# GuidoManni/BodySLAM

Measured on AMD Instinct MI355X. Metric: frames/sec depth+pose+back-proj, 640x480 seq, higher is better.
Workload: dtype f16

## Files before the change

bodyslam_amd/_lib.py:

```python
from __future__ import annotations

import ctypes as C
import os
from typing import Optional

import torch

_HERE = os.path.dirname(os.path.abspath(__file__))
LIB_PATH = os.environ.get("BODYSLAM_HIP_LIB") or os.path.join(_HERE, "libbodyslam_hip.so")

F32, F16, BF16 = 0, 1, 2
F64 = 3
ACT_NONE, ACT_RELU, ACT_GELU, ACT_SOFTPLUS, ACT_SOFTPLUS_FAST = 0, 1, 2, 3, 4
OUT_PLAIN, OUT_SHUFFLE, OUT_QKV = 0, 1, 2

_TORCH2BS = {torch.float32: F32, torch.float16: F16, torch.bfloat16: BF16}
BS2TORCH = {F32: torch.float32, F16: torch.float16, BF16: torch.bfloat16}


class BodySlamHipError(RuntimeError):
    pass


class GemmDesc(C.Structure):
    _fields_ = [
        ("A", C.c_void_p), ("W", C.c_void_p), ("dtype", C.c_int32),
        ("M", C.c_int32), ("N", C.c_int32), ("K", C.c_int32), ("lda", C.c_int32), ("conv", C.c_int32),
        ("Hin", C.c_int32), ("Win", C.c_int32), ("Cin", C.c_int32), ("Hout", C.c_int32), ("Wout", C.c_int32),
        ("KH", C.c_int32), ("KW", C.c_int32), ("stride", C.c_int32), ("pad_h", C.c_int32), ("pad_w", C.c_int32),
        ("relu_a", C.c_int32),
        ("bias", C.c_void_p), ("bias_group_rows", C.c_int32), ("act", C.c_int32),
        ("scale", C.c_void_p), ("res", C.c_void_p), ("res_dtype", C.c_int32), ("ldr", C.c_int32), ("res2", C.c_void_p),
        ("out", C.c_void_p), ("out2", C.c_void_p), ("out3", C.c_void_p),
        ("out_dtype", C.c_int32), ("ldo", C.c_int32), ("out_mode", C.c_int32),
        ("out_group_rows", C.c_int32), ("out_group_stride", C.c_int32), ("out_row_offset", C.c_int32),
        ("shuffle_s", C.c_int32), ("shuffle_cout", C.c_int32),
        ("qkv_hidden", C.c_int32), ("qkv_tokens", C.c_int32), ("qkv_sp", C.c_int32), ("q_scale", C.c_float),
        ("tile", C.c_int32), ("seg1", C.c_int32), ("out_split_off", C.c_int32), ("res_split_off", C.c_int32),
        ("f8_seg", C.c_int32), ("f8_scales", C.c_uint32), ("out_f8", C.c_int32), ("res_f8", C.c_int32),
        ("qkv_cls_last", C.c_int32), ("qkv_cls_rows", C.c_int32), ("qkv_patch_row0", C.c_int32), ("f8_wonly_from", C.c_int32), ("out_lo8_rows", C.c_int32),
        ("f8_skip_from", C.c_int32), ("bias2_row0", C.c_int32), ("bias2_group_rows", C.c_int32), ("out_planes_rows", C.c_int32),
        ("bias2", C.c_void_p),
        ("qkv_lo_off", C.c_int32), ("out2_relu", C.c_int32),
    ]


_lib: Optional[C.CDLL] = None

_SIGS = {
    "bs_init": [C.c_int],
    "bs_version": [],
    "bs_gemm": [C.POINTER(GemmDesc), C.c_void_p],
    "bs_gemm_tile": [C.POINTER(GemmDesc)],
    "bs_attention": [C.c_void_p] * 5 + [C.c_int32] * 5 + [C.c_void_p],
    "bs_attention_table": [C.c_void_p] * 5 + [C.c_int32] * 7 + [C.c_void_p],
    "bs_attention_table_corr": [C.c_void_p] * 8 + [C.c_int32] * 7 + [C.c_void_p],
    "bs_layernorm": [C.c_void_p] * 5 + [C.c_int32, C.c_int32, C.c_float, C.c_int32, C.c_void_p],
    "bs_cast": [C.c_void_p, C.c_void_p, C.c_int64, C.c_int32, C.c_void_p],
    "bs_copy_f32": [C.c_void_p, C.c_void_p, C.c_int64, C.c_void_p],
    "bs_cast_split": [C.c_void_p, C.c_void_p, C.c_int64, C.c_int32, C.c_int32, C.c_void_p],
    "bs_relu_split": [C.c_void_p, C.c_void_p, C.c_int64, C.c_int32, C.c_int32, C.c_void_p],
    "bs_preprocess_patches": [C.c_void_p, C.c_void_p] + [C.c_int32] * 7 + [C.c_void_p],
    "bs_preprocess_image": [C.c_void_p, C.c_void_p] + [C.c_int32] * 6 + [C.c_void_p],
    "bs_fill_rows": [C.c_void_p, C.c_void_p, C.c_int32, C.c_int32, C.c_int32, C.c_void_p],
    "bs_resize_bilinear_nhwc": [C.c_void_p, C.c_void_p] + [C.c_int32] * 8 + [C.c_void_p],
    "bs_upconv_tapsum": [C.c_void_p] * 3 + [C.c_int32] * 9 + [C.c_void_p],
    "bs_upconv_fused": [C.c_void_p] * 4 + [C.c_int32] * 15 + [C.c_void_p],
    "bs_resize_bias_relu_nhwc": [C.c_void_p] * 3 + [C.c_int32] * 8 + [C.c_void_p],
    "bs_col_mean": [C.c_void_p, C.c_int64] + [C.c_int32] * 5 + [C.c_void_p, C.c_void_p, C.c_int64, C.c_int32, C.c_void_p],
    "bs_rank1_bias": [C.c_void_p] * 3 + [C.c_int32] * 3 + [C.c_void_p],
    "bs_depth_u16_to_m": [C.c_void_p, C.c_int64, C.c_double, C.c_double, C.c_void_p, C.c_void_p],
    "bs_engine_load": [C.c_char_p, C.c_void_p],
    "bs_engine_destroy": [C.c_void_p],
    "bs_engine_io": [C.c_void_p, C.c_char_p, C.c_void_p, C.c_void_p],
    "bs_engine_device_bytes": [C.c_void_p],
    "bs_engine_run": [C.c_void_p, C.c_void_p],
    "bs_engine_upload": [C.c_void_p, C.c_char_p, C.c_void_p, C.c_int64],
    "bs_engine_download": [C.c_void_p, C.c_char_p, C.c_void_p, C.c_int64],
    "bs_zoedepth_forward": [C.c_void_p, C.c_void_p, C.c_int32, C.c_int32, C.c_int32, C.c_void_p, C.c_void_p, C.c_void_p],
    "bs_cyclepose_forward": [C.c_void_p, C.c_void_p, C.c_int32, C.c_int32, C.c_int32, C.c_void_p, C.c_int32, C.c_void_p, C.c_void_p],
    "bs_tsdf_frames_upload": [C.c_void_p, C.c_void_p, C.c_void_p, C.c_void_p, C.c_void_p, C.c_int32, C.c_void_p, C.c_void_p],
    "bs_tsdf_touch_batch": [C.c_void_p, C.c_int32, C.c_int32, C.c_int32, C.c_int32, C.c_double, C.c_double, C.c_void_p, C.c_void_p, C.c_int32, C.c_void_p,
                            C.c_void_p],
    "bs_tsdf_integrate_batch": [C.c_void_p, C.c_int32, C.c_int32, C.c_int32, C.c_void_p, C.c_void_p, C.c_void_p, C.c_int32, C.c_void_p, C.c_int32, C.c_void_p,
                                C.c_void_p, C.c_void_p, C.c_void_p, C.c_int32, C.c_int32, C.c_double, C.c_double, C.c_void_p],
    "bs_tsdf_update_batch": [C.c_void_p, C.c_int32, C.c_int32, C.c_int32, C.c_void_p, C.c_void_p, C.c_void_p, C.c_int32, C.c_void_p, C.c_int32, C.c_void_p,
                             C.c_void_p, C.c_void_p, C.c_void_p, C.c_int32, C.c_int32, C.c_double, C.c_double, C.c_uint64, C.c_void_p],
    "bs_odo_prepare": [C.c_void_p, C.c_void_p, C.c_int32, C.c_int32, C.c_int32, C.c_double, C.c_void_p, C.c_void_p, C.c_void_p],
    "bs_odo_pyrdown": [C.c_void_p, C.c_int32, C.c_int32, C.c_int32, C.c_void_p, C.c_int32, C.c_double, C.c_void_p],
    "bs_odo_sobel": [C.c_void_p, C.c_int32, C.c_int32, C.c_int32, C.c_void_p, C.c_void_p, C.c_void_p],
    "bs_odo_accumulate": [C.c_void_p] * 8 + [C.c_int32, C.c_int32, C.c_void_p, C.c_void_p, C.c_double, C.c_double, C.c_double, C.c_void_p, C.c_void_p,
                                              C.c_int32, C.c_void_p],
    "bs_odo_step": [C.c_void_p] * 8 + [C.c_int32, C.c_int32, C.c_int32, C.c_void_p, C.c_void_p, C.c_int32, C.c_double, C.c_double, C.c_double, C.c_void_p,
                                        C.c_void_p, C.c_int32, C.c_void_p],
    "bs_odo_p2p_prepare": [C.c_void_p, C.c_int32, C.c_int32, C.c_int32, C.c_double, C.c_void_p, C.c_void_p],
    "bs_odo_p2p_target": [C.c_void_p, C.c_int32, C.c_int32, C.c_int32, C.c_void_p, C.c_void_p, C.c_void_p],
    "bs_odo_p2p_accumulate": [C.c_void_p, C.c_void_p, C.c_int32, C.c_int32, C.c_void_p, C.c_void_p, C.c_double, C.c_double, C.c_void_p, C.c_void_p,
                              C.c_void_p],
    "bs_odo_p2p_step": [C.c_void_p, C.c_void_p, C.c_int32, C.c_int32, C.c_int32, C.c_void_p, C.c_void_p, C.c_int32, C.c_double, C.c_double, C.c_void_p,
                        C.c_void_p, C.c_void_p],
    "bs_tsdf_extract": [C.c_void_p, C.c_int32, C.c_void_p, C.c_void_p, C.c_int32, C.c_void_p, C.c_int32, C.c_int32, C.c_double, C.c_void_p, C.c_void_p,
                        C.c_void_p, C.c_void_p, C.c_void_p, C.c_void_p],
    "bs_tsdf_mesh": [C.c_void_p, C.c_int32, C.c_void_p, C.c_void_p, C.c_int32, C.c_void_p, C.c_int32, C.c_int32, C.c_double, C.c_void_p, C.c_int32] + [C.c_void_p] * 7,
    "bs_tsdf_raycast": [C.c_void_p, C.c_void_p, C.c_int32, C.c_int32, C.c_int32, C.c_double, C.c_double, C.c_void_p, C.c_void_p, C.c_int32, C.c_void_p,
                        C.c_int32, C.c_int32, C.c_double, C.c_double, C.c_void_p, C.c_void_p, C.c_void_p, C.c_void_p, C.c_void_p],
    "bs_attractor_step": [C.c_void_p] * 4 + [C.c_int32] * 8 + [C.c_void_p],
    "bs_add_resized": [C.c_void_p] * 3 + [C.c_int32] * 7 + [C.c_void_p],
    "bs_mlp2": [C.c_void_p, C.c_int32] + [C.c_void_p] * 5 + [C.c_int32] * 6 + [C.c_void_p],
    "bs_mlp2_add": [C.c_void_p] * 7 + [C.c_int32] * 10 + [C.c_void_p],
    "bs_projector_level": [C.c_void_p] * 10 + [C.c_int32] * 9 + [C.c_void_p],
    "bs_logbinom_depth": [C.c_void_p] * 8 + [C.c_int32] * 5 + [C.c_float, C.c_float, C.c_int32, C.c_void_p],
    "bs_logbinom_depth_ex": [C.c_void_p] * 7 + [C.c_int32] + [C.c_void_p] * 2 + [C.c_int32] * 5 + [C.c_float, C.c_float, C.c_int32, C.c_void_p],
    "bs_small_attention": [C.c_void_p, C.c_void_p, C.c_int32, C.c_int32, C.c_int32, C.c_int32, C.c_void_p],
    "bs_route_argmax": [C.c_void_p, C.c_int32, C.c_void_p, C.c_int32, C.c_void_p],
    "bs_postprocess_depth": [C.c_void_p] * 3 + [C.c_int32] * 6 + [C.c_void_p],
    "bs_cyclepose_im2col": [C.c_void_p] * 3 + [C.c_int32] * 4 + [C.c_void_p],
    "bs_cyclepose_im2col_window": [C.c_void_p] * 3 + [C.c_int32] * 8 + [C.c_void_p],
    "bs_instnorm_relu_nhwc": [C.c_void_p] * 4 + [C.c_int32] * 3 + [C.c_float, C.c_int32, C.c_void_p],
    "bs_avgpool_nhwc": [C.c_void_p, C.c_void_p, C.c_int32, C.c_int32, C.c_int32, C.c_void_p],
    "bs_cyclepose_head": [C.c_void_p] * 12 + [C.c_int32] * 3 + [C.c_void_p],
    "bs_backproject": [C.c_void_p, C.c_int32, C.c_int32, C.c_int32, C.c_void_p, C.c_double, C.c_double] + [C.c_void_p] * 6,
    "bs_pose_chain": [C.c_void_p, C.c_int32, C.c_void_p, C.c_void_p, C.c_void_p],
    "bs_pose_chain_from": [C.c_void_p, C.c_int32, C.c_void_p, C.c_void_p, C.c_void_p],
    "bs_pixel_to_3d": [C.c_void_p, C.c_int64, C.c_void_p, C.c_void_p, C.c_void_p],
    "bs_depth_metrics_workspace": [C.c_int32, C.c_int32, C.c_int32],
    "bs_depth_metrics": [C.c_void_p, C.c_void_p] + [C.c_int32] * 3 + [C.c_double, C.c_double, C.c_int32, C.c_double, C.c_void_p, C.c_int64,
# ... 88 lines not shown


_inited_device: Optional[int] = None


def init(device: int = 0) -> None:
    global _inited_device
    lib = load_library()
    if _inited_device == device:
        return
    if not torch.cuda.is_available():
        raise BodySlamHipError("bodyslam_amd needs an MI355X (gfx950) GPU: torch.cuda.is_available() is False "
                               "and there is no CPU fallback")
    check(lib.bs_init(device), "bs_init")
    _inited_device = device


def check(status: int, what: str) -> None:
    if status != 0:
        msg = load_library().bs_last_error().decode(errors="replace")
        raise BodySlamHipError(f"{what} failed with status {status}: {msg}")


def stream_ptr() -> int:
    return torch.cuda.current_stream().cuda_stream


def dt(t: torch.Tensor) -> int:
    return _TORCH2BS[t.dtype]


def p(t: Optional[torch.Tensor]) -> Optional[int]:
    return None if t is None else t.data_ptr()


def make_gemm_desc(A: torch.Tensor, W: torch.Tensor, out: torch.Tensor, *, M: int, N: int, K: int, lda: int,
                   conv=None, relu_a: bool = False, bias: Optional[torch.Tensor] = None, bias_group_rows: int = 0,
                   act: int = ACT_NONE, scale: Optional[torch.Tensor] = None, res: Optional[torch.Tensor] = None,
                   res2: Optional[torch.Tensor] = None, ldr: int = 0, ldo: Optional[int] = None, out_group=None,
                   shuffle=None, qkv=None, a_offset: int = 0, tile: int = 0, seg1: int = 0, out_split_off: int = 0,
                   res_split_off: int = 0, f8_seg: int = 0, f8_scales=(127, 127, 127, 127), out_f8=None, res_f8: bool = False,
                   f8_wonly_from: int = 0, out_lo8_rows: int = 0, f8_skip_from: int = 0, bias2=None, out_planes_rows: int = 0,
                   out_relu: Optional[torch.Tensor] = None) -> GemmDesc:
    d = GemmDesc()
    d.A = A.data_ptr() + a_offset * A.element_size()
    d.W = W.data_ptr()
    assert A.dtype == W.dtype and A.dtype in (torch.float16, torch.bfloat16), (A.dtype, W.dtype)
    d.dtype = dt(A)
    d.M, d.N, d.K, d.lda = M, N, K, lda
    if conv is not None:
        d.conv = 1
        (d.Hin, d.Win, d.Cin, d.Hout, d.Wout, d.KH, d.KW, d.stride, d.pad_h, d.pad_w) = conv
    d.relu_a = int(relu_a)
    if bias is not None:
        assert bias.dtype == torch.float32
        d.bias = bias.data_ptr()
    d.bias_group_rows = bias_group_rows
    d.act = act
    if scale is not None:
        assert scale.dtype == torch.float32
        d.scale = scale.data_ptr()
    if res is not None:
        d.res = res.data_ptr()
        d.res_dtype = dt(res)
        d.ldr = ldr if ldr else N
    if res2 is not None:
        assert res is not None and res2.dtype == A.dtype
        d.res2 = res2.data_ptr()
    d.out = out.data_ptr()
    d.out_dtype = dt(out)
    d.ldo = N if ldo is None else ldo
    if out_group is not None:
        d.out_group_rows, d.out_group_stride, d.out_row_offset = out_group
    if shuffle is not None:
        d.out_mode = OUT_SHUFFLE
        d.shuffle_s, d.shuffle_cout, d.Hout, d.Wout = shuffle
    if qkv is not None:
        d.out_mode = OUT_QKV
        hidden, tokens, sp, q_scale, out_k, out_vt = qkv[:6]
        d.qkv_cls_last = int(bool(qkv[6])) if len(qkv) > 6 else 0
        d.qkv_cls_rows = int(qkv[7]) if len(qkv) > 7 else 0
        d.qkv_patch_row0 = int(qkv[8]) if len(qkv) > 8 else d.qkv_cls_rows
        d.qkv_lo_off = int(qkv[9]) if len(qkv) > 9 else 0
        d.qkv_hidden, d.qkv_tokens, d.qkv_sp, d.q_scale = hidden, tokens, sp, q_scale
        d.out2 = out_k.data_ptr()
        d.out3 = out_vt.data_ptr()
    d.tile = tile
    d.seg1, d.out_split_off, d.res_split_off = seg1, out_split_off, res_split_off
    d.f8_seg = f8_seg
    d.f8_scales = f8_scales[0] | (f8_scales[1] << 8) | (f8_scales[2] << 16) | (f8_scales[3] << 24)
    d.out_f8 = 0 if out_f8 is None else ((out_f8[0] & 0xff) | ((out_f8[1] & 0xff) << 8))
    d.res_f8 = int(res_f8)
    d.f8_wonly_from = f8_wonly_from
    d.out_lo8_rows = out_lo8_rows
    d.f8_skip_from = f8_skip_from
    d.out_planes_rows = out_planes_rows
    if bias2 is not None:
        b2, row0, grows = bias2
        assert b2.dtype == torch.float32 and b2.shape[-1] == N
        d.bias2, d.bias2_row0, d.bias2_group_rows = b2.data_ptr(), row0, grows
    if out_relu is not None:
        assert qkv is None and out_f8 is not None and out_relu.dtype == out.dtype and out_relu.numel() == out.numel()
        d.out2 = out_relu.data_ptr()
        d.out2_relu = 1
    return d


def gemm(A: torch.Tensor, W: torch.Tensor, out: torch.Tensor, **kw) -> None:
    d = make_gemm_desc(A, W, out, **kw)
    check(load_library().bs_gemm(C.byref(d), stream_ptr()), "bs_gemm")


def _gemm_bytes(d) -> float:
    rows_in = float(d.M if not d.conv else d.M / max(d.stride * d.stride, 1))
    rows_f8 = 0.0 if d.f8_skip_from < 0 else (rows_in if (d.conv or not d.f8_skip_from) else float(min(d.f8_skip_from, d.M)))
    taps = d.KH * d.KW if d.conv else 1
    a = rows_in * (d.Cin if d.conv else d.K) * 2 + rows_f8 * d.f8_seg
    w = float(d.N) * (d.K * 2 + taps * d.f8_seg)
    if d.out_dtype == F32:
        per_row = [4.0, 4.0, 4.0]
    elif d.out_f8:
        per_row = [4.0, 3.0, 2.0]
    else:
        per_row = [2.0 * (2 if d.out_split_off else 1)] * 3
    full = float(d.M)
    r_planes = float(min(d.out_planes_rows, d.M)) if d.out_planes_rows else full
    r_lo = float(min(d.out_lo8_rows, d.M)) if d.out_lo8_rows else r_planes
    r_lo = min(r_lo, r_planes)
    out = d.N * (r_lo * per_row[0] + (r_planes - r_lo) * per_row[1] + (full - r_planes) * per_row[2])
    res = float(d.M) * d.N * (4 if (d.res and d.res_dtype == F32) else 0)
    return a + w + out + res


class Plan:

    def __init__(self, device=None):
        self.device = None if device is None else torch.device(device)
        self.calls = []
        self.names = []
        self.keep = []
        self.keep_descs = []
        self.marks = {}
        self.gemm_info = {}
        self.stack_info = {}
        self.events = None
        self._graph = None

    def gemm(self, name, A, W, out, **kw):
        passes = kw.pop("precision_passes", 1)
        d = make_gemm_desc(A, W, out, **kw)
        kw["precision_passes"] = passes
        self.keep.append((d, A, W, out, kw))
        self.keep_descs.append(d)
        self.calls.append((load_library().bs_gemm, (C.byref(d),)))
        self.names.append(name)
        self.gemm_info[len(self.calls) - 1] = dict(
            name=name, tile=load_library().bs_gemm_tile(C.byref(d)), conv=bool(d.conv),
            flops=2.0 * d.N * (d.M * d.K + (0 if d.f8_skip_from < 0 else (min(d.f8_skip_from, d.M) if d.f8_skip_from else d.M)) * (d.KH * d.KW if d.conv else 1) * d.f8_seg
                               / (4 if d.f8_wonly_from else 2)),
            alg_flops=2.0 * d.M * d.N * (d.K / kw.get("precision_passes", 1)),
            bytes=_gemm_bytes(d))

    def add(self, name, fn_name, *args):
        cargs = []
        for a in args:
            if isinstance(a, torch.Tensor):
# ... 73 lines not shown
def _f8_pack_device(device):
    if device is None or os.environ.get("BS_PACK_ON_HOST") == "1":
        return torch.device("cpu")
    device = torch.device(device)
    if device.type != "cuda":
        return torch.device("cpu")
    ok = _F8_ON_DEVICE.get(device.index)
    if ok is None:
        g = torch.Generator().manual_seed(7)
        t = torch.cat([torch.randn(4096, generator=g) * 100.0, torch.randn(4096, generator=g) * 1e-2, torch.linspace(-460.0, 460.0, 4097),
                       torch.arange(0, 4096, dtype=torch.float32) * 2.0 ** -11, torch.tensor([0.0, -0.0, 448.0, -448.0, 2.0 ** -9, 2.0 ** -10, 3 * 2.0 ** -11])])
        t = t.clamp(-448.0, 448.0)
        try:
            ok = bool(torch.equal(t.to(torch.float8_e4m3fn).view(torch.uint8), t.to(device).to(torch.float8_e4m3fn).view(torch.uint8).cpu()))
        except Exception:
            ok = False
        _F8_ON_DEVICE[device.index] = ok
    return device if ok else torch.device("cpu")


def f8_weight(w: torch.Tensor, dtype, planes: str = "both", device=None) -> tuple:
    import math
    w = w.detach().to(_f8_pack_device(device)).float()
    hi = w.to(dtype)
    lo = w - hi.float()

    def plane(t):
        mx = float(t.abs().max())
        e = 0 if mx == 0.0 else min(int(math.floor(math.log2(448.0 / mx))), 100)
        return (t * (2.0 ** e)).clamp(-448.0, 448.0).to(torch.float8_e4m3fn).view(torch.uint8), e

    hi8, e_hi = plane(hi.float())
    lo8, e_lo = plane(lo)
    hi16 = hi.contiguous().view(torch.uint8).view(w.shape[0], -1)
    if planes == "lo":
        row = torch.cat([hi16, lo8], 1).contiguous()
    elif planes == "hi_only":
        row = torch.cat([hi16, torch.zeros_like(lo8), hi8], 1).contiguous()
    else:
        row = torch.cat([hi16, lo8, hi8], 1).contiguous()
    return row.view(dtype), (127 - e_lo, 127 - e_hi)


def f8_conv_weight(w_ohwi: torch.Tensor, dtype, device=None) -> tuple:
    import math
    w = w_ohwi.detach().to(_f8_pack_device(device)).float()
    O, kh, kw, I = w.shape
    assert I % 128 == 0, I
    hi = w.to(dtype)
    lo = w - hi.float()

    def plane(t):
        mx = float(t.abs().max())
        e = 0 if mx == 0.0 else min(int(math.floor(math.log2(448.0 / mx))), 100)
        q = (t * (2.0 ** e)).clamp(-448.0, 448.0).to(torch.float8_e4m3fn).view(torch.uint8)
        return q.reshape(O, kh, kw, I // 128, 128).permute(0, 3, 1, 2, 4).reshape(O, -1), e

    hi8, e_hi = plane(hi.float())
    lo8, e_lo = plane(lo)
    hi16 = conv_weight(hi).view(torch.uint8).view(O, -1)
    row = torch.cat([hi16, lo8, hi8], 1).contiguous()
    return row.view(dtype), (127 - e_lo, 127 - e_hi)


F8_ACT_HI_EXP, F8_ACT_LO_EXP = 0, 11


def conv_weight(w_ohwi: torch.Tensor) -> torch.Tensor:
    O, kh, kw, I = w_ohwi.shape
    assert I % 64 == 0, I
    return w_ohwi.reshape(O, kh, kw, I // 64, 64).permute(0, 3, 1, 2, 4).reshape(O, -1).contiguous()


def conv_geom(Hin, Win, Cin, KH, KW, stride, pad):
    Hout = (Hin + 2 * pad - KH) // stride + 1
    Wout = (Win + 2 * pad - KW) // stride + 1
    return (Hin, Win, Cin, Hout, Wout, KH, KW, stride, pad, pad)


def attention(q, k, vt, bias, out, B, nh, S, Sp, split=0):
    check(load_library().bs_attention(p(q), p(k), p(vt), p(bias), p(out), B, nh, S, Sp, dt(q) | split, stream_ptr()), "bs_attention")


def attention_table(q, k, vt, table, out, B, nh, hp, wp, Sp, split=0, grouped=0):
    check(load_library().bs_attention_table(p(q), p(k), p(vt), p(table), p(out), B, nh, hp, wp, Sp, int(grouped), dt(q) | split, stream_ptr()),
          "bs_attention_table")


def attention_table_corr(q, k, vt, q_lo, k_lo, vt_lo, table, out, B, nh, hp, wp, Sp, split=0, grouped=0):
    check(load_library().bs_attention_table_corr(p(q), p(k), p(vt), p(q_lo), p(k_lo), p(vt_lo), p(table), p(out), B, nh, hp, wp, Sp, int(grouped),
                                                 dt(q) | split, stream_ptr()), "bs_attention_table_corr")


def layernorm(x, gamma, beta, out16, out32, rows, cols, eps, dtype=F16):
    check(load_library().bs_layernorm(p(x), p(gamma), p(beta), p(out16), p(out32), rows, cols, eps,
                                      dt(out16) if out16 is not None else dtype, stream_ptr()), "bs_layernorm")


def cast(x, out):
    check(load_library().bs_cast(p(x), p(out), x.numel(), dt(out), stream_ptr()), "bs_cast")


def cast_split(x, out, rows, cols, f8=False):
    check(load_library().bs_cast_split(p(x), p(out), rows, cols, dt(out) | (32 if f8 else 0), stream_ptr()), "bs_cast_split")


def relu_split(x, out, rows, cols, f8=False):
    check(load_library().bs_relu_split(p(x), p(out), rows, cols, dt(out) | (32 if f8 else 0), stream_ptr()), "bs_relu_split")


def preprocess_patches(frames, out, B, H, W, nh, nw, flip):
    check(load_library().bs_preprocess_patches(p(frames), p(out), B, H, W, nh, nw, int(flip), dt(out), stream_ptr()),
          "bs_preprocess_patches")


def preprocess_image(frames, out, B, H, W, nh, nw, flip):
    check(load_library().bs_preprocess_image(p(frames), p(out), B, H, W, nh, nw, int(flip), stream_ptr()), "bs_preprocess_image")


def fill_rows(x, v, B, rows_per_image, cols):
    check(load_library().bs_fill_rows(p(x), p(v), B, rows_per_image, cols, stream_ptr()), "bs_fill_rows")


def resize_bilinear_nhwc(x, out, B, Hin, Win, Cch, Hout, Wout, align_corners=True, split=False):
    check(load_library().bs_resize_bilinear_nhwc(p(x), p(out), B, Hin, Win, Cch, Hout, Wout, int(align_corners) | (4 if split == 2 else (2 if split else 0)), dt(x),
                                                 stream_ptr()), "bs_resize_bilinear_nhwc")


def depth_u16_to_m(depth_u16: torch.Tensor, depth_scale: float, depth_trunc: float) -> torch.Tensor:
    assert depth_u16.dtype == torch.int16 and depth_u16.is_cuda and depth_u16.is_contiguous()
    out = torch.empty(depth_u16.shape, dtype=torch.float32, device=depth_u16.device)
    check(load_library().bs_depth_u16_to_m(p(depth_u16), depth_u16.numel(), float(depth_scale), float(depth_trunc), p(out), stream_ptr()),
          "bs_depth_u16_to_m")
    return out


def col_mean(A, lda, row0, rows_per_group, groups, row_step, K, out, zero=None):
    assert out.dtype == torch.bfloat16 and (zero is None or zero.dtype == torch.float32)
    check(load_library().bs_col_mean(p(A), lda, row0, rows_per_group, groups, row_step, K, p(out), p(zero), 0 if zero is None else zero.numel(),
                                     dt(A), stream_ptr()), "bs_col_mean")


def rank1_bias(abar, dw, out):
    assert abar.dtype == torch.bfloat16 and dw.dtype == torch.bfloat16 and out.dtype == torch.float32
    G, K = abar.shape
    N = dw.shape[0]
    assert dw.shape[1] == K and tuple(out.shape) == (G, N)
    check(load_library().bs_rank1_bias(p(abar), p(dw), p(out), G, N, K, stream_ptr()), "bs_rank1_bias")


def upconv_tapsum(y, bias, out, B, Hin, Win, Cout, Hout, Wout, align_corners=True, split=False, relu=True):
    check(load_library().bs_upconv_tapsum(p(y), p(bias), p(out), B, Hin, Win, Cout, Hout, Wout,
                                          int(align_corners) | (4 if split == 2 else (2 if split else 0)), int(relu), dt(out), stream_ptr()),
          "bs_upconv_tapsum")


def upconv_fused(x, w, bias, out, B, Hin, Win, Cin, Cout, mode=0, split=0, relu=True, f8_scales=(127, 127, 127, 127)):
    check(load_library().bs_upconv_fused(p(x), p(w), p(bias), p(out), B, Hin, Win, Cin, Cout, 2 * Hin, 2 * Win,
                                         1 | (4 if split == 2 else (2 if split else 0)), int(relu), mode, *[int(v) for v in f8_scales], dt(out),
                                         stream_ptr()), "bs_upconv_fused")


def resize_bias_relu_nhwc(x, bias, out, B, Hin, Win, Cch, Hout, Wout, split=False):
    check(load_library().bs_resize_bias_relu_nhwc(p(x), p(bias), p(out), B, Hin, Win, Cch, Hout, Wout, 1 | (2 if split else 0), dt(out), stream_ptr()),
          "bs_resize_bias_relu_nhwc")


def attractor_step(A, bins_prev, bins_out, route, B, Hp, Wp, H, W, groups, n_bins, n_attr):
    check(load_library().bs_attractor_step(p(A), p(bins_prev), p(bins_out), p(route), B, Hp, Wp, H, W, groups, n_bins, n_attr,
                                           stream_ptr()), "bs_attractor_step")


def mlp2(x, ldx, W1, b1, W2, b2, out, M, K1, N1, N2, act2=ACT_SOFTPLUS_FAST):
    check(load_library().bs_mlp2(p(x), ldx, p(W1), p(b1), p(W2), p(b2), p(out), M, K1, N1, N2, act2, dt(x), stream_ptr()), "bs_mlp2")
# ... 631 lines not shown
```

bodyslam_amd/csrc/attention.hip:

```cpp
#include <stdlib.h>

#include <type_traits>

#include "common.h"

namespace bs {
__device__ __forceinline__ float half_swap_max(float v) {
    int k = __builtin_bit_cast(int, v);
    k ^= (k >> 31) & 0x7fffffff;
    const auto sw = __builtin_amdgcn_permlane32_swap((unsigned)k, (unsigned)k, false, false);
    const int a = (int)sw[0], b = (int)sw[1];
    int m = a > b ? a : b;
    m ^= (m >> 31) & 0x7fffffff;
    return __builtin_bit_cast(float, m);
}

__device__ __forceinline__ void dma_barrier() {
    asm volatile("s_waitcnt vmcnt(0)" ::: "memory");
    __syncthreads();
}


template <typename T, int QW>
__global__ __launch_bounds__(QW * 64) void attention_kernel(const T* __restrict__ Q, const T* __restrict__ K, const T* __restrict__ Vt,
// ... 359 lines not shown
    dma_barrier();
    if (1 < nkt) stage(1, 1);
    load_bias(0);
    for (int kt = 0; kt < nkt; ++kt) {
        if (ablate & 32) break;
        if (kt > 0) {
            dma_barrier();
            if (kt + 1 < nkt && !(ablate & 16)) stage(kt + 1, (kt + 1) & 1);
        }
        const char* sk = smem + (kt & 1) * STAGE;
        const char* sv = sk + 8 * 1024;
#pragma unroll
        for (int sub = 0; sub < 2; ++sub) {
            const int ky = kt * 2 + sub;
            if (ky > hp) break;
            f32x16 sacc;
#pragma unroll
            for (int i = 0; i < 16; ++i) sacc[i] = bnext[i] - m_run;
            if (ky + 1 <= hp && !(ablate & 8)) load_bias(ky + 1);
            const int krow = sub * 32 + kap;
#pragma unroll
            for (int ks = 0; ks < 4; ++ks) {
                if (ablate & 4) break;
                const int chunk = 2 * ks + h2;
                const v8 kf = *reinterpret_cast<const v8*>(sk + krow * 128 + ((chunk ^ ((krow >> 1) & 7)) << 4));
                sacc = T16<T>::mfma32(kf, qf[ks], sacc);
            }
            float mloc = fmaxf(fmaxf(sacc[0], sacc[1]), sacc[2]);
#pragma unroll
            for (int i = 3; i < 15; i += 2) mloc = fmaxf(fmaxf(mloc, sacc[i]), sacc[i + 1]);
            mloc = fmaxf(mloc, sacc[15]);
            mloc = half_swap_max(mloc);
            if (first || __any(mloc > THR)) {
                const float sh = first ? mloc : fmaxf(mloc, 0.0f);
                const float alpha = first ? 1.0f : __builtin_amdgcn_exp2f(-sh);
                l_run *= alpha;
#pragma unroll
                for (int i = 0; i < 16; ++i) {
                    oacc[0][i] *= alpha;
                    oacc[1][i] *= alpha;
                    sacc[i] -= sh;
                }
                m_run += sh;
                first = false;
            }
            float p[16];
            float psum = 0.f;
            if (ablate & 1) {
#pragma unroll
                for (int i = 0; i < 16; ++i) p[i] = sacc[i];
            } else {
#pragma unroll
                for (int i = 0; i < 16; ++i) {
                    p[i] = __builtin_amdgcn_exp2f(sacc[i]);
                    psum += p[i];
                }
            }
            l_run += psum;
            v8 pf[2];
#pragma unroll
            for (int s2 = 0; s2 < 2; ++s2)
#pragma unroll
                for (int e = 0; e < 8; ++e) pf[s2][e] = T16<T>::from_f32(p[8 * s2 + e]);
#pragma unroll
            for (int dh = 0; dh < 2; ++dh) {
                if (ablate & 2) break;
                const int drow = dh * 32 + r;
#pragma unroll
                for (int s2 = 0; s2 < 2; ++s2) {
                    const int chunk = sub * 4 + 2 * s2 + h2;
                    const v8 vf = *reinterpret_cast<const v8*>(sv + drow * 128 + ((chunk ^ ((drow >> 1) & 7)) << 4));
                    oacc[dh] = T16<T>::mfma32(vf, pf[s2], oacc[dh]);
                }
            }
        }
    }
    const float l_tot = l_run + __shfl_xor(l_run, 32, 64);
    const float inv = 1.0f / l_tot;
    __syncthreads();
    store_out_tile<T>(smem + wave * 8192, oacc, inv, out, split, nh, head, grouped ? (int64_t)grouped + (int64_t)b * (S - 1) : (int64_t)b * S + 1,
                      grouped ? (int64_t)b : (int64_t)b * S, S, q0, active, lane, cls_planes);
}

template <typename T, int QW, bool CORR>
__device__ __forceinline__ void cls_query_pass(const T* __restrict__ Qg, const T* __restrict__ Kg, const T* __restrict__ Vg, const T* __restrict__ Qlg,
                                               const T* __restrict__ Klg, const T* __restrict__ Vlg, int Sp, int hp, const float* __restrict__ tail3,
                                               char* area, int wave, int lane, T* __restrict__ out, int split, int nh, int head, int64_t row0,
                                               int64_t row_cls, int S, bool cls_planes) {
    typedef typename T16<T>::v8 v8;
    const int r = lane & 31, h2 = lane >> 5;
    const int kap = (r & ~12) | ((r & 4) << 1) | ((r & 8) >> 1);
    const int q0 = hp * 32;
    constexpr float THR = 6.0f;
    const float b_cp = tail3[0], b_cc = tail3[2];
    v8 qf[4], qlf[CORR ? 4 : 1];
#pragma unroll
    for (int ks = 0; ks < 4; ++ks) {
        qf[ks] = *reinterpret_cast<const v8*>(Qg + (int64_t)(q0 + r) * 64 + ks * 16 + h2 * 8);
        if constexpr (CORR) qlf[ks] = *reinterpret_cast<const v8*>(Qlg + (int64_t)(q0 + r) * 64 + ks * 16 + h2 * 8);
    }
    f32x16 oacc[2];
#pragma unroll
    for (int i = 0; i < 16; ++i) {
        oacc[0][i] = 0.f;
        oacc[1][i] = 0.f;
    }
    float m_run = 0.f, l_run = 0.f;
    bool first = true;
    auto load_k = [&](int ky, v8 (&kf)[4], v8 (&kfl)[CORR ? 4 : 1]) {
        const int64_t krow = (int64_t)ky * 32 + kap;
#pragma unroll
        for (int ks = 0; ks < 4; ++ks) {
            kf[ks] = *reinterpret_cast<const v8*>(Kg + krow * 64 + (2 * ks + h2) * 8);
            if constexpr (CORR) kfl[ks] = *reinterpret_cast<const v8*>(Klg + krow * 64 + (2 * ks + h2) * 8);
        }
    };
    v8 kf[4], kfl[CORR ? 4 : 1];
    load_k(wave, kf, kfl);
#pragma unroll 1
    for (int ky = wave; ky <= hp; ky += QW) {
        v8 vf[4], vfl[CORR ? 4 : 1];
#pragma unroll
        for (int dh = 0; dh < 2; ++dh)
#pragma unroll
            for (int s2 = 0; s2 < 2; ++s2) {
                const int64_t voff = (int64_t)(dh * 32 + r) * Sp + ky * 32 + (2 * s2 + h2) * 8;
                vf[dh * 2 + s2] = *reinterpret_cast<const v8*>(Vg + voff);
                if constexpr (CORR) vfl[dh * 2 + s2] = *reinterpret_cast<const v8*>(Vlg + voff);
            }
        v8 kn[4], knl[CORR ? 4 : 1];
        const int kyn = ky + QW <= hp ? ky + QW : ky;
        load_k(kyn, kn, knl);
        f32x16 sacc;
#pragma unroll
        for (int i = 0; i < 16; ++i) sacc[i] = (ky < hp ? b_cp : -1.0e30f) - m_run;
        if (ky == hp && h2 == 0) sacc[0] = b_cc - m_run;
#pragma unroll
        for (int ks = 0; ks < 4; ++ks) {
            sacc = T16<T>::mfma32(kf[ks], qf[ks], sacc);
            if constexpr (CORR) {
                sacc = T16<T>::mfma32(kf[ks], qlf[ks], sacc);
                sacc = T16<T>::mfma32(kfl[ks], qf[ks], sacc);
            }
        }
        float mloc = sacc[0];
#pragma unroll
        for (int i = 1; i < 16; ++i) mloc = fmaxf(mloc, sacc[i]);
        mloc = half_swap_max(mloc);
        if (first || __any(mloc > THR)) {
            const float sh = first ? mloc : fmaxf(mloc, 0.0f);
            const float alpha = first ? 1.0f : __builtin_amdgcn_exp2f(-sh);
            l_run *= alpha;
#pragma unroll
            for (int i = 0; i < 16; ++i) {
                oacc[0][i] *= alpha;
                oacc[1][i] *= alpha;
                sacc[i] -= sh;
            }
            m_run += sh;
            first = false;
        }
        float psum = 0.f;
        v8 pf[2], pfl[CORR ? 2 : 1];
#pragma unroll
        for (int s2 = 0; s2 < 2; ++s2)
#pragma unroll
            for (int e = 0; e < 8; ++e) {
                const float pv = __builtin_amdgcn_exp2f(sacc[8 * s2 + e]);
                psum += pv;
                pf[s2][e] = T16<T>::from_f32(pv);
                if constexpr (CORR) pfl[s2][e] = T16<T>::from_f32(pv - T16<T>::to_f32(pf[s2][e]));
            }
        l_run += psum;
#pragma unroll
        for (int dh = 0; dh < 2; ++dh)
#pragma unroll
            for (int s2 = 0; s2 < 2; ++s2) {
                oacc[dh] = T16<T>::mfma32(vf[dh * 2 + s2], pf[s2], oacc[dh]);
                if constexpr (CORR) {
                    oacc[dh] = T16<T>::mfma32(vf[dh * 2 + s2], pfl[s2], oacc[dh]);
                    oacc[dh] = T16<T>::mfma32(vfl[dh * 2 + s2], pf[s2], oacc[dh]);
                }
            }
#pragma unroll
        for (int ks = 0; ks < 4; ++ks) {
            kf[ks] = kn[ks];
            if constexpr (CORR) kfl[ks] = knl[ks];
        }
    }
    const float l_tot = l_run + __shfl_xor(l_run, 32, 64);
    float* part = reinterpret_cast<float*>(area);
    if (r == 0) {
        float* pp = part + (wave * 2 + h2) * 36;
        pp[0] = m_run;
        pp[1] = l_tot;
#pragma unroll
        for (int i = 0; i < 16; ++i) {
            pp[2 + i] = oacc[0][i];
            pp[18 + i] = oacc[1][i];
        }
    }
    __syncthreads();
    if (wave != 0) return;
    float M = part[h2 * 36];
#pragma unroll 1
    for (int w = 1; w < QW; ++w) M = fmaxf(M, part[(w * 2 + h2) * 36]);
    float L = 0.f;
#pragma unroll
    for (int i = 0; i < 16; ++i) {
        oacc[0][i] = 0.f;
        oacc[1][i] = 0.f;
    }
#pragma unroll 1
    for (int w = 0; w < QW; ++w) {
        const float* pp = part + (w * 2 + h2) * 36;
        const float f = __builtin_amdgcn_exp2f(pp[0] - M);
        L = fmaf(pp[1], f, L);
#pragma unroll
        for (int i = 0; i < 16; ++i) {
            oacc[0][i] = fmaf(pp[2 + i], f, oacc[0][i]);
            oacc[1][i] = fmaf(pp[18 + i], f, oacc[1][i]);
        }
    }
    __builtin_amdgcn_fence(__ATOMIC_RELEASE, "wavefront");
    __builtin_amdgcn_wave_barrier();
    store_out_tile<T>(area, oacc, 1.0f / L, out, split, nh, head, row0, row_cls, S, q0, true, lane, cls_planes);
}

template <typename T, int QW, int WPE, bool CORR, bool PK = false, bool CLS2 = false>
__global__ __launch_bounds__(QW * 64, WPE) void attention_tab2_kernel(const T* __restrict__ Q, const T* __restrict__ K, const T* __restrict__ Vt,
                                                                  const T* __restrict__ Ql, const T* __restrict__ Kl, const T* __restrict__ Vtl,
                                                                  const float* __restrict__ table, T* __restrict__ out, int split, int B, int nh,
                                                                  int hp, int Sp, int nqb, int ntab, int grouped) {
    BS_ARG_NOW(out);
    const bool cls_planes = (split & 4) != 0;
    const int abl = split >> 3;
    split &= 3;
    typedef typename T16<T>::v8 v8;
    constexpr int HALF = 16 * 1024;
    constexpr int STAGE = CORR ? 2 * HALF : HALF;
    constexpr int WP = 32, RW = 2 * WP - 1;
    extern __shared__ __attribute__((aligned(16))) char smem[];
    float* tab = reinterpret_cast<float*>(smem + 2 * STAGE);
    const int ntab_pad = (ntab + 255) & ~255;
    float* creg = tab + ntab_pad;
    const int S = hp * WP + 1, nqt = CLS2 ? hp : hp + 1;

    const int nwg = gridDim.x, bid = blockIdx.x;
    const int xq = nwg >> 3, xr = nwg & 7, xcd = bid & 7, loc = bid >> 3;
    const int wg = (xcd < xr ? xcd * (xq + 1) : xr * (xq + 1) + (xcd - xr) * xq) + loc;
    const int qblk = wg % nqb;
    const int b = (wg / nqb) % B;
    const int head = wg / (B * nqb);

    const int tid = threadIdx.x, lane = tid & 63;
    const int wave = __builtin_amdgcn_readfirstlane(tid >> 6);
    const int r = lane & 31, h2 = lane >> 5;
    int qt = qblk * QW + wave;
    const bool active = qt < nqt;
    qt = active ? qt : nqt - 1;
    const int q0 = qt * 32;
    const bool cls_tile = !CLS2 && qt == hp;
    const int64_t bh = (int64_t)b * nh + head;

    const T* Qg = Q + bh * Sp * 64;
    const T* Kg = K + bh * Sp * 64;
    const T* Vg = Vt + bh * 64 * Sp;
    const T* Klg = CORR ? Kl + bh * Sp * 64 : nullptr;
    const T* Vlg = CORR ? Vtl + bh * 64 * Sp : nullptr;

    load_table<QW * 64>(tab, table, head, ntab, tid, wave, lane);
    if (tid < 64) creg[tid] = table[(int64_t)head * ntab + ntab - 3];

    v8 qf[4], qlf[CORR ? 4 : 1];
#pragma unroll
    for (int ks = 0; ks < 4; ++ks) qf[ks] = *reinterpret_cast<const v8*>(Qg + (int64_t)(q0 + r) * 64 + ks * 16 + h2 * 8);
    if constexpr (CORR) {
#pragma unroll
        for (int ks = 0; ks < 4; ++ks) qlf[ks] = *reinterpret_cast<const v8*>(Ql + bh * Sp * 64 + (int64_t)(q0 + r) * 64 + ks * 16 + h2 * 8);
    }

    const int srow = lane >> 3;
    auto stage = [&](int kt, int buf) {
        char* sb = smem + buf * STAGE;
        for (int i = wave; i < (CORR ? 32 : 16); i += QW) {
            const int j = i & 15;
            const int row = (j & 7) * 8 + srow;
            const int cs8 = ((lane & 7) ^ ((row >> 1) & 7)) * 8;
            const T* kb = (CORR && i >= 16) ? Klg : Kg;
            const T* vb = (CORR && i >= 16) ? Vlg : Vg;
            const T* src = j < 8 ? kb + (int64_t)(kt * 64 + row) * 64 + cs8 : vb + (int64_t)row * Sp + kt * 64 + cs8;
            glds16(src, sb + i * 1024);
        }
    };

    f32x16 oacc[2];
#pragma unroll
    for (int i = 0; i < 16; ++i) {
        oacc[0][i] = 0.f;
        oacc[1][i] = 0.f;
    }
    float m_run = 0.f, l_run = 0.f;
    bool first = true;
    const int kap = (r & ~12) | ((r & 4) << 1) | ((r & 8) >> 1);
    constexpr float THR = 6.0f;

    const int nbody = ntab - 3;
    const float* lt = cls_tile ? creg : tab + (nbody - RW - (qt + hp - 1) * RW) + (31 - r + 8 * h2);
    const int rstep = cls_tile ? 0 : RW;
    auto load_bias = [&](f32x16& sacc, int ky) {
        const float* rowp = lt + ky * rstep;
#pragma unroll
        for (int s2 = 0; s2 < 2; ++s2)
#pragma unroll
            for (int e = 0; e < 8; ++e) sacc[8 * s2 + e] = rowp[16 * s2 + e];
    };
    auto qk = [&](f32x16& sacc, const char* sk, int sub) {
        if constexpr (PK) {
            const f32x2_ nm = {-m_run, -m_run};
#pragma unroll
            for (int i = 0; i < 16; i += 2) {
                const f32x2_ v = f32x2_{sacc[i], sacc[i + 1]} + nm;
                sacc[i] = v[0];
                sacc[i + 1] = v[1];
            }
        } else {
#pragma unroll
            for (int i = 0; i < 16; ++i) sacc[i] -= m_run;
        }
        const int krow = sub * 32 + kap;
#pragma unroll
        for (int ks = 0; ks < 4; ++ks) {
            const int chunk = 2 * ks + h2;
            const int off = krow * 128 + ((chunk ^ ((krow >> 1) & 7)) << 4);
            const v8 kf = *reinterpret_cast<const v8*>(sk + off);
            sacc = T16<T>::mfma32(kf, qf[ks], sacc);
            if constexpr (CORR) {
                sacc = T16<T>::mfma32(kf, qlf[ks], sacc);
                const v8 kfl = *reinterpret_cast<const v8*>(sk + HALF + off);
                sacc = T16<T>::mfma32(kfl, qf[ks], sacc);
            }
        }
    };
    auto softmax_pv = [&](f32x16& sacc, f32x16& other, const char* sv, int sub, int next_ky, auto other_tag, auto next_tag) {
        constexpr bool OTHER = decltype(other_tag)::value;
        constexpr bool NEXT = decltype(next_tag)::value;
        float mloc = fmaxf(fmaxf(sacc[0], sacc[1]), sacc[2]);
#pragma unroll
        for (int i = 3; i < 15; i += 2) mloc = fmaxf(fmaxf(mloc, sacc[i]), sacc[i + 1]);
        mloc = fmaxf(mloc, sacc[15]);
        mloc = half_swap_max(mloc);
        if (first || __any(mloc > THR)) {
                const float sh = first ? mloc : fmaxf(mloc, 0.0f);
                const float alpha = first ? 1.0f : __builtin_amdgcn_exp2f(-sh);
            l_run *= alpha;
#pragma unroll
            for (int i = 0; i < 16; ++i) {
                oacc[0][i] *= alpha;
                oacc[1][i] *= alpha;
                sacc[i] -= sh;
                if (OTHER) other[i] -= sh;
            }
            m_run += sh;
            first = false;
        }
        float psum = 0.f;
        v8 pf[2], pfl[CORR ? 2 : 1];
#pragma unroll
        for (int s2 = 0; s2 < 2; ++s2)
#pragma unroll
            for (int e = 0; e < 8; ++e) {
                const float pv = __builtin_amdgcn_exp2f(sacc[8 * s2 + e]);
                psum += pv;
                pf[s2][e] = T16<T>::from_f32(pv);
                if constexpr (CORR) pfl[s2][e] = T16<T>::from_f32(pv - T16<T>::to_f32(pf[s2][e]));
            }
        l_run += psum;
        if (NEXT) load_bias(sacc, next_ky);
#pragma unroll
        for (int dh = 0; dh < 2; ++dh) {
            const int drow = dh * 32 + r;
#pragma unroll
            for (int s2 = 0; s2 < 2; ++s2) {
                const int chunk = sub * 4 + 2 * s2 + h2;
                const int off = drow * 128 + ((chunk ^ ((drow >> 1) & 7)) << 4);
                const v8 vf = *reinterpret_cast<const v8*>(sv + off);
                oacc[dh] = T16<T>::mfma32(vf, pf[s2], oacc[dh]);
                if constexpr (CORR) {
                    oacc[dh] = T16<T>::mfma32(vf, pfl[s2], oacc[dh]);
                    const v8 vfl = *reinterpret_cast<const v8*>(sv + HALF + off);
                    oacc[dh] = T16<T>::mfma32(vfl, pf[s2], oacc[dh]);
                }
            }
        }
    };

    const int NT = hp >> 1;
    f32x16 sa, sb2;
    typedef std::true_type Yes;
    typedef std::false_type No;
    stage(0, 0);
    dma_barrier();
    load_bias(sa, 0);
    load_bias(sb2, 1);
    for (int kt = 0; kt < NT - 1; ++kt) {
        if (kt > 0) {
            if (abl == 0) dma_barrier();
            else {
                if (!(abl & 2)) asm volatile("s_waitcnt vmcnt(0)" ::: "memory");
                if (!(abl & 1)) __syncthreads();
            }
        }
        if (!(abl & 4) || kt == 0) stage(kt + 1, (kt + 1) & 1);
        const char* sk = smem + (kt & 1) * STAGE;
        qk(sa, sk, 0);
        qk(sb2, sk, 1);
        softmax_pv(sa, sb2, sk + 8 * 1024, 0, 2 * kt + 2, Yes{}, Yes{});
        softmax_pv(sb2, sa, sk + 8 * 1024, 1, 2 * kt + 3, No{}, Yes{});
    }
    {
        if (NT > 1) dma_barrier();
        stage(NT, NT & 1);
        const char* sk = smem + ((NT - 1) & 1) * STAGE;
        qk(sa, sk, 0);
        qk(sb2, sk, 1);
        softmax_pv(sa, sb2, sk + 8 * 1024, 0, 0, Yes{}, No{});
#pragma unroll
        for (int i = 0; i < 16; ++i) sa[i] = -1.0e30f;
        if (h2 == 0) sa[0] = cls_tile ? tab[ntab - 1] : tab[ntab - 2];
        softmax_pv(sb2, sa, sk + 8 * 1024, 1, 0, No{}, No{});
        dma_barrier();
        const char* sk2 = smem + (NT & 1) * STAGE;
        qk(sa, sk2, 0);
        softmax_pv(sa, sb2, sk2 + 8 * 1024, 0, 0, No{}, No{});
    }
    const float l_tot = l_run + __shfl_xor(l_run, 32, 64);
    const float inv = 1.0f / l_tot;
    __syncthreads();
    store_out_tile<T>(smem + wave * 8192, oacc, inv, out, split, nh, head, grouped ? (int64_t)grouped + (int64_t)b * (S - 1) : (int64_t)b * S + 1,
                      grouped ? (int64_t)b : (int64_t)b * S, S, q0, active, lane, cls_planes);
    if constexpr (CLS2) {
        if (qblk == 0) {
            __syncthreads();
            cls_query_pass<T, QW, CORR>(Qg, Kg, Vg, CORR ? Ql + bh * Sp * 64 : nullptr, Klg, Vlg, Sp, hp, table + (int64_t)head * ntab + ntab - 3,
                                        smem + 2 * STAGE + (ntab_pad + 64) * 4, wave, lane, out, split, nh, head,
                                        grouped ? (int64_t)grouped + (int64_t)b * (S - 1) : (int64_t)b * S + 1, grouped ? (int64_t)b : (int64_t)b * S, S,
                                        cls_planes);
        }
    }
}

template <typename T>
static int launch_attn_tab(const void* q, const void* k, const void* vt, const void* ql, const void* kl, const void* vtl, const float* table, void* out,
                           int split, int B, int nh, int hp, int Sp, int grouped, hipStream_t st) {
    constexpr int QW = 5;
    const int nqt = hp + 1, nqb = cdiv(nqt, QW), ntab = (2 * hp - 1) * 63 + 3;
    const int tab_bytes = (((ntab + 255) & ~255) + 64) * 4;
    if (ql) {
        static const bool cls2_ok = diag_env("BS_ATTN_NO_CLS2") == nullptr;
        if (cls2_ok && hp % 8 == 0) {
            auto kb = attention_tab2_kernel<T, 8, 2, true, false, true>;
            BS_MAX_DYNAMIC_LDS(reinterpret_cast<const void*>(kb), 96 * 1024);
            hipLaunchKernelGGL(kb, dim3(B * nh * (hp / 8)), dim3(8 * 64), 64 * 1024 + tab_bytes + 8192, st, (const T*)q, (const T*)k, (const T*)vt,
                               (const T*)ql, (const T*)kl, (const T*)vtl, table, (T*)out, split, B, nh, hp, Sp, hp / 8, ntab, grouped);
            BS_CHECK_LAUNCH();
            return BS_OK;
        }
        {
            const int nb8 = cdiv(nqt, 8), qw8 = cdiv(nqt, nb8);
#define BS_ATTN_CORR_BIG(QWB)                                                                                                                \
    do {                                                                                                                                     \
        auto kb = attention_tab2_kernel<T, QWB, 2, true>;                                                                                    \
        BS_MAX_DYNAMIC_LDS(reinterpret_cast<const void*>(kb), 96 * 1024); \
        hipLaunchKernelGGL(kb, dim3(B * nh * nb8), dim3(QWB * 64), 64 * 1024 + tab_bytes, st, (const T*)q, (const T*)k, (const T*)vt,        \
                           (const T*)ql, (const T*)kl, (const T*)vtl, table, (T*)out, split, B, nh, hp, Sp, nb8, ntab, grouped);             \
        BS_CHECK_LAUNCH();                                                                                                                   \
        return BS_OK;                                                                                                                        \
    } while (0)
            if (qw8 == 7) BS_ATTN_CORR_BIG(7);
            if (qw8 == 8) BS_ATTN_CORR_BIG(8);
#undef BS_ATTN_CORR_BIG
        }
        auto kc = attention_tab2_kernel<T, QW, 2, true>;
        BS_MAX_DYNAMIC_LDS(reinterpret_cast<const void*>(kc), 88 * 1024);
        hipLaunchKernelGGL(kc, dim3(B * nh * nqb), dim3(QW * 64), 64 * 1024 + tab_bytes, st, (const T*)q, (const T*)k, (const T*)vt, (const T*)ql,
                           (const T*)kl, (const T*)vtl, table, (T*)out, split, B, nh, hp, Sp, nqb, ntab, grouped);
        BS_CHECK_LAUNCH();
        return BS_OK;
    }
    int smem = 32 * 1024 + ((ntab * 4 + 1023) & ~1023);
    smem = smem < QW * 8192 ? QW * 8192 : smem;
    auto kern = attention_tab_kernel<T, QW>;
    BS_MAX_DYNAMIC_LDS(reinterpret_cast<const void*>(kern), 64 * 1024);
    static const bool pipelined_ok = diag_env("BS_ATTN_NO_PIPE") == nullptr;
    if (hp % 2 == 0 && pipelined_ok) {
        static const bool wpe3 = diag_env("BS_ATTN_WPE3") != nullptr, pk = diag_env("BS_ATTN_NO_PK") == nullptr;
        auto kern2 = wpe3 ? (pk ? attention_tab2_kernel<T, QW, 3, false, true> : attention_tab2_kernel<T, QW, 3, false>)
                          : (pk ? attention_tab2_kernel<T, QW, 4, false, true> : attention_tab2_kernel<T, QW, 4, false>);
        BS_MAX_DYNAMIC_LDS(reinterpret_cast<const void*>(kern2), 64 * 1024);
        static const int abl = diag_env("BS_ATTN_ABL") ? atoi(diag_env("BS_ATTN_ABL")) : 0;
        static const bool cls2_ok = diag_env("BS_ATTN_NO_CLS2") == nullptr;
        if (!wpe3 && pk && abl == 0 && cls2_ok && hp % 8 == 0) {
            auto kb = attention_tab2_kernel<T, 8, 4, false, true, true>;
            BS_MAX_DYNAMIC_LDS(reinterpret_cast<const void*>(kb), 128 * 1024);
            const int ldsb = 8 * 8192 > 32 * 1024 + tab_bytes + 8192 ? 8 * 8192 : 32 * 1024 + tab_bytes + 8192;
            hipLaunchKernelGGL(kb, dim3(B * nh * (hp / 8)), dim3(8 * 64), ldsb, st, (const T*)q, (const T*)k, (const T*)vt, (const T*)nullptr,
                               (const T*)nullptr, (const T*)nullptr, table, (T*)out, split, B, nh, hp, Sp, hp / 8, ntab, grouped);
            BS_CHECK_LAUNCH();
            return BS_OK;
        }
        if (!wpe3 && pk && abl == 0) {
            const int nb_big = cdiv(nqt, 14), qw_big = cdiv(nqt, nb_big);
#define BS_ATTN_BIG(QWB)                                                                                                                     \
    do {                                                                                                                                     \
        auto kb = attention_tab2_kernel<T, QWB, 4, false, true>;                                                                             \
        BS_MAX_DYNAMIC_LDS(reinterpret_cast<const void*>(kb), 128 * 1024); \
        const int ldsb = QWB * 8192 > 32 * 1024 + tab_bytes ? QWB * 8192 : 32 * 1024 + tab_bytes;                                            \
        hipLaunchKernelGGL(kb, dim3(B * nh * nb_big), dim3(QWB * 64), ldsb, st, (const T*)q, (const T*)k, (const T*)vt, (const T*)nullptr,   \
                           (const T*)nullptr, (const T*)nullptr, table, (T*)out, split, B, nh, hp, Sp, nb_big, ntab, grouped);               \
        BS_CHECK_LAUNCH();                                                                                                                   \
        return BS_OK;                                                                                                                        \
    } while (0)
            if (qw_big == 11) BS_ATTN_BIG(11);
            if (qw_big == 12) BS_ATTN_BIG(12);
            if (qw_big == 13) BS_ATTN_BIG(13);
            if (qw_big == 14) BS_ATTN_BIG(14);
#undef BS_ATTN_BIG
        }
        hipLaunchKernelGGL(kern2, dim3(B * nh * nqb), dim3(QW * 64), 32 * 1024 + tab_bytes, st, (const T*)q, (const T*)k, (const T*)vt, (const T*)nullptr,
                           (const T*)nullptr, (const T*)nullptr, table, (T*)out, split | (abl << 3), B, nh, hp, Sp, nqb, ntab, grouped);
        BS_CHECK_LAUNCH();
        return BS_OK;
    }
    hipLaunchKernelGGL(kern, dim3(B * nh * nqb), dim3(QW * 64), smem, st, (const T*)q, (const T*)k, (const T*)vt, table, (T*)out, split, B,
                       nh, hp, Sp, nqb, ntab, grouped, diag_env("BS_ATTN_ABLATE") ? atoi(diag_env("BS_ATTN_ABLATE")) : 0);
    BS_CHECK_LAUNCH();
    return BS_OK;
}

template <typename T, int QW>
static int launch_attn(const void* q, const void* k, const void* vt, const float* bias, void* out, int split, int B, int nh, int S, int Sp,
                       hipStream_t st) {
    const int nqt = cdiv(S, 32), nqb = cdiv(nqt, QW);
    hipLaunchKernelGGL((attention_kernel<T, QW>), dim3(B * nh * nqb), dim3(QW * 64), 32 * 1024, st, (const T*)q, (const T*)k,
                       (const T*)vt, bias, (T*)out, split, B, nh, S, Sp, nqt, nqb, diag_env("BS_ATTN_ABLATE") ? atoi(diag_env("BS_ATTN_ABLATE")) : 0);
    BS_CHECK_LAUNCH();
    return BS_OK;
}

template <typename T>
static int dispatch_attn(const void* q, const void* k, const void* vt, const float* bias, void* out, int split, int B, int nh, int S, int Sp,
                         hipStream_t st) {
    const int nqt = cdiv(S, 32);
    if (nqt >= 5) return launch_attn<T, 5>(q, k, vt, bias, out, split, B, nh, S, Sp, st);
    if (nqt % 3 == 0) return launch_attn<T, 3>(q, k, vt, bias, out, split, B, nh, S, Sp, st);
    return launch_attn<T, 4>(q, k, vt, bias, out, split, B, nh, S, Sp, st);
}

}

extern "C" int bs_attention(const void* q, const void* k, const void* vt, const float* bias, void* out, int32_t B, int32_t nh, int32_t S,
                            int32_t Sp, int32_t dtype, void* stream) {
    using namespace bs;
    if (!initialized()) { set_error("bs_attention: call bs_init first"); return BS_ERR_NOT_INIT; }
    BS_REQUIRE(q && k && vt && bias && out && B >= 0 && nh > 0 && S > 0, "bs_attention: bad argument");
    BS_REQUIRE(Sp % 64 == 0 && Sp >= S, "bs_attention: Sp=%d must be a multiple of 64 and >= S=%d", Sp, S);
    const int split = (dtype & 32) ? 2 : ((dtype & 16) ? 1 : 0);
    dtype &= 15;
    BS_REQUIRE(dtype == BS_F16 || dtype == BS_BF16, "bs_attention: dtype");
    if (B == 0) return BS_OK;
    hipStream_t st = reinterpret_cast<hipStream_t>(stream);
    return dtype == BS_F16 ? dispatch_attn<f16>(q, k, vt, bias, out, split, B, nh, S, Sp, st)
                           : dispatch_attn<bf16>(q, k, vt, bias, out, split, B, nh, S, Sp, st);
}

static int attention_table_entry(const char* who, const void* q, const void* k, const void* vt, const void* ql, const void* kl, const void* vtl,
                                 const float* table, void* out, int32_t B, int32_t nh, int32_t hp, int32_t wp, int32_t Sp, int32_t grouped,
                                 int32_t dtype, void* stream) {
    using namespace bs;
    if (!initialized()) { set_error("%s: call bs_init first", who); return BS_ERR_NOT_INIT; }
    BS_REQUIRE(q && k && vt && table && out && B >= 0 && nh > 0 && hp > 0, "%s: bad argument", who);
    BS_REQUIRE(wp == 32, "%s: built for windows of 32 patches per row (wp=%d): use bs_attention", who, wp);
    BS_REQUIRE(hp <= 40, "%s: hp=%d: the table must fit 32 KiB of LDS", who, hp);
    BS_REQUIRE(grouped == 0 || grouped >= B, "%s: grouped=%d is the first patch row, >= B", who, grouped);
    BS_REQUIRE(!ql || hp % 2 == 0, "%s: the split-precision kernel is built for an even number of patch rows (hp=%d)", who, hp);
    const int S = hp * wp + 1;
    BS_REQUIRE(Sp % 64 == 0 && Sp >= S, "%s: Sp=%d must be a multiple of 64 and >= S=%d", who, Sp, S);
    int split = (dtype & 32) ? 2 : ((dtype & 16) ? 1 : 0);
    if ((dtype & 64) && split == 2) split |= 4;
    dtype &= 15;
    BS_REQUIRE(dtype == BS_F16 || dtype == BS_BF16, "%s: dtype", who);
    if (B == 0) return BS_OK;
    hipStream_t st = reinterpret_cast<hipStream_t>(stream);
    return dtype == BS_F16 ? launch_attn_tab<f16>(q, k, vt, ql, kl, vtl, table, out, split, B, nh, hp, Sp, grouped, st)
                           : launch_attn_tab<bf16>(q, k, vt, ql, kl, vtl, table, out, split, B, nh, hp, Sp, grouped, st);
}

extern "C" int bs_attention_table(const void* q, const void* k, const void* vt, const float* table, void* out, int32_t B, int32_t nh,
                                  int32_t hp, int32_t wp, int32_t Sp, int32_t grouped, int32_t dtype, void* stream) {
    return attention_table_entry("bs_attention_table", q, k, vt, nullptr, nullptr, nullptr, table, out, B, nh, hp, wp, Sp, grouped, dtype, stream);
}

extern "C" int bs_attention_table_corr(const void* q, const void* k, const void* vt, const void* q_lo, const void* k_lo, const void* vt_lo,
                                       const float* table, void* out, int32_t B, int32_t nh, int32_t hp, int32_t wp, int32_t Sp, int32_t grouped,
                                       int32_t dtype, void* stream) {
    if (!q_lo || !k_lo || !vt_lo) { bs::set_error("bs_attention_table_corr: null residual tensor"); return BS_ERR_INVALID; }
    return attention_table_entry("bs_attention_table_corr", q, k, vt, q_lo, k_lo, vt_lo, table, out, B, nh, hp, wp, Sp, grouped, dtype, stream);
}
```

bodyslam_amd/csrc/engine.hip:

```cpp
#include <stdio.h>
#include <string.h>

#include <exception>
#include <map>
#include <string>
#include <tuple>
#include <type_traits>
#include <utility>
#include <memory>
#include <vector>

#include "common.h"

namespace {

constexpr char kMagic[8] = {'B', 'S', 'E', 'N', 'G', '0', '2', '\0'};
enum { KIND_WORKSPACE = 0, KIND_ZERO = 1, KIND_DATA = 2 };
enum { ARG_I64 = 0, ARG_F64 = 1, ARG_PTR = 2, ARG_NULL = 3, ARG_DESC = 4 };
enum { OP_CALL = 0, OP_SIGNAL = 1, OP_WAIT = 2 };

struct Arg {
    int64_t i = 0;
    double d = 0.0;
    void* p = nullptr;
};

template <typename T>
T arg_as(const Arg& a) {
    if constexpr (std::is_pointer<T>::value) return reinterpret_cast<T>(a.p);
    else if constexpr (std::is_floating_point<T>::value) return static_cast<T>(a.d);
    else return static_cast<T>(a.i);
}
template <typename... Args, size_t... I>
int call_unpacked(int (*fn)(Args...), const Arg* args, void* st, std::index_sequence<I...>) {
    using Tup = std::tuple<Args...>;
    return fn(arg_as<std::tuple_element_t<I, Tup>>(args[I])..., st);
}
struct Entry {
    int nargs;
    int (*thunk)(const void* fn, const Arg* args, void* st);
    const void* fn;
};
template <typename... Args>
Entry make_entry(int (*fn)(Args...)) {
    static_assert(sizeof...(Args) >= 1, "an entry point takes the stream last");
    Entry e;
    e.nargs = (int)sizeof...(Args) - 1;
    e.fn = reinterpret_cast<const void*>(fn);
    e.thunk = [](const void* f, const Arg* args, void* st) {
        return call_unpacked<Args...>(reinterpret_cast<int (*)(Args...)>(const_cast<void*>(f)), args, st, std::make_index_sequence<sizeof...(Args) - 1>{});
    };
    return e;
}
#define BS_ENGINE_ENTRY(name) {#name, make_entry(name)}
const std::map<std::string, Entry>& entries() {
    static const std::map<std::string, Entry> m = {
        BS_ENGINE_ENTRY(bs_gemm),           BS_ENGINE_ENTRY(bs_attention),          BS_ENGINE_ENTRY(bs_attention_table),
        BS_ENGINE_ENTRY(bs_attention_table_corr),
        BS_ENGINE_ENTRY(bs_layernorm),      BS_ENGINE_ENTRY(bs_cast),               BS_ENGINE_ENTRY(bs_copy_f32),
        BS_ENGINE_ENTRY(bs_cast_split),     BS_ENGINE_ENTRY(bs_relu_split),         BS_ENGINE_ENTRY(bs_preprocess_patches),
        BS_ENGINE_ENTRY(bs_fill_rows),      BS_ENGINE_ENTRY(bs_upconv_tapsum),      BS_ENGINE_ENTRY(bs_small_attention),
        BS_ENGINE_ENTRY(bs_route_argmax),   BS_ENGINE_ENTRY(bs_resize_bilinear_nhwc), BS_ENGINE_ENTRY(bs_rank1_bias),
        BS_ENGINE_ENTRY(bs_postprocess_depth), BS_ENGINE_ENTRY(bs_logbinom_depth_ex), BS_ENGINE_ENTRY(bs_col_mean),
        BS_ENGINE_ENTRY(bs_attractor_step), BS_ENGINE_ENTRY(bs_add_resized),        BS_ENGINE_ENTRY(bs_instnorm_relu_nhwc),
        BS_ENGINE_ENTRY(bs_cyclepose_im2col), BS_ENGINE_ENTRY(bs_cyclepose_im2col_window), BS_ENGINE_ENTRY(bs_cyclepose_head),
        BS_ENGINE_ENTRY(bs_avgpool_nhwc),   BS_ENGINE_ENTRY(bs_mlp2),            BS_ENGINE_ENTRY(bs_mlp2_add),
        BS_ENGINE_ENTRY(bs_upconv_fused),   BS_ENGINE_ENTRY(bs_resize_bias_relu_nhwc), BS_ENGINE_ENTRY(bs_projector_level),
    };
    return m;
}

struct Op {
    int kind = OP_CALL, lane = 0;
    const Entry* entry = nullptr;
    std::vector<Arg> args;
    std::vector<char> desc;
    std::string name;
};
struct Io {
    void* ptr;
    int64_t nbytes;
};

}

struct bs_engine {
    int device = 0;
    std::vector<void*> bufs;
    std::vector<Op> ops;
    std::map<std::string, Io> io;
    hipStream_t side = nullptr;
    std::map<int, hipEvent_t> events;
    int64_t device_bytes = 0;
};

namespace {

struct Reader {
    FILE* f;
// ... 296 lines not shown
```

bodyslam_amd/csrc/igemm.hip:

```cpp
#include <stdlib.h>

#include <map>
#include <mutex>
#include <utility>

#include "igemm_kernel.h"

namespace bs {

#define BS_DECL_TILE(t, cm)                                                  \
    int igemm_launch_tile##t##_f16_cm##cm(const IgemmParams&, bool, hipStream_t); \
    int igemm_launch_tile##t##_bf16_cm##cm(const IgemmParams&, bool, hipStream_t);
BS_DECL_TILE(1, 0) BS_DECL_TILE(1, 1)
BS_DECL_TILE(2, 0) BS_DECL_TILE(2, 1)
BS_DECL_TILE(3, 0) BS_DECL_TILE(3, 1)
BS_DECL_TILE(9, 0) BS_DECL_TILE(9, 1)
BS_DECL_TILE(10, 0) BS_DECL_TILE(11, 0)
BS_DECL_TILE(9s8, 0) BS_DECL_TILE(9s8, 1)
#undef BS_DECL_TILE

static int auto_tile(int M, int N, int K, int tile, bool conv) {
    if (tile != 0) return tile;
    if (N <= 32) return 3;
    if (N <= 64) return 2;
// ... 99 lines not shown
    }
    p.m_begin = 0;
    return launch_tile(p, dtype, conv, tile, st);
}

}

extern "C" int bs_gemm_tile(const bs_gemm_desc* d) {
    if (!d) return BS_ERR_INVALID;
    const int tile = bs::auto_tile(d->M, d->N, d->K + d->f8_seg / 2, d->tile % 100, d->conv != 0);
    return ((d->f8_seg > 0 || d->out_f8 || d->res_f8) && (tile == 10 || tile == 11)) ? 9 : tile;
}

extern "C" int bs_gemm(const bs_gemm_desc* d, void* stream) {
    using namespace bs;
    if (!initialized()) { set_error("bs_gemm: call bs_init first"); return BS_ERR_NOT_INIT; }
    BS_REQUIRE(d && d->A && d->W && d->out, "bs_gemm: null operand");
    BS_REQUIRE(d->dtype == BS_F16 || d->dtype == BS_BF16, "bs_gemm: dtype must be f16 or bf16");
    BS_REQUIRE(d->M > 0 && d->N > 0 && d->K > 0, "bs_gemm: empty problem M=%d N=%d K=%d", d->M, d->N, d->K);
    BS_REQUIRE(d->N % 4 == 0, "bs_gemm: N=%d must be a multiple of 4", d->N);
    BS_REQUIRE(d->K % 64 == 0, "bs_gemm: K=%d must be a multiple of 64", d->K);
    BS_REQUIRE(d->lda % 8 == 0, "bs_gemm: lda=%d must be a multiple of 8 (16-byte rows)", d->lda);
    BS_REQUIRE(d->out_dtype == BS_F32 || d->out_dtype == d->dtype, "bs_gemm: out_dtype must be f32 or the operand dtype");
    BS_REQUIRE(!d->res || d->res_dtype == BS_F32 || d->res_dtype == d->dtype, "bs_gemm: res_dtype must be f32 or the operand dtype");
    IgemmParams p{};
    p.A = d->A; p.W = d->W; p.zero = zero_page();
    p.a_bytes = d->conv ? (long long)(d->M / (d->Hout > 0 && d->Wout > 0 ? d->Hout * d->Wout : 1)) * d->Hin * d->Win * d->lda * 2
                        : ((long long)(d->M - 1) * d->lda + (d->K + d->f8_seg / 2 - d->seg1)) * 2;
    BS_REQUIRE((long long)d->N * (d->K + d->f8_seg / 2) * 2 < 0x7FFFFFF0ll, "bs_gemm: weight matrix too large for one descriptor");
    p.M = d->M; p.N = d->N; p.K = d->K + d->f8_seg / 2; p.lda = d->lda;
    p.f8_seg = d->f8_seg;
    p.f8_sa0 = d->f8_scales & 0xff; p.f8_sb0 = (d->f8_scales >> 8) & 0xff; p.f8_sa1 = (d->f8_scales >> 16) & 0xff; p.f8_sb1 = d->f8_scales >> 24;
    p.out_f8 = d->out_f8;
    p.res_f8 = d->res_f8;
    BS_REQUIRE(!d->res_f8 || (d->res && d->res_dtype == d->dtype && d->res_split_off == 0 && d->ldr >= 2 * d->N && d->N % 8 == 0), "bs_gemm: res_f8 needs a 16-bit residual in (hi16 | hi8 | lo8) rows, ldr >= 2N");
    BS_REQUIRE(d->f8_seg >= 0 && d->f8_seg % 256 == 0, "bs_gemm: f8_seg=%d must be a multiple of 256 (two halves of whole 128-byte stages)", d->f8_seg);
    BS_REQUIRE(d->f8_seg == 0 || (d->seg1 == 0 && !d->relu_a), "bs_gemm: the FP8 segment excludes seg1 and relu_a");
    p.f8_stages = d->f8_seg / 128;
    BS_REQUIRE(d->out_f8 == 0 || (d->out_dtype == d->dtype && d->ldo % 8 == 0 &&
                                  ((d->out_mode == BS_OUT_PLAIN && d->out_split_off == d->N && d->N % 8 == 0) ||
                                   (d->out_mode == BS_OUT_SHUFFLE && d->out_split_off == d->shuffle_cout && d->shuffle_cout % 8 == 0))),
               "bs_gemm: out_f8 needs a plain / shuffle 16-bit output with out_split_off = channels, channels %% 8 == 0");
    p.Hin = d->Hin; p.Win = d->Win; p.Cin = d->Cin; p.Hout = d->Hout; p.Wout = d->Wout;
    p.KH = d->KH; p.KW = d->KW; p.stride = d->stride; p.pad_h = d->pad_h; p.pad_w = d->pad_w;
    if (d->conv) {
        BS_REQUIRE(d->Cin > 0 && d->Cin % 64 == 0, "bs_gemm: conv Cin=%d must be a multiple of 64", d->Cin);
        BS_REQUIRE(d->K == d->KH * d->KW * (d->Cin + d->seg1), "bs_gemm: conv K=%d != KH*KW*(Cin+seg1)", d->K);
        BS_REQUIRE(d->Hout > 0 && d->Wout > 0 && d->M % (d->Hout * d->Wout) == 0, "bs_gemm: conv M=%d not a multiple of Hout*Wout", d->M);
        BS_REQUIRE(d->stride > 0 && d->lda >= d->Cin, "bs_gemm: bad conv stride/lda");
        BS_REQUIRE(d->KH > 0 && d->KW > 0 && d->KH * d->KW <= 32, "bs_gemm: conv window %dx%d: at most 32 taps", d->KH, d->KW);
        BS_REQUIRE((long long)d->Hin * d->Win * d->lda * 2 * 4 < 0x7FFFFFF0ll, "bs_gemm: image too large for the 2 GiB tile window");
        p.tiles_per_tap = d->Cin / 64;
        if (d->f8_seg > 0) {
            BS_REQUIRE(d->f8_seg == 2 * d->Cin && d->Cin % 128 == 0 && d->lda >= 2 * d->Cin, "bs_gemm: conv FP8 segment needs f8_seg = 2*Cin, Cin %% 128 == 0, lda >= 2*Cin");
            p.Cin = 2 * d->Cin;
            p.K = d->KH * d->KW * p.Cin;
            p.f8_stages = d->KH * d->KW * (d->f8_seg / 128);
            BS_REQUIRE((long long)d->N * p.K * 2 < 0x7FFFFFF0ll, "bs_gemm: weight matrix too large for one descriptor");
        }
    }
    p.relu_a = d->relu_a;
    p.cin1 = d->seg1;
    p.split_off = d->out_split_off;
    p.res_split_off = d->res_split_off;
    BS_REQUIRE(d->seg1 >= 0 && d->seg1 % 64 == 0, "bs_gemm: seg1=%d must be a multiple of 64", d->seg1);
    BS_REQUIRE(d->conv || d->seg1 < d->K, "bs_gemm: seg1 must be smaller than K");
    BS_REQUIRE(d->out_split_off == 0 || (d->out_mode != BS_OUT_QKV && d->out_dtype == d->dtype), "bs_gemm: split output needs a plain / shuffle 16-bit output");
    BS_REQUIRE(d->res_split_off == 0 || (d->res && d->res_dtype == d->dtype), "bs_gemm: split residual must be 16-bit");
    p.ablate = d->tile >= 100 ? d->tile / 100 : 0;

    BS_REQUIRE(!d->relu_a || d->conv, "bs_gemm: relu_a is only built for conv mode");
    BS_REQUIRE(d->act >= BS_ACT_NONE && d->act <= BS_ACT_SOFTPLUS_FAST, "bs_gemm: unknown activation %d", d->act);
    p.bias = d->bias; p.bias_group_rows = d->bias_group_rows; p.act = d->act; p.scale = d->scale;
    p.res = d->res; p.res2 = d->res2; p.res_dtype = d->res_dtype; p.ldr = d->ldr;
    BS_REQUIRE(!d->res2 || d->res, "bs_gemm: res2 needs res (they share ldr)");
    p.out = d->out; p.out2 = d->out2; p.out3 = d->out3; p.out_dtype = d->out_dtype; p.ldo = d->ldo; p.out_mode = d->out_mode;
    p.out_group_rows = d->out_group_rows; p.out_group_stride = d->out_group_stride; p.out_row_offset = d->out_row_offset;
    p.shuffle_s = d->shuffle_s; p.shuffle_cout = d->shuffle_cout;
    p.qkv_hidden = d->qkv_hidden; p.qkv_tokens = d->qkv_tokens; p.qkv_sp = d->qkv_sp; p.q_scale = d->q_scale;
    p.qkv_cls_last = d->qkv_cls_last;
    p.qkv_cls_rows = d->qkv_cls_rows;
    p.qkv_patch_row0 = d->qkv_patch_row0;
    p.qkv_lo_off = d->qkv_lo_off;
    p.out2_relu = d->out2_relu;
    BS_REQUIRE(!d->out2_relu || (d->out2 && d->out_mode == BS_OUT_PLAIN && d->out_f8 && !d->scale && !d->out_group_rows && !d->bias_group_rows &&
                                 !d->bias2 && (d->act == BS_ACT_NONE || d->act == BS_ACT_RELU) && d->out_split_off == d->N && d->N % 256 == 0 &&
                                 d->ldo % 8 == 0 && d->out_dtype == d->dtype && (!d->res || d->res_f8)),
               "bs_gemm: out2_relu needs the plain (hi16 | hi8 | lo8) output form (out_f8, N %% 256 == 0, no scale / row groups / bias2)");
    BS_REQUIRE(d->qkv_lo_off == 0 || (d->out_mode == BS_OUT_QKV && d->qkv_lo_off > 0 && d->qkv_lo_off % 8 == 0),
               "bs_gemm: qkv_lo_off needs BS_OUT_QKV and a multiple of 8 elements");
    p.f8_wonly_from = d->f8_wonly_from;
    p.out_lo8_rows = d->out_lo8_rows;
    p.f8_skip_from = d->f8_skip_from;
    p.out_planes_rows = d->out_planes_rows;
    BS_REQUIRE(d->out_planes_rows == 0 || (d->out_f8 && d->out_planes_rows > 0 && d->out_planes_rows % 256 == 0),
               "bs_gemm: out_planes_rows needs out_f8 and a multiple of 256 rows");
    p.bias2 = d->bias2;
    p.bias2_row0 = d->bias2_row0;
    p.bias2_group_rows = d->bias2_group_rows;
    BS_REQUIRE(d->f8_skip_from == 0 || (d->f8_seg > 0 && (d->f8_skip_from == -1 || (d->f8_skip_from > 0 && d->f8_skip_from % 256 == 0 && !d->conv))),
               "bs_gemm: f8_skip_from needs the FP8 correction segment and is -1 (every tile) or, for a plain GEMM, a multiple of 256 rows");
    BS_REQUIRE(!d->bias2 || (d->bias2_group_rows > 0 && d->bias2_row0 >= 0 && d->bias_group_rows == 0 && !d->conv && d->out_mode != BS_OUT_SHUFFLE &&
                             d->N % 4 == 0),
               "bs_gemm: bias2 needs bias2_group_rows > 0, a plain GEMM (PLAIN or QKV output) and no bias_group_rows");
    BS_REQUIRE(d->out_lo8_rows == 0 || (d->out_f8 && d->out_lo8_rows % 256 == 0), "bs_gemm: out_lo8_rows needs out_f8 and a multiple of 256 rows");
    BS_REQUIRE(d->f8_wonly_from == 0 || d->f8_seg > 0, "bs_gemm: f8_wonly_from needs the FP8 correction segment");
    BS_REQUIRE(d->qkv_cls_rows == 0 || (d->out_mode == BS_OUT_QKV && d->qkv_cls_last && d->qkv_tokens > 1 && d->qkv_patch_row0 >= d->qkv_cls_rows &&
                                        d->M == d->qkv_patch_row0 + d->qkv_cls_rows * (d->qkv_tokens - 1)),
               "bs_gemm: qkv_cls_rows needs BS_OUT_QKV, qkv_cls_last and M = qkv_patch_row0 + qkv_cls_rows * (tokens - 1)");
    if (d->out_mode == BS_OUT_SHUFFLE) {
        BS_REQUIRE(!d->conv && d->shuffle_s > 0 && d->shuffle_cout % 4 == 0 && d->N == d->shuffle_s * d->shuffle_s * d->shuffle_cout,
                   "bs_gemm: bad shuffle geometry");
        BS_REQUIRE(d->Hout > 0 && d->Wout > 0 && d->M % (d->Hout * d->Wout) == 0, "bs_gemm: shuffle needs the input grid in Hout/Wout");
    } else if (d->out_mode == BS_OUT_QKV) {
        BS_REQUIRE(d->out2 && d->out3 && d->qkv_hidden % 64 == 0 && d->N == 3 * d->qkv_hidden && d->qkv_tokens > 0 &&
                       (d->qkv_cls_rows > 0 || d->M % d->qkv_tokens == 0) && d->qkv_sp >= d->qkv_tokens && d->out_dtype == d->dtype,
                   "bs_gemm: bad qkv geometry");
    } else {
        BS_REQUIRE(d->out_mode == BS_OUT_PLAIN && d->ldo >= d->N, "bs_gemm: bad out_mode/ldo");
        BS_REQUIRE(d->ldo % 4 == 0, "bs_gemm: ldo must be a multiple of 4");
    }
    hipStream_t st = reinterpret_cast<hipStream_t>(stream);
    const int tile = d->tile % 100;
    return dispatch(p, d->dtype, d->conv != 0, tile, st);
}
```

bodyslam_amd/csrc/igemm_kernel.h:

```cpp
#pragma once
#include <type_traits>

#include "common.h"

namespace bs {

struct IgemmParams {
    const void* A;
    const void* W;
    const void* zero;
    long long a_bytes;
    int M, N, K, lda;
    int Hin, Win, Cin, Hout, Wout, KH, KW, stride, pad_h, pad_w;
    int tiles_per_tap;
    int cin1;
    int split_off;
    int res_split_off;
    int relu_a;
    const float* bias;
    int bias_group_rows;
    int act;
    const float* scale;
    const void* res;
    const void* res2;
    int res_dtype, ldr;
    void* out;
    void* out2;
    void* out3;
    int out_dtype, ldo, out_mode;
    int out_group_rows, out_group_stride, out_row_offset;
    int shuffle_s, shuffle_cout;
    int qkv_hidden, qkv_tokens, qkv_sp;
    int qkv_cls_last;
    int qkv_cls_rows;
    int qkv_patch_row0;
    int qkv_lo_off;
    int f8_wonly_from;
    float q_scale;
    int ntm, ntn;
    int m_begin;
    int f8_seg;
    int f8_sa0, f8_sb0, f8_sa1, f8_sb1;
    int f8_stages;
    int res_f8;
    int out_f8;
    int out2_relu;
    int out_lo8_rows;
    int f8_skip_from;
    int out_planes_rows;
    const float* bias2;
    int bias2_row0, bias2_group_rows;
    int strip;
    int ablate;
};

template <typename T>
__device__ __forceinline__ typename T16<T>::v8 relu8(typename T16<T>::v8 x) {
    typedef short s16x8 __attribute__((ext_vector_type(8)));
    s16x8 b = __builtin_bit_cast(s16x8, x);
    s16x8 neg = b >> 15;
    b = b & ~neg;
    return __builtin_bit_cast(typename T16<T>::v8, b);
}

template <typename T>
__device__ __forceinline__ void store4(void* base, int64_t off, int out_dtype, const float (&y)[4], int split_off = 0) {
    if (split_off > 0) {
        typename T16<T>::v4 h, l;
#pragma unroll
        for (int e = 0; e < 4; ++e) {
            h[e] = T16<T>::from_f32(y[e]);
            l[e] = T16<T>::from_f32(y[e] - T16<T>::to_f32(h[e]));
        }
        *reinterpret_cast<typename T16<T>::v4*>(reinterpret_cast<T*>(base) + off) = h;
        *reinterpret_cast<typename T16<T>::v4*>(reinterpret_cast<T*>(base) + off + split_off) = l;
        return;
    }
    if (out_dtype == BS_F32) {
        f32x4 v = {y[0], y[1], y[2], y[3]};
        *reinterpret_cast<f32x4*>(reinterpret_cast<float*>(base) + off) = v;
    } else {
        typename T16<T>::v4 v;
        v[0] = T16<T>::from_f32(y[0]);
        v[1] = T16<T>::from_f32(y[1]);
        v[2] = T16<T>::from_f32(y[2]);
        v[3] = T16<T>::from_f32(y[3]);
        *reinterpret_cast<typename T16<T>::v4*>(reinterpret_cast<T*>(base) + off) = v;
    }
}

template <typename T>
__device__ __forceinline__ void store8(void* base, int64_t off, int out_dtype, const float (&y)[8], int split_off = 0) {
    typedef typename T16<T>::v8 v8;
    if (split_off > 0) {
        v8 h, l;
#pragma unroll
        for (int e = 0; e < 8; ++e) {
            h[e] = T16<T>::from_f32(y[e]);
            l[e] = T16<T>::from_f32(y[e] - T16<T>::to_f32(h[e]));
        }
        *reinterpret_cast<v8*>(reinterpret_cast<T*>(base) + off) = h;
        *reinterpret_cast<v8*>(reinterpret_cast<T*>(base) + off + split_off) = l;
        return;
    }
    if (out_dtype == BS_F32) {
        *reinterpret_cast<f32x4*>(reinterpret_cast<float*>(base) + off) = f32x4{y[0], y[1], y[2], y[3]};
        *reinterpret_cast<f32x4*>(reinterpret_cast<float*>(base) + off + 4) = f32x4{y[4], y[5], y[6], y[7]};
    } else {
        v8 v;
#pragma unroll
        for (int e = 0; e < 8; ++e) v[e] = T16<T>::from_f32(y[e]);
        *reinterpret_cast<v8*>(reinterpret_cast<T*>(base) + off) = v;
    }
}

template <typename T>
__device__ __forceinline__ void store8_f8(void* base, int64_t row_off, int n, int plane_off, const float (&y)[8], int ea, int el, bool lo = true,
                                          bool hi8 = true) {
    typedef typename T16<T>::v8 v8;
// ... 448 lines not shown
                        for (int j = 0; j < FN; ++j) acc[i][j] = T16<T>::mfma16(bf[j], af[i], acc[i][j]);
                    __builtin_amdgcn_s_setprio(0);
                }
            }
            cbuf = cbuf + 1 == STAGES ? 0 : cbuf + 1;
            sbuf = sbuf + 1 == STAGES ? 0 : sbuf + 1;
        };
        int t = 0;
        __builtin_amdgcn_s_waitcnt(0xc07f);
        for (; t < nt16; ++t) iteration(t, std::integral_constant<int, 0>{});
        if constexpr (F8 && BK == 64 && !RELU_A) {
            for (; t < nt; ++t) iteration(t, std::integral_constant<int, 1>{});
        }
    } else {
        static_assert(BK == 32 && STAGES == 4 && WM == 2 && NW_CHECK(WM, WN) == 8, "ping-pong variant: 256x256x32, 8 waves");
        const int grp = wm;
        v8 af[FM], bf[FN];
        auto load_frags = [&](int buf) {
            const char* sa = smem + buf * STAGE;
            const char* sb = sa + A_BYTES;
#pragma unroll
            for (int i = 0; i < FM; ++i) {
                af[i] = *reinterpret_cast<const v8*>(sa + a_base + i * 16 * ROWB + koff0);
                if (RELU_A) af[i] = relu8<T>(af[i]);
            }
#pragma unroll
            for (int j = 0; j < FN; ++j) bf[j] = *reinterpret_cast<const v8*>(sb + b_base + j * 16 * ROWB + koff0);
        };
        auto compute = [&]() {
            __builtin_amdgcn_s_setprio(1);
#pragma unroll
            for (int i = 0; i < FM; ++i)
#pragma unroll
                for (int j = 0; j < FN; ++j) acc[i][j] = T16<T>::mfma16(bf[j], af[i], acc[i][j]);
            __builtin_amdgcn_s_setprio(0);
        };
        auto wait_tiles = [&](int younger) {
            if (younger >= 2) wait_vmcnt<2 * GL>();
            else if (younger == 1) wait_vmcnt<GL>();
            else wait_vmcnt<0>();
        };
        auto phase_barrier = [&]() {
            __builtin_amdgcn_sched_barrier(0);
            __builtin_amdgcn_s_barrier();
            __builtin_amdgcn_sched_barrier(0);
        };
#pragma unroll
        for (int s = 0; s < 3; ++s)
            if (s < nt) stage(s);
        wait_tiles((nt - 1 < 2 ? nt - 1 : 2));
        phase_barrier();
        int issued = nt - 1 < 2 ? nt - 1 : 2;
        if (grp == 1) {
            phase_barrier();
            if (3 < nt) { stage(3); issued = 3; }
        }
        __builtin_amdgcn_s_waitcnt(0xc07f);
        load_frags(0);
        int buf = 0;
        const int last = nt - 1;
        for (int t = 0; t < nt; ++t) {
            const int nbuf = buf == 3 ? 0 : buf + 1;
            if (grp == 1 && t + 1 < nt) wait_tiles(issued - (t + 1));
            phase_barrier();
            compute();
            if (grp == 0 && t + 1 < nt) wait_tiles(issued - (t + 1));
            phase_barrier();
            if (t + 1 < nt) {
                if (issued < last) { ++issued; stage(issued & 3); }
                load_frags(nbuf);
            }
            buf = nbuf;
        }
        if (grp == 0) phase_barrier();
    }

#define BS_FRESH_LANE                                                                                                       \
    int lane;                                                                                                               \
    asm volatile("v_mbcnt_lo_u32_b32 %0, -1, 0\n\tv_mbcnt_hi_u32_b32 %0, -1, %0" : "=v"(lane));                             \
    const int frow = lane & 15, fq = lane >> 4;                                                                             \
    (void)frow; (void)fq;
    {
    const int n_wave = tn * BN + wn * TN;
    const bool v_tile = (p.out_mode == BS_OUT_QKV) && (tn * BN >= 2 * p.qkv_hidden);
    if (p.ablate & 4) {
        if (acc[0][0][0] == 12345.678f) reinterpret_cast<float*>(p.out)[0] = 1.f;
        return;
    }
    int g2 = -1;
    bool b2_rows = false;
    if (p.bias2) {
        const int lo = m0 - p.bias2_row0, hi = (m0 + BM < p.M ? m0 + BM : p.M) - 1 - p.bias2_row0;
        if (hi >= 0) {
            if (lo >= 0 && lo / p.bias2_group_rows == hi / p.bias2_group_rows) g2 = lo / p.bias2_group_rows;
            else b2_rows = true;
        }
    }
    if (!v_tile) {
        auto epi = [&](auto act_tag) {
            constexpr int ACT = decltype(act_tag)::value;
            BS_FRESH_LANE
            f32x4 bj[FN], sj[FN];
            int n0j[FN];
            int64_t coff[FN];
            int which[FN];
#pragma unroll
            for (int j = 0; j < FN; ++j) {
                const int n0 = n_wave + (j >> 1) * 32 + fq * 8 + (j & 1) * 4;
                n0j[j] = n0;
                const bool ok = n0 < p.N;
                bj[j] = (p.bias && !p.bias_group_rows && ok) ? *reinterpret_cast<const f32x4*>(p.bias + n0) : f32x4{0.f, 0.f, 0.f, 0.f};
                if (g2 >= 0 && ok) bj[j] += *reinterpret_cast<const f32x4*>(p.bias2 + (int64_t)g2 * p.N + n0);
                sj[j] = (p.scale && ok) ? *reinterpret_cast<const f32x4*>(p.scale + n0) : f32x4{1.f, 1.f, 1.f, 1.f};
                which[j] = 0;
                if (p.out_mode == BS_OUT_PLAIN) {
                    coff[j] = n0;
                } else if (p.out_mode == BS_OUT_SHUFFLE) {
                    const int s = p.shuffle_s;
                    const int tap = n0 / p.shuffle_cout, co = n0 - tap * p.shuffle_cout;
                    const int ky = tap / s, kx = tap - ky * s;
                    coff[j] = ((int64_t)ky * (p.Wout * s) + kx) * p.ldo + co;
                } else {
                    const int w_ = n0 / p.qkv_hidden, rem = n0 - w_ * p.qkv_hidden;
                    which[j] = w_;
                    coff[j] = (int64_t)(rem >> 6) * p.qkv_sp * 64 + (rem & 63);
                    if (w_ == 0) {
#pragma unroll
                        for (int e = 0; e < 4; ++e) { sj[j][e] *= p.q_scale; bj[j][e] *= 1.0f; }
                    }
                }
            }
            const bool wide_ok = (p.out_mode == BS_OUT_QKV) || (p.ldo % 8 == 0 && p.split_off % 8 == 0);
#pragma unroll
            for (int i = 0; i < FM; ++i) {
                const int m = m0 + wm * TM + i * 16 + frow;
                if (m >= p.M) continue;
                int64_t orow = m;
                int64_t roff;
                const float* brow = nullptr;
                if (p.bias && p.bias_group_rows) brow = p.bias + (int64_t)(m / p.bias_group_rows) * p.N;
                const float* brow2 = (b2_rows && m >= p.bias2_row0) ? p.bias2 + (int64_t)((m - p.bias2_row0) / p.bias2_group_rows) * p.N : nullptr;
                if (p.out_mode == BS_OUT_PLAIN) {
                    if (p.out_group_rows) {
                        const int g = m / p.out_group_rows;
                        orow = (int64_t)g * p.out_group_stride + (m - g * p.out_group_rows) + p.out_row_offset;
                    }
                    roff = orow * p.ldo;
                } else if (p.out_mode == BS_OUT_SHUFFLE) {
                    const int hw = p.Hout * p.Wout;
                    const int ob = m / hw, rem = m - ob * hw;
                    const int oy = rem / p.Wout, ox = rem - oy * p.Wout;
                    const int s = p.shuffle_s;
                    roff = (((int64_t)(ob * p.Hout + oy) * s) * (p.Wout * s) + ox * s) * p.ldo;
                } else {
                    int ob, otok;
                    if (p.qkv_cls_rows > 0) {
                        if (m >= p.qkv_cls_rows && m < p.qkv_patch_row0) continue;
                        const int mp = m - p.qkv_patch_row0;
                        ob = mp < 0 ? m : mp / (p.qkv_tokens - 1);
                        otok = mp < 0 ? p.qkv_tokens - 1 : mp - ob * (p.qkv_tokens - 1);
                    } else {
                        ob = m / p.qkv_tokens;
                        otok = m - ob * p.qkv_tokens;
                        if (p.qkv_cls_last) otok = otok == 0 ? p.qkv_tokens - 1 : otok - 1;
                    }
                    roff = ((int64_t)ob * (p.qkv_hidden >> 6) * p.qkv_sp + otok) * 64;
                }
                float yall[FN / 2][8];
#pragma unroll
                for (int jp = 0; jp < FN / 2; ++jp) {
                    float (&y8)[8] = yall[jp];
#pragma unroll
                    for (int h = 0; h < 2; ++h) {
                        const int j = jp * 2 + h;
                        float* y = y8 + h * 4;
                        if (n0j[j] >= p.N) continue;
                        f32x4 bsum = brow ? *reinterpret_cast<const f32x4*>(brow + n0j[j]) : bj[j];
                        if (brow2) bsum += *reinterpret_cast<const f32x4*>(brow2 + n0j[j]);
#pragma unroll
                        for (int e = 0; e < 4; ++e) y[e] = acc[i][j][e] + bsum[e];
                        const bool res32 = p.res && p.res_dtype == BS_F32;
                        if (ACT == BS_ACT_GELU) {
                            const f32x2_ g0 = gelu_erf2(f32x2_{y[0], y[1]}), g1 = gelu_erf2(f32x2_{y[2], y[3]});
                            y[0] = g0[0]; y[1] = g0[1]; y[2] = g1[0]; y[3] = g1[1];
                        }
#pragma unroll
                        for (int e = 0; e < 4; ++e) {
                            if (ACT == BS_ACT_RELU) y[e] = fmaxf(y[e], 0.0f);
                            else if (ACT == BS_ACT_SOFTPLUS) y[e] = softplus20(y[e]);
                            else if (ACT == BS_ACT_SOFTPLUS_FAST) y[e] = softplus_fast(y[e]);
                            if (!res32) y[e] *= sj[j][e];
                        }
                        if (p.res) {
                            const int64_t ro = orow * p.ldr + n0j[j];
                            if (p.res_dtype == BS_F32) {
                                const f32x4 rr = *reinterpret_cast<const f32x4*>(reinterpret_cast<const float*>(p.res) + ro);
#pragma unroll
                                for (int e = 0; e < 4; ++e) y[e] = __builtin_fmaf(y[e], sj[j][e], rr[e]);
                            } else {
                                const typename T16<T>::v4 rr = *reinterpret_cast<const typename T16<T>::v4*>(reinterpret_cast<const T*>(p.res) + ro);
#pragma unroll
                                for (int e = 0; e < 4; ++e) y[e] += T16<T>::to_f32(rr[e]);
                                if (p.res_split_off > 0) {
                                    const typename T16<T>::v4 rl = *reinterpret_cast<const typename T16<T>::v4*>(reinterpret_cast<const T*>(p.res) + ro + p.res_split_off);
#pragma unroll
                                    for (int e = 0; e < 4; ++e) y[e] += T16<T>::to_f32(rl[e]);
                                } else if (F8 && p.res_f8) {
                                    add_lo8<T>(y, p.res, orow * p.ldr, p.N, n0j[j]);
                                }
                            }
                            if (p.res2) {
                                const typename T16<T>::v4 rr = *reinterpret_cast<const typename T16<T>::v4*>(reinterpret_cast<const T*>(p.res2) + ro);
#pragma unroll
                                for (int e = 0; e < 4; ++e) y[e] += T16<T>::to_f32(rr[e]);
                                if (p.res_split_off > 0) {
                                    const typename T16<T>::v4 rl = *reinterpret_cast<const typename T16<T>::v4*>(reinterpret_cast<const T*>(p.res2) + ro + p.res_split_off);
#pragma unroll
                                    for (int e = 0; e < 4; ++e) y[e] += T16<T>::to_f32(rl[e]);
                                } else if (F8 && p.res_f8) {
                                    add_lo8<T>(y, p.res2, orow * p.ldr, p.N, n0j[j]);
                                }
                            }
                        }
                    }
                }
#pragma unroll
                for (int jp = 0; jp < FN / 2; ++jp) {
                    float (&y8)[8] = yall[jp];
                    const int j0 = jp * 2, j1 = j0 + 1;
                    if (n0j[j0] >= p.N) continue;
                    void* dst = (p.out_mode == BS_OUT_QKV && which[j0] == 1) ? p.out2 : p.out;
                    const int so = p.out_mode != BS_OUT_QKV ? p.split_off : p.qkv_lo_off;
                    if (F8 && p.out_f8) {
                        const int nloc = p.out_mode == BS_OUT_SHUFFLE ? n0j[j0] % p.shuffle_cout : n0j[j0];
                        store8_f8<T>(dst, roff + coff[j0] - nloc, nloc, so, y8, p.out_f8 & 0xff, (p.out_f8 >> 8) & 0xff);
                    } else if (wide_ok && n0j[j1] < p.N && coff[j1] == coff[j0] + 4 && which[j1] == which[j0]) {
                        store8<T>(dst, roff + coff[j0], p.out_dtype, y8, so);
                    } else {
                        const float(&ya)[4] = *reinterpret_cast<const float(*)[4]>(y8);
                        store4<T>(dst, roff + coff[j0], p.out_dtype, ya, so);
                        if (n0j[j1] < p.N) {
                            const float(&yb)[4] = *reinterpret_cast<const float(*)[4]>(y8 + 4);
                            void* dst1 = (p.out_mode == BS_OUT_QKV && which[j1] == 1) ? p.out2 : p.out;
                            store4<T>(dst1, roff + coff[j1], p.out_dtype, yb, so);
                        }
                    }
                }
            }
        };
        const bool plain_full = p.out_mode == BS_OUT_PLAIN && !p.out_group_rows && p.bias && !p.bias_group_rows && p.N % BN == 0 &&
                                p.ldo % 8 == 0 && !b2_rows && !(p.ablate & 16);
        if (plain_full && p.act == BS_ACT_NONE && p.res && p.res_dtype == BS_F32 && !p.res2 && p.out_dtype == BS_F32 && p.split_off == 0 &&
            !(F8 && p.out_f8) && p.scale && p.ldr % 4 == 0) {
            BS_FRESH_LANE
            constexpr int NP = FM * (FN / 2), DEPTH = 8;
            const float* resp = reinterpret_cast<const float*>(p.res);
            float* outp = reinterpret_cast<float*>(p.out);
            f32x4 bj[FN], sj[FN];
#pragma unroll
            for (int j = 0; j < FN; ++j) {
                const int n0 = n_wave + (j >> 1) * 32 + fq * 8 + (j & 1) * 4;
                bj[j] = *reinterpret_cast<const f32x4*>(p.bias + n0);
                if (g2 >= 0) bj[j] += *reinterpret_cast<const f32x4*>(p.bias2 + (int64_t)g2 * p.N + n0);
                sj[j] = *reinterpret_cast<const f32x4*>(p.scale + n0);
            }
            const int mrow = m0 + wm * TM + frow;
            f32x4 rq[DEPTH][2];
            auto issue = [&](int it, int slot) {
                const int i = it / (FN / 2), jp = it - i * (FN / 2);
                int m = mrow + i * 16;
                m = m < p.M ? m : p.M - 1;
                const float* rp = resp + (int64_t)m * p.ldr + n_wave + jp * 32 + fq * 8;
                rq[slot][0] = *reinterpret_cast<const f32x4*>(rp);
                rq[slot][1] = *reinterpret_cast<const f32x4*>(rp + 4);
            };
#pragma unroll
            for (int it = 0; it < DEPTH; ++it) issue(it, it);
#pragma unroll
            for (int it = 0; it < NP; ++it) {
                const int i = it / (FN / 2), jp = it - i * (FN / 2);
                const int m = mrow + i * 16;
                f32x4 y0, y1;
#pragma unroll
                for (int e = 0; e < 4; ++e) {
                    y0[e] = __builtin_fmaf(acc[i][2 * jp][e] + bj[2 * jp][e], sj[2 * jp][e], rq[it % DEPTH][0][e]);
                    y1[e] = __builtin_fmaf(acc[i][2 * jp + 1][e] + bj[2 * jp + 1][e], sj[2 * jp + 1][e], rq[it % DEPTH][1][e]);
                }
                if (it + DEPTH < NP) issue(it + DEPTH, it % DEPTH);
                if (m < p.M) {
                    float* op = outp + (int64_t)m * p.ldo + n_wave + jp * 32 + fq * 8;
                    *reinterpret_cast<f32x4*>(op) = y0;
                    *reinterpret_cast<f32x4*>(op + 4) = y1;
                }
            }
            return;
        }
        if constexpr (F8) {
            if (p.out_mode == BS_OUT_PLAIN && !p.out_group_rows && !p.bias_group_rows && p.N % BN == 0 && p.ldo % 8 == 0 && !b2_rows &&
                !(p.ablate & (16 | 2048)) && p.out_f8 && !p.scale && (p.act == BS_ACT_NONE || p.act == BS_ACT_RELU) && p.split_off == p.N &&
                p.N % 8 == 0 && p.out_dtype != BS_F32 &&
                (!p.res || (p.res_f8 && p.res_dtype != BS_F32 && p.res_split_off == 0 && p.ldr % 8 == 0)) && (!p.res2 || p.res)) {
                BS_FRESH_LANE
                typedef typename T16<T>::v8 v8;
                typedef int i32x2 __attribute__((ext_vector_type(2)));
                typedef float f32x2 __attribute__((ext_vector_type(2)));
                constexpr int NP = FM * (FN / 2), RDEPTH = 4;
                f32x4 bj[FN];
#pragma unroll
                for (int j = 0; j < FN; ++j) {
                    const int n0 = n_wave + (j >> 1) * 32 + fq * 8 + (j & 1) * 4;
                    bj[j] = p.bias ? *reinterpret_cast<const f32x4*>(p.bias + n0) : f32x4{0.f, 0.f, 0.f, 0.f};
                    if (g2 >= 0) bj[j] += *reinterpret_cast<const f32x4*>(p.bias2 + (int64_t)g2 * p.N + n0);
                }
                const bool relu = p.act == BS_ACT_RELU;
                const int mrow = m0 + wm * TM + frow;
                const int ea = p.out_f8 & 0xff, el = (p.out_f8 >> 8) & 0xff;
                const bool lo_plane = !(p.out_lo8_rows > 0 && m0 >= p.out_lo8_rows);
                const bool hi_plane = !(p.out_planes_rows > 0 && m0 >= p.out_planes_rows);
                const float lsc = __builtin_ldexpf(1.0f, -BS_F8_ACT_LO_EXP);
                auto body = [&](auto nres_tag) {
                    constexpr int NRES = decltype(nres_tag)::value;
                    v8 rh[NRES ? RDEPTH : 1][NRES ? NRES : 1];
                    i32x2 rl[NRES ? RDEPTH : 1][NRES ? NRES : 1];
                    auto issue = [&](int it, int slot) {
                        const int i = it / (FN / 2), jp = it - i * (FN / 2);
                        int m = mrow + i * 16;
// ... 53 lines not shown
            }
            if (plain_full && p.act == BS_ACT_GELU && !p.res && p.out_f8 && !p.scale && p.split_off == p.N && p.N % 8 == 0) {
                BS_FRESH_LANE
                const bool lo = !(p.out_lo8_rows > 0 && m0 >= p.out_lo8_rows);
                const bool planes = !(p.out_planes_rows > 0 && m0 >= p.out_planes_rows);
                f32x4 bj[FN];
#pragma unroll
                for (int j = 0; j < FN; ++j) {
                    const int n0 = n_wave + (j >> 1) * 32 + fq * 8 + (j & 1) * 4;
                    bj[j] = *reinterpret_cast<const f32x4*>(p.bias + n0);
                    if (g2 >= 0) bj[j] += *reinterpret_cast<const f32x4*>(p.bias2 + (int64_t)g2 * p.N + n0);
                }
                if constexpr (TM == 128 && TN == 64 && LDS_BYTES >= WM * WN * 16384) {
                    if (!planes && m0 + BM <= p.M && !(p.ablate & 1024)) {
                        typedef unsigned u32x4_ __attribute__((ext_vector_type(4)));
                        __syncthreads();
                        char* sw = smem + wave * 16384;
                        const int s7 = frow & 7;
                        const int wb0 = frow * 128 + ((fq ^ s7) << 4), wb1 = frow * 128 + (((4 + fq) ^ s7) << 4);
                        const int rr = lane >> 3, pc = lane & 7;
                        const int rb = rr * 128 + ((pc ^ rr) << 4);
                        T* op = reinterpret_cast<T*>(p.out) + (int64_t)(m0 + wm * TM + rr) * p.ldo + n_wave + pc * 8;
                        const int64_t step = (int64_t)8 * p.ldo;
#pragma unroll
                        for (int ip = 0; ip < FM; ip += 2) {
                            char* sr = sw + ((ip >> 1) & 1) * 4096;
#pragma unroll
                            for (int ii = 0; ii < 2; ++ii) {
                                const int i = ip + ii;
#pragma unroll
                                for (int jp = 0; jp < FN / 2; ++jp) {
                                    typename T16<T>::v8 h8v;
#pragma unroll
                                    for (int h = 0; h < 2; ++h) {
                                        const f32x4 v = acc[i][2 * jp + h] + bj[2 * jp + h];
                                        const f32x2_ g0 = gelu_erf2(f32x2_{v[0], v[1]}), g1 = gelu_erf2(f32x2_{v[2], v[3]});
                                        h8v[4 * h] = T16<T>::from_f32(g0[0]); h8v[4 * h + 1] = T16<T>::from_f32(g0[1]);
                                        h8v[4 * h + 2] = T16<T>::from_f32(g1[0]); h8v[4 * h + 3] = T16<T>::from_f32(g1[1]);
                                    }
                                    *reinterpret_cast<typename T16<T>::v8*>(sr + (jp ? wb1 : wb0) + ii * 2048) = h8v;
                                }
                            }
                            __builtin_amdgcn_fence(__ATOMIC_RELEASE, "wavefront");
                            __builtin_amdgcn_wave_barrier();
#pragma unroll
                            for (int it = 0; it < 4; ++it) {
                                *reinterpret_cast<u32x4_*>(op) = *reinterpret_cast<const u32x4_*>(sr + rb + it * 1024);
                                op += step;
                            }
                        }
                        return;
                    }
                }
#pragma unroll
                for (int i = 0; i < FM; ++i) {
                    const int m = m0 + wm * TM + i * 16 + frow;
                    if (m >= p.M) continue;
#pragma unroll
                    for (int jp = 0; jp < FN / 2; ++jp) {
                        float y8[8];
#pragma unroll
                        for (int h = 0; h < 2; ++h) {
                            const f32x4 v = acc[i][2 * jp + h] + bj[2 * jp + h];
                            const f32x2_ g0 = gelu_erf2(f32x2_{v[0], v[1]}), g1 = gelu_erf2(f32x2_{v[2], v[3]});
                            y8[4 * h] = g0[0]; y8[4 * h + 1] = g0[1]; y8[4 * h + 2] = g1[0]; y8[4 * h + 3] = g1[1];
                        }
                        if (planes) {
                            store8_f8<T>(p.out, (int64_t)m * p.ldo, n_wave + jp * 32 + fq * 8, p.split_off, y8, p.out_f8 & 0xff, (p.out_f8 >> 8) & 0xff, lo);
                        } else {
                            typename T16<T>::v8 h;
#pragma unroll
                            for (int e = 0; e < 8; ++e) h[e] = T16<T>::from_f32(y8[e]);
                            *reinterpret_cast<typename T16<T>::v8*>(reinterpret_cast<T*>(p.out) + (int64_t)m * p.ldo + n_wave + jp * 32 + fq * 8) = h;
                        }
                    }
                }
                return;
            }
        }
        if (F8 && p.out_mode == BS_OUT_QKV && p.qkv_hidden % BN == 0 && p.act == BS_ACT_NONE && !p.res && p.bias && !p.bias_group_rows && !b2_rows &&
            p.out_dtype != BS_F32 && !(p.ablate & 16)) {
            BS_FRESH_LANE
            const int part = (tn * BN) / p.qkv_hidden;
            T* dst = reinterpret_cast<T*>(part == 1 ? p.out2 : p.out);
            const float qs = part == 0 ? p.q_scale : 1.0f;
            f32x4 bj[FN], sj[FN];
            int64_t coff[FN / 2];
#pragma unroll
            for (int j = 0; j < FN; ++j) {
                const int n0 = n_wave + (j >> 1) * 32 + fq * 8 + (j & 1) * 4;
                bj[j] = *reinterpret_cast<const f32x4*>(p.bias + n0);
                if (g2 >= 0) bj[j] += *reinterpret_cast<const f32x4*>(p.bias2 + (int64_t)g2 * p.N + n0);
                sj[j] = p.scale ? *reinterpret_cast<const f32x4*>(p.scale + n0) : f32x4{1.f, 1.f, 1.f, 1.f};
#pragma unroll
                for (int e = 0; e < 4; ++e) sj[j][e] *= qs;
                if (!(j & 1)) {
                    const int rem = n0 - part * p.qkv_hidden;
                    coff[j >> 1] = (int64_t)(rem >> 6) * p.qkv_sp * 64 + (rem & 63);
                }
            }
            const int nhead = p.qkv_hidden >> 6;
            const long long q_bytes = (long long)p.qkv_cls_rows * nhead * p.qkv_sp * 128;
            if (p.qkv_cls_rows > 0 && m0 >= p.qkv_patch_row0 && p.qkv_lo_off == 0 && !(p.ablate & (128 | 256)) && q_bytes < 0x7FFFFFF0ll) {
                typedef unsigned u32x4_ __attribute__((ext_vector_type(4)));
                const __amdgpu_buffer_rsrc_t orsrc = __builtin_amdgcn_make_buffer_rsrc(dst, 0, (int)q_bytes, 0x00020000);
                const int Tk = p.qkv_tokens - 1;
                int m = m0 + wm * TM + frow;
                const int mp0 = m - p.qkv_patch_row0;
                const int ob0 = mp0 / Tk;
                int otok = mp0 - ob0 * Tk;
                const unsigned img_bytes = (unsigned)(nhead * p.qkv_sp) * 128u;
                unsigned roff = (unsigned)ob0 * img_bytes + (unsigned)otok * 128u;
                if constexpr (TM == 128 && TN == 64 && LDS_BYTES >= WM * WN * 16384) {
                    if (m0 + BM <= p.M && Tk % 8 == 0 && (m0 - p.qkv_patch_row0) % 8 == 0 && !(p.ablate & 1024)) {
                        __syncthreads();
                        char* sw = smem + wave * 16384;
                        const int s7 = frow & 7;
                        const int wb0 = frow * 128 + ((fq ^ s7) << 4), wb1 = frow * 128 + (((4 + fq) ^ s7) << 4);
#pragma unroll
                        for (int i = 0; i < FM; ++i) {
#pragma unroll
                            for (int jp = 0; jp < FN / 2; ++jp) {
                                typename T16<T>::v8 v;
#pragma unroll
                                for (int e = 0; e < 4; ++e) {
                                    v[e] = T16<T>::from_f32((acc[i][2 * jp][e] + bj[2 * jp][e]) * sj[2 * jp][e]);
                                    v[4 + e] = T16<T>::from_f32((acc[i][2 * jp + 1][e] + bj[2 * jp + 1][e]) * sj[2 * jp + 1][e]);
                                }
                                *reinterpret_cast<typename T16<T>::v8*>(sw + (jp ? wb1 : wb0) + i * 2048) = v;
                            }
                        }
                        __builtin_amdgcn_fence(__ATOMIC_RELEASE, "wavefront");
                        __builtin_amdgcn_wave_barrier();
                        const int rr = lane >> 3, pc = lane & 7;
                        const int mpl = m0 + wm * TM + rr - p.qkv_patch_row0;
                        const int obl = mpl / Tk;
                        int tokl = mpl - obl * Tk;
                        const int rem0 = n_wave - part * p.qkv_hidden;
                        unsigned ro = (unsigned)obl * img_bytes + (unsigned)tokl * 128u + (unsigned)(rem0 >> 6) * (unsigned)p.qkv_sp * 128u + pc * 16u;
                        const int rb = rr * 128 + ((pc ^ rr) << 4);
#pragma unroll
                        for (int it = 0; it < 16; ++it) {
                            const u32x4_ x = *reinterpret_cast<const u32x4_*>(sw + rb + it * 1024);
                            __builtin_amdgcn_raw_buffer_store_b128(x, orsrc, ro, 0, 0);
                            tokl += 8;
                            ro += 8u * 128u;
                            if (tokl >= Tk) {
                                tokl -= Tk;
                                ro += img_bytes - (unsigned)Tk * 128u;
                            }
                        }
                        return;
                    }
                }
                unsigned cb[FN / 2];
#pragma unroll
                for (int jp = 0; jp < FN / 2; ++jp) cb[jp] = (unsigned)coff[jp] * 2u;
#pragma unroll
                for (int i = 0; i < FM; ++i) {
                    if (m < p.M) {
#pragma unroll
                        for (int jp = 0; jp < FN / 2; ++jp) {
                            typename T16<T>::v8 v;
#pragma unroll
                            for (int e = 0; e < 4; ++e) {
                                v[e] = T16<T>::from_f32((acc[i][2 * jp][e] + bj[2 * jp][e]) * sj[2 * jp][e]);
                                v[4 + e] = T16<T>::from_f32((acc[i][2 * jp + 1][e] + bj[2 * jp + 1][e]) * sj[2 * jp + 1][e]);
                            }
                            __builtin_amdgcn_raw_buffer_store_b128(__builtin_bit_cast(u32x4_, v), orsrc, roff + cb[jp], 0, 0);
                        }
                    }
                    m += 16;
                    otok += 16;
                    roff += 16u * 128u;
                    if (otok >= Tk) {
                        otok -= Tk;
// ... 208 lines not shown
```

bodyslam_amd/engine_export.py:

```python
from __future__ import annotations

import bisect
import ctypes as C
import struct
from typing import Dict, Iterable, List, Tuple

import torch

from . import _lib as L

MAGIC = b"BSENG02\0"
KIND_WORKSPACE, KIND_ZERO, KIND_DATA = 0, 1, 2
ARG_I64, ARG_F64, ARG_PTR, ARG_NULL, ARG_DESC = 0, 1, 2, 3, 4
OP_CALL = 0


def _tensors(obj, out: list):
    if isinstance(obj, torch.Tensor):
        if obj.is_cuda:
            out.append(obj)
    elif isinstance(obj, (tuple, list)):
        for o in obj:
            _tensors(o, out)
    elif isinstance(obj, dict):
        for o in obj.values():
            _tensors(o, out)


class _Buffers:

    def __init__(self, tensors: Iterable[torch.Tensor], workspace_ptrs: set):
        seen: Dict[int, torch.Tensor] = {}
        for t in tensors:
            st = t.untyped_storage()
            if st.data_ptr() not in seen:
                seen[st.data_ptr()] = t
        self.base = sorted(seen)
        self.size = [seen[b].untyped_storage().nbytes() for b in self.base]
        self.rep = [seen[b] for b in self.base]
        self.workspace = [b in workspace_ptrs for b in self.base]

    def locate(self, ptr: int, what: str) -> Tuple[int, int]:
        i = bisect.bisect_right(self.base, ptr) - 1
        if i < 0 or ptr >= self.base[i] + max(self.size[i], 1):
            raise ValueError(f"engine export: {what} points at device memory the plan does not keep alive ({ptr:#x})")
        return i, ptr - self.base[i]

    def bytes_of(self, i: int) -> torch.Tensor:
        st = self.rep[i].untyped_storage()
        return torch.empty(0, dtype=torch.uint8, device=self.rep[i].device).set_(st, 0, (st.nbytes(),)).cpu()


def _pack_name(s: str, n: int) -> bytes:
    b = s.encode()
    assert len(b) < n, s
    return b + b"\0" * (n - len(b))


def export_plan(plan: L.Plan, path: str, io: Dict[str, torch.Tensor], workspace: Iterable[torch.Tensor] = ()) -> dict:
    ts: List[torch.Tensor] = []
    _tensors(plan.keep, ts)
    _tensors(list(io.values()), ts)
    ws = list(workspace)
    _tensors(ws, ts)
    bufs = _Buffers(ts, {t.untyped_storage().data_ptr() for t in ws})
    io_ptrs = {t.untyped_storage().data_ptr() for t in io.values()}
    desc_of = {}
    gi = 0
    for i, (fn, args) in enumerate(plan.calls):
        if fn.__name__ == "bs_gemm":
            desc_of[i] = plan.keep_descs[gi]
            gi += 1
    ptr_fields = [(name, getattr(L.GemmDesc, name).offset) for name, ty in L.GemmDesc._fields_ if ty is C.c_void_p]

    calls = bytearray()
    n_ops = 0
    for i, (fn, args) in enumerate(plan.calls):
        name = fn.__name__
        sig = L._SIGS[name][:-1]
        assert len(sig) == len(args), (name, len(sig), len(args))
        calls += struct.pack("<II", OP_CALL, 0) + _pack_name(name, 48) + struct.pack("<I", len(args))
        for j, (ty, a) in enumerate(zip(sig, args)):
            if name == "bs_gemm":
                d = desc_of[i]
                raw = bytes(C.string_at(C.addressof(d), C.sizeof(d)))
                rel = []
                for fname, off in ptr_fields:
                    v = getattr(d, fname)
                    if v:
                        b, o = bufs.locate(int(v), f"{plan.names[i]}: bs_gemm_desc.{fname}")
                        rel.append((off, b, o))
                calls += struct.pack("<II", ARG_DESC, len(raw)) + raw + struct.pack("<I", len(rel))
                for off, b, o in rel:
                    calls += struct.pack("<IIq", off, b, o)
# ... 84 lines not shown
```

bodyslam_amd/zoedepth.py:

```python
from __future__ import annotations

import math
import os
import warnings
import dataclasses
from dataclasses import dataclass
from typing import Dict, Optional, Sequence, Tuple

import numpy as np
import torch
import torch.nn.functional as F

from . import _lib as L
from .calibration import DEFAULT_POLICY, NECK_RELHEAD_WONLY, CalibrationPolicy, Scope, choose, finish_report, saving_gflop, worst

LOG2E = 1.4426950408889634


@dataclass
class ZoeConfig:
    hidden: int = 1024
    layers: int = 24
    heads: int = 16
    intermediate: int = 4096
    taps: Tuple[int, ...] = (6, 12, 18, 24)
    image_size: int = 384
    patch: int = 16
    ln_eps: float = 1e-12
    neck_hidden: Tuple[int, ...] = (256, 512, 1024, 1024)
    fusion: int = 256
    rel_features: int = 32
    bottleneck: int = 256
    bin_dim: int = 128
    n_attractors: int = 16
    n_bins: int = 64
    min_temp: float = 0.0212
    max_temp: float = 50.0
    pt_layers: int = 4
    pt_hidden: int = 128
    pt_inter: int = 1024
    pt_heads: int = 4
    head_names: Tuple[str, ...] = ("nyu", "kitti")
    add_projection: bool = True
    level_attractors: Tuple[int, ...] = (16, 8, 4, 1)

    @property
    def single_head(self) -> bool:
        return len(self.head_names) == 1

    @property
    def seed_mlp(self) -> int:
        return 256 if self.single_head else self.bin_dim // 2

    @property
    def proj_mlp(self) -> int:
        return 128 if self.single_head else self.bin_dim // 2

    @property
    def clb_hidden(self) -> int:
        return (self.rel_features + 1 + self.bin_dim) // 2 if self.single_head else (self.rel_features + self.bin_dim) // 4

    def attractors_at(self, level: int) -> int:
        return self.level_attractors[level] if self.single_head else self.n_attractors


BACKBONE_CLASSES = ("qkv", "o", "fc1", "fc2")
ACCURATE_CLASS_MODES = "auto"
AUTO_CANDIDATES = DEFAULT_POLICY.candidates
AUTO_TOL_CLASS_M = DEFAULT_POLICY.tol_class
AUTO_TOL_TOTAL_M = DEFAULT_POLICY.tol_total
AUTO_TOL_ABS_M = DEFAULT_POLICY.tol_abs
TOLERANCE_M = DEFAULT_POLICY.tolerance_m
ACCURATE_ATTN_MODE = "auto"
AUTO_ATTN_RATE_FACTOR = DEFAULT_POLICY.attn_rate_factor
AUTO_NECK_CANDIDATES = DEFAULT_POLICY.neck_candidates
AUTO_TOL_NECK_ABS_M = DEFAULT_POLICY.tol_neck_abs
AUTO_NECK_SITE_MIN_SHARE = DEFAULT_POLICY.neck_site_min_share
AUTO_NECK_SMALL_GROUPS = dict(DEFAULT_POLICY.neck_small_groups)
AUTO_NECK_PLAIN_MIN_SHARE = DEFAULT_POLICY.neck_plain_min_share
AUTO_TOL_NECK_PLAIN_ABS_M = DEFAULT_POLICY.tol_neck_plain_abs
AUTO_NECK_WONLY_INCREMENT_M = DEFAULT_POLICY.neck_wonly_increment
AUTO_NECK_PLAIN_INCREMENT_M = DEFAULT_POLICY.neck_plain_increment
AUTO_TOL_NECK_CAP_M = DEFAULT_POLICY.tol_neck_cap
AUTO_CAL_FRAMES = DEFAULT_POLICY.cal_frames
AUTO_HOLDOUT_FRAMES = DEFAULT_POLICY.holdout_frames
AUTO_TOL_HOLDOUT_M = DEFAULT_POLICY.tol_holdout
AUTO_CAL_SEEDS = DEFAULT_POLICY.cal_seeds
AUTO_HOLDOUT_SEEDS = DEFAULT_POLICY.holdout_seeds
ACCURATE_NECK_MODE = "full"

_CALIBRATION_CACHE: Dict[Tuple, dict] = {}
_ARITHMETIC_SWITCHES = ("BS_UPCONV_FUSED", "BS_NECK_PLAIN", "BS_MLP2", "BS_NECK_BIAS_CORR", "BS_PROJECTOR_LEVEL", "BS_AUTO_WSTAT")

ZOED_NK = ZoeConfig()
ZOED_N = ZoeConfig(head_names=("nyu",))
ZOED_K = ZoeConfig(head_names=("kitti",))


def pad_sizes(h: int, w: int) -> Tuple[int, int]:
    return int(np.sqrt(h / 2) * 3), int(np.sqrt(w / 2) * 3)


def net_size(h: int, w: int, out_hw=(384, 512), multiple: int = 32) -> Tuple[int, int]:
    ph, pw = pad_sizes(h, w)
    hp, wp = h + 2 * ph, w + 2 * pw
    sh, sw = out_hw[0] / hp, out_hw[1] / wp
    if abs(1 - sw) < abs(1 - sh):
        sh = sw
    else:
        sw = sh
    return int(np.round(sh * hp / multiple) * multiple), int(np.round(sw * wp / multiple) * multiple)


def _relative_position_index(wh: int, ww: int) -> torch.Tensor:
    nrd = (2 * wh - 1) * (2 * ww - 1) + 3
    coords = torch.stack(torch.meshgrid(torch.arange(wh), torch.arange(ww), indexing="ij")).flatten(1)
    rel = (coords[:, :, None] - coords[:, None, :]).permute(1, 2, 0).contiguous()
    rel[:, :, 0] += wh - 1
    rel[:, :, 1] += ww - 1
    rel[:, :, 0] *= 2 * ww - 1
    idx = torch.zeros((wh * ww + 1,) * 2, dtype=rel.dtype)
    idx[1:, 1:] = rel.sum(-1)
    idx[0, 0:] = nrd - 3
    idx[0:, 0] = nrd - 2
    idx[0, 0] = nrd - 1
    return idx


class _Measurement:

    def __init__(self, eng: "ZoeDepthEngine", frames_u8: torch.Tensor):
        self.eng, self.frames, self.hold = eng, frames_u8, None
        self.ncal, self.H, self.W = int(frames_u8.shape[0]), int(frames_u8.shape[1]), int(frames_u8.shape[2])
        self.site_flops: Dict[str, float] = {}
        self.ref = self.truth = self.truth_hold = None

    def depth(self, modes, neck, attn, holdout=False, means=None):
        frames = self.hold if holdout else self.frames
        self.eng.set_class_modes(modes, neck, attn)
        plan = _ZoePlan(self.eng, int(frames.shape[0]), self.H, self.W, True)
        plan.frames.copy_(frames)
        plan.run(None if means is None else {"__site_means__": means})
        d = plan.depth_m.clone()
        torch.cuda.synchronize(self.eng.dev)
        self.site_flops.update(plan.site_flops)
        del plan
        return d

    def set_site_bias_corr(self, means):
        e = self.eng
        e.site_bias_corr = {k_[3:]: (e.dw_sum[k_[3:]].double() * m_.double()).sum(1).float().contiguous() for k_, m_ in means.items() if k_[3:] in e.dw_sum}
        e._bias_corr_cache.clear()
        return sorted(e.site_bias_corr)

class ZoeDepthEngine:

    def __init__(self, weights: Dict[str, torch.Tensor], cfg: Optional[ZoeConfig] = None, dtype=torch.float16,
                 device: int = 0, target_hw: Tuple[int, int] = (384, 512), precision: str = "fast",
                 class_modes: Optional[Dict[str, str]] = None, neck_mode: Optional[str] = None, attn_mode: Optional[str] = None):
        L.init(device)
        assert precision in ("fast", "accurate", "reference")
        if precision == "reference":
            class_modes, neck_mode, attn_mode = "pairs", "pairs", "corr"
        self.precision = precision
        self.acc = precision != "fast"
        self._sd = weights if self.acc else None
        self.target_hw = target_hw
        self.cfg = cfg or ZoeConfig()
        assert dtype in (torch.float16, torch.bfloat16)
        self.dtype = dtype
        self.dev = torch.device("cuda", device)
        self.w: Dict[str, torch.Tensor] = {}
        self._bias_cache: Dict[Tuple[int, int], list] = {}
        self._plans: Dict[Tuple, "_ZoePlan"] = {}
        self._raw_tables = []
        self.f8s: Dict[str, Tuple[int, int]] = {}
        cm = class_modes if class_modes is not None else (os.environ.get("BS_ACCURATE_CLASS_MODE") or ACCURATE_CLASS_MODES)
        if isinstance(cm, str) and cm != "auto":
            cm = {k: cm for k in BACKBONE_CLASSES}
        self.auto_classes = self.acc and isinstance(cm, str)
        self.auto_modes = self.auto_classes
        self.calibration: Optional[dict] = None
        self.class_modes = {k: "full" for k in BACKBONE_CLASSES}
        if isinstance(cm, dict):
            self.class_modes.update(cm)
        assert all(v in ("full", "w", "wcls", "wmean", "wstat", "a", "single", "pairs") for v in self.class_modes.values()), self.class_modes
        am_ = attn_mode or os.environ.get("BS_ATTN_MODE") or (ACCURATE_ATTN_MODE if self.acc else "single")
        assert am_ in ("auto", "single", "corr"), am_
        assert self.acc or am_ != "corr", "attn_mode='corr' belongs to precision='accurate'"
        self.auto_attn = am_ == "auto"
        self.attn_mode = "corr" if am_ == "auto" else am_
        self.auto_modes = self.auto_modes or (self.acc and self.auto_attn)
        self.single_keys = set()
        self.wmode: Dict[str, str] = {}
        self.dw_sum: Dict[str, torch.Tensor] = {}
        self.backbone_bias_corr: Dict[str, torch.Tensor] = {}
        self.site_bias_corr: Dict[str, torch.Tensor] = {}
        self._bias_corr_cache: Dict[str, torch.Tensor] = {}
        self.neck_mode = neck_mode or os.environ.get("BS_NECK_MODE") or ACCURATE_NECK_MODE
        self.fuse_mlp = int(os.environ.get("BS_MLP2", "2"))
        c_ = self.cfg
        self.neck_f8 = self.acc and self.neck_mode != "pairs" and all(v % 128 == 0 for v in (c_.hidden, c_.fusion, c_.fusion // 2, *c_.neck_hidden))
        with torch.no_grad():
            self._ingest(weights)

    def _h(self, t: torch.Tensor) -> torch.Tensor:
        return t.to(self.dev, dtype=self.dtype).contiguous()

    def _f(self, t: torch.Tensor) -> torch.Tensor:
        return t.to(self.dev, dtype=torch.float32).contiguous()

    def _conv_w(self, t: torch.Tensor) -> torch.Tensor:
        return self._h(L.conv_weight(t.permute(0, 2, 3, 1)))

    def _split(self, t: torch.Tensor):
        hi = t.to(self.dtype)
        lo = (t - hi.float()).to(self.dtype)
        return hi, lo

    def _w8(self, key: str, t: torch.Tensor) -> torch.Tensor:
        if not self.acc:
            return self._h(t)
        mode = self.class_modes.get(key.split(".")[-2], "full") if key[0] == "l" else "full"
        if mode == "single":
            self.single_keys.add(key)
            return self._h(t)
        if mode == "pairs":
            return self._wn(t)
        if t.shape[1] % 128 != 0:
            return self._wn(t)
        if mode == "w" and t.shape[1] % 256 != 0:
            mode = "full"
        w8, sb = L.f8_weight(t, self.dtype, planes={"full": "both", "wcls": "both", "wmean": "both", "wstat": "both", "w": "lo", "a": "hi_only"}[mode], device=self.dev)
        self.f8s[key] = sb
        self.wmode[key] = mode
        if key[0] == "l" and mode in ("full", "wcls", "wmean", "wstat"):
            td = t.to(self.dev)
            self.w[key + ".lo"] = (td - td.to(self.dtype).float()).to(torch.bfloat16).contiguous()
        return w8.to(self.dev)

    def mode_of(self, wkey: str) -> Optional[str]:
        m = self.wmode.get(wkey)
        if m in ("full", "wcls", "wmean", "wstat") and wkey[0] == "l":
            return self.class_modes.get(wkey.split(".")[-2], m)
        return m

    def neck_site_wonly(self, wkey: str) -> bool:
        nm = self.neck_mode
        if wkey.endswith("w_cls") or nm in ("full", "pairs"):
            return False
        if nm == "w":
            return True
        if nm.startswith("wonly:"):
            return any(wkey in part.split(":", 1)[1].split(",") for part in nm.split(";") if ":" in part)
        return not any(wkey.startswith(p_) for p_ in nm.split(","))

    def neck_site_plain(self, wkey: str) -> bool:
        nm = self.neck_mode
        if not nm.startswith("wonly:") or wkey.endswith("w_cls") or wkey == "rh.conv2.w":
            return False
        return any(part.startswith("plain:") and wkey in part[6:].split(",") for part in nm.split(";"))

    def set_class_modes(self, modes: Dict[str, str], neck_mode: Optional[str] = None, attn_mode: Optional[str] = None) -> None:
        for k, v in modes.items():
            assert k in BACKBONE_CLASSES and v in ("full", "wcls", "wmean", "wstat"), (k, v)
            assert self.class_modes[k] in ("full", "wcls", "wmean", "wstat"), f"class {k} was ingested as {self.class_modes[k]!r}: not switchable"
        self.class_modes.update(modes)
        if neck_mode is not None:
            assert (neck_mode == "pairs") == (self.neck_mode == "pairs"), "the neck's operand format is fixed at ingestion"
            self.neck_mode = neck_mode
        if attn_mode is not None:
            assert attn_mode in ("single", "corr") and (self.acc or attn_mode == "single")
            self.attn_mode = attn_mode
        self._plans.clear()

    def apply_calibration(self, report: dict) -> None:
        self.set_class_modes({k: v for k, v in report["class_modes"].items() if self.class_modes[k] in ("full", "wcls", "wmean", "wstat")},
                             report["neck_mode"], report.get("attn_mode"))
        self.backbone_bias_corr = {k: torch.tensor(v, dtype=torch.float32, device=self.dev).view(1, -1)
                                   for k, v in (report.get("backbone_bias_corr") or {}).items()}
        self.site_bias_corr = {k: torch.tensor(v, dtype=torch.float32, device=self.dev) for k, v in (report.get("site_bias_corr") or {}).items()}
        self._bias_corr_cache.clear()
        self.calibration = dict(report)
# ... 329 lines not shown
        key = (B, H, W, flip)
        if key not in self._plans:
            self._plans[key] = _ZoePlan(self, B, H, W, flip)
        return self._plans[key]

    def infer(self, frames_u8: torch.Tensor, flip_aug: bool = True, taps: Optional[dict] = None, want_u16: bool = True,
              graph: bool = False):
        assert frames_u8.dtype == torch.uint8 and frames_u8.is_cuda and frames_u8.dim() == 4 and frames_u8.shape[-1] == 3
        B, H, W, _ = frames_u8.shape
        if B == 0:
            return (torch.empty(0, H, W, device=self.dev), torch.empty(0, H, W, device=self.dev, dtype=torch.int16))
        plan = self.plan_for(B, H, W, flip_aug)
        plan.frames.copy_(frames_u8)
        if graph and taps is None:
            plan.plan.capture()
        plan.run(taps)
        return plan.depth_m, plan.depth_u16


class _Pool:

    def __init__(self, dev):
        self.dev = dev
        self.free_blocks = []
        self.blocks = []
        self.owner = {}
        self.bytes_new = 0

    def alloc(self, shape, dtype):
        n = 1
        for d in shape:
            n *= int(d)
        nbytes = max(n * torch.empty((), dtype=dtype).element_size(), 16)
        fits = [b for b in self.free_blocks if b.numel() >= nbytes]
        if fits:
            blk = min(fits, key=lambda b: b.numel())
            self.free_blocks = [b for b in self.free_blocks if b is not blk]
        else:
            blk = torch.empty((nbytes + 255) // 256 * 256, dtype=torch.uint8, device=self.dev)
            self.bytes_new += blk.numel()
            self.blocks.append(blk)
        t = blk[:nbytes].view(dtype).view(*shape)
        self.owner[t.data_ptr()] = blk
        return t

    def free(self, *tensors):
        for t in tensors:
            blk = self.owner.pop(t.data_ptr(), None) if t is not None else None
            if blk is not None:
                self.free_blocks.append(blk)


class _ZoePlan:

    MEAN_STEP = 8
    F8O = (L.F8_ACT_HI_EXP, L.F8_ACT_LO_EXP)

    def __init__(self, eng: ZoeDepthEngine, B: int, H: int, W: int, flip: bool):
        self.eng, self.c, self.w = eng, eng.cfg, eng.w
        c = eng.cfg
        self.B, self.H, self.W, self.flip = B, H, W, flip
        self.NB = NB = 2 * B if flip else B
        self.nh, self.nw = nh_, nw_ = net_size(H, W, eng.target_hw)
        self.hp, self.wp = hp, wp = nh_ // c.patch, nw_ // c.patch
        self.T0 = T0 = hp * wp
        self.S = S = T0 + 1
        self.Sp = Sp = (S + 63) // 64 * 64
        self.geom = dict(B=B, NB=NB, H=H, W=W, nh=nh_, nw=nw_, hp=hp, wp=wp, S=S, Sp=Sp)
        self.site_flops: Dict[str, float] = {}
        self.plan = L.Plan(eng.dev)
        self.pool = _Pool(eng.dev)
        self.use_tab = wp == 32 and hp <= 40
        self.grouped = grouped = self.use_tab
        self.CP = CP = (NB + 255) // 256 * 256 if grouped else 0
        self.MT = CP + NB * T0 if grouped else NB * S
        self.TOK = ("tokens_grouped" if grouped else "tokens", NB, S, c.hidden, CP)
        self.acc = acc = eng.acc
        self.m2 = 2 if acc else 1
        self.np3 = 3 if acc else 1
        self.nf8 = nf8 = eng.neck_f8
        self.NSP = (32 if nf8 else 16) if acc else 0
        self.RZ = 1 | ((4 if nf8 else 2) if acc else 0)
        self.attn_corr = bool(acc and eng.attn_mode == "corr" and self.use_tab and hp % 2 == 0)

        x = self._embed()
        taps16 = self._backbone(x)
        feats, fshape = self._reassemble(taps16)
        bins, emb = self._bins_seed(feats[3], *fshape[3])
        fused, pj_low = self._fusion(feats, fshape)
        last = self._relative_head(*fused[3])
        levels = self._levels_fused if self._projector_level_fits(fused, pj_low) else self._levels_four
        bins, Eh, ph_, pw_ = levels(fused, pj_low, bins, emb, *fshape[3])
        self._depth(last, Eh, bins, ph_, pw_)

    def e16(self, *s):
        return self.pool.alloc(s, self.eng.dtype)

    def e32(self, *s):
        return self.pool.alloc(s, torch.float32)

    def fmt(self, *wkeys):
        if not self.acc or all(k_ in self.eng.single_keys for k_ in wkeys):
            return 0
        return 32 if all(k_ in self.eng.f8s for k_ in wkeys) else 16

    def am(self, wkey):
        return 2 if self.fmt(wkey) else 1

    def prow(self, wkey):
        return (self.CP << 8) if (self.acc and self.grouped and self.fmt(wkey) == 32 and self.eng.mode_of(wkey) in ("wmean", "wstat")) else 0

    def mfmt(self):
        return (2 if self.nf8 else 1) if self.acc else 0

    def f8_scales(self, wkey, lo_plane=True):
        sb0, sb1 = self.eng.f8s[wkey]
        if not lo_plane:
            return (127 - L.F8_ACT_HI_EXP, sb0, 127 - L.F8_ACT_HI_EXP, sb0)
        return (127 - L.F8_ACT_HI_EXP, sb0, 127 - L.F8_ACT_LO_EXP, sb1)

    def f8kw(self, wkey):
        return dict(f8_scales=self.f8_scales(wkey), f8_wonly_from=-1 if self.eng.neck_site_wonly(wkey) else 0,
                    f8_skip_from=-1 if self.eng.neck_site_plain(wkey) else 0)

    def okw(self, Cout, out_pairs, out8):
        if not (self.acc and out_pairs):
            return dict(ldo=Cout, out_split_off=0)
        return dict(ldo=Cout * self.m2, out_split_off=Cout, out_f8=self.F8O if (self.nf8 and out8) else None)

    def lo8_rows(self, *consumer_wkeys):
        return 256 if (self.acc and self.nf8 and all(k_ in self.eng.f8s and self.eng.neck_site_wonly(k_) for k_ in consumer_wkeys)) else 0

    def hi8_rows(self, *consumer_wkeys):
        return 256 if (self.acc and self.nf8 and all(k_ in self.eng.f8s and self.eng.neck_site_plain(k_) for k_ in consumer_wkeys)) else 0

    def bgemm(self, name, A, wkey, out, M, N, K, **kw):
        eng, P, w, acc, grouped, CP, NB, T0 = self.eng, self.plan, self.w, self.acc, self.grouped, self.CP, self.NB, self.T0
        f8s, mode = eng.f8s, eng.mode_of(wkey)

        def f8gemm(f8_seg, scales, **f8):
            P.gemm(name, A, w[wkey], out, M=M, N=N, K=K, lda=2 * K, f8_seg=f8_seg, f8_scales=scales, precision_passes=1, **f8, **kw)

        if acc and grouped and wkey in f8s and wkey[0] == "l":
            P.mark("in:" + wkey, A, ("chanmean", CP * 2 * K, NB * T0, 2 * K, K))
        if acc and wkey in eng.single_keys:
            P.gemm(name, A, w[wkey], out, M=M, N=N, K=K, lda=K, precision_passes=1, **kw)
        elif acc and wkey in f8s and mode == "w":
            f8gemm(K, self.f8_scales(wkey, lo_plane=False))
        elif acc and wkey in f8s and mode == "wstat" and grouped and wkey in eng.backbone_bias_corr:
            f8gemm(2 * K, self.f8_scales(wkey), f8_skip_from=CP, bias2=(eng.backbone_bias_corr[wkey], CP, NB * T0))
        elif acc and wkey in f8s and mode in ("wmean", "wstat") and grouped:
            abar = self.pool.alloc((NB, K), torch.bfloat16)
            b2 = self.e32(NB, N)
            P.add(name + ".cm", "bs_col_mean", A, 2 * K, CP, T0, NB, self.MEAN_STEP, K, abar, b2, NB * N, L.dt(A))
            P.add(name + ".r1", "bs_rank1_bias", abar, w[wkey + ".lo"], b2, NB, N, K)
            f8gemm(2 * K, self.f8_scales(wkey), f8_skip_from=CP, bias2=(b2, CP, T0))
            self.pool.free(abar, b2)
        elif acc and wkey in f8s:
            wonly = CP if (mode == "wcls" and grouped) else 0
            f8gemm(2 * K, self.f8_scales(wkey), f8_wonly_from=wonly)
        else:
            P.gemm(name, A, w[wkey], out, M=M, N=N, K=K * self.np3, lda=K * self.m2, seg1=K if acc else 0, precision_passes=self.np3, **kw)

    def nplain(self, name, A, wkey, out, M, N, K, shuffle=None, out_pairs=True, **kw):
        eng, P, w, acc = self.eng, self.plan, self.w, self.acc
        out8 = kw.pop("out8", True)
        ok = self.okw(shuffle[1] if shuffle else N, out_pairs, out8)
        if "ldo" in kw:
            ok["ldo"] = kw.pop("ldo")
        if "split_off" in kw:
            ok["out_split_off"] = kw.pop("split_off")
        if not out_pairs:
            ok = dict(ldo=ok["ldo"], out_split_off=0)
        if acc and wkey in eng.f8s:
            self.site_flops[wkey] = self.site_flops.get(wkey, 0.0) + 2.0 * M * N * K
            lda_ = kw.pop("lda", 2 * K)
            P.mark("in:" + wkey, A, ("chanmean", kw.get("a_offset", 0), M, lda_, K))
            if not kw.get("bias_group_rows"):
                kw["bias"] = eng.site_bias(wkey, kw.get("bias"))
            P.gemm(name, A, w[wkey], out, M=M, N=N, K=K, lda=lda_, f8_seg=2 * K, shuffle=shuffle,
                   precision_passes=1, **ok, **self.f8kw(wkey), **kw)
        else:
            ok.pop("out_f8", None)
            P.gemm(name, A, w[wkey], out, M=M, N=N, K=K * self.np3, lda=kw.pop("lda", K * self.m2), seg1=K if acc else 0,
                   shuffle=shuffle, precision_passes=self.np3, **ok, **kw)

    def nconv(self, name, A, wkey, out, hh, ww, Ci, Co, stride=1, **kw):
        eng, P, w, acc, NB, m2, np3 = self.eng, self.plan, self.w, self.acc, self.NB, self.m2, self.np3
        use8 = acc and wkey in eng.f8s
        g_ = L.conv_geom(hh, ww, Ci if use8 else Ci * m2, 3, 3, stride, 1)
        ho, wo = g_[3], g_[4]
        has_res = "res" in kw
        if use8:
            self.site_flops[wkey] = self.site_flops.get(wkey, 0.0) + 2.0 * NB * ho * wo * Co * 9 * Ci
            P.mark("in:" + wkey, A, ("chanmean", 0, NB * hh * ww, 2 * Ci, Ci))
            kw["bias"] = eng.site_bias(wkey, kw.get("bias"))
            P.gemm(name, A, w[wkey], out, M=NB * ho * wo, N=Co, K=9 * Ci, lda=2 * Ci, conv=g_, f8_seg=2 * Ci, ldo=2 * Co,
                   ldr=2 * Co if has_res else 0, res_f8=has_res, out_split_off=Co, out_f8=self.F8O, precision_passes=1, **self.f8kw(wkey), **kw)
        else:
            if has_res and acc:
                kw["res_split_off"] = Co
            P.gemm(name, A, w[wkey], out, M=NB * ho * wo, N=Co, K=9 * Ci * np3, lda=Ci * m2, conv=g_, seg1=Ci if acc else 0,
                   ldo=Co * m2, ldr=Co * m2 if has_res else 0, out_split_off=Co if acc else 0, precision_passes=np3, **kw)
        return ho, wo

    def _embed(self):
        c, w, P, NB, T0, S, CP, dev = self.c, self.w, self.plan, self.NB, self.T0, self.S, self.CP, self.eng.dev
        B, H, W, Hd = self.B, self.H, self.W, c.hidden
        PK = 3 * c.patch * c.patch
        self.frames = torch.empty(B, H, W, 3, device=dev, dtype=torch.uint8)
        patches = self.e16(NB * T0, PK * self.m2)
        x = torch.zeros(self.MT, Hd, device=dev, dtype=torch.float32)
        P.add("preprocess", "bs_preprocess_patches", self.frames, patches, B, H, W, self.nh, self.nw, int(self.flip), L.dt(patches) | self.fmt("pe.w"))
        if self.grouped:
            P.add("cls", "bs_fill_rows", x, w["cls"], NB, 1, Hd)
            self.bgemm("patch_embed", patches, "pe.w", x, NB * T0, Hd, PK, bias=w["pe.b"], out_group=(NB * T0, 0, CP))
        else:
            P.add("cls", "bs_fill_rows", x, w["cls"], NB, S, Hd)
            self.bgemm("patch_embed", patches, "pe.w", x, NB * T0, Hd, PK, bias=w["pe.b"], out_group=(T0, S, 1))
        self.pool.free(patches)
        P.mark("embed", x, self.TOK)
        return x

    def _backbone(self, x):
        c, w, P, eng, NB, S, Sp, CP, MT, hp, wp = self.c, self.w, self.plan, self.eng, self.NB, self.S, self.Sp, self.CP, self.MT, self.hp, self.wp
        acc, grouped, use_tab, corr, m2, Hd = self.acc, self.grouped, self.use_tab, self.attn_corr, self.m2, c.hidden
        fmt, prow, bgemm = self.fmt, self.prow, self.bgemm
        z16 = lambda *s: torch.zeros(*s, device=eng.dev, dtype=eng.dtype)
        bias = eng._rel_table(hp, wp) if use_tab else eng._rel_bias(hp, wp, Sp)
        xn = z16(MT, Hd * m2)
        QN = NB * c.heads * Sp * 64
        q, k, vt = z16((2 if corr else 1) * NB, c.heads, Sp, 64), z16((2 if corr else 1) * NB, c.heads, Sp, 64), z16((2 if corr else 1) * NB, c.heads, 64, Sp)
        ao = z16(MT, Hd * m2)
        hid = z16(MT, c.intermediate * m2)
        taps16 = [z16(MT, Hd * m2) for _ in c.taps]
        ti = 0
        for l in range(c.layers):
            P.add(f"l{l}.ln1", "bs_layernorm", x, w[f"l{l}.ln1.g"], w[f"l{l}.ln1.b"], xn, None, MT, Hd, c.ln_eps,
                  L.dt(xn) | fmt(f"l{l}.qkv.w") | prow(f"l{l}.qkv.w"))
            bgemm(f"l{l}.qkv", xn, f"l{l}.qkv.w", q, MT, 3 * Hd, Hd, bias=w[f"l{l}.qkv.b"],
                  qkv=(Hd, S, Sp, LOG2E / math.sqrt(64.0), k, vt, use_tab, NB if grouped else 0, CP, QN if corr else 0))
            if corr:
                P.add(f"l{l}.attn", "bs_attention_table_corr", q, k, vt, q.view(-1)[QN:], k.view(-1)[QN:], vt.view(-1)[QN:], bias[l], ao, NB,
                      c.heads, hp, wp, Sp, CP, L.dt(q) | fmt(f"l{l}.o.w") | (64 if prow(f"l{l}.o.w") else 0))
            elif use_tab:
                P.add(f"l{l}.attn", "bs_attention_table", q, k, vt, bias[l], ao, NB, c.heads, hp, wp, Sp, CP,
                      L.dt(q) | fmt(f"l{l}.o.w") | (64 if prow(f"l{l}.o.w") else 0))
            else:
                P.add(f"l{l}.attn", "bs_attention", q, k, vt, bias[l], ao, NB, c.heads, S, Sp, L.dt(q) | fmt(f"l{l}.o.w"))
            bgemm(f"l{l}.o", ao, f"l{l}.o.w", x, MT, Hd, Hd, bias=w[f"l{l}.o.b"], scale=w[f"l{l}.lam1"], res=x, ldr=Hd)
            P.add(f"l{l}.ln2", "bs_layernorm", x, w[f"l{l}.ln2.g"], w[f"l{l}.ln2.b"], xn, None, MT, Hd, c.ln_eps,
                  L.dt(xn) | fmt(f"l{l}.fc1.w") | prow(f"l{l}.fc1.w"))
            hfmt = fmt(f"l{l}.fc2.w")
            bgemm(f"l{l}.fc1", xn, f"l{l}.fc1.w", hid, MT, c.intermediate, Hd, bias=w[f"l{l}.fc1.b"], act=L.ACT_GELU,
                  ldo=c.intermediate * self.am(f"l{l}.fc2.w"), out_split_off=c.intermediate if hfmt else 0,
                  out_f8=self.F8O if hfmt == 32 else None,
                  out_lo8_rows=CP if (hfmt == 32 and grouped and eng.mode_of(f"l{l}.fc2.w") in ("wcls", "wmean", "wstat")) else 0,
                  out_planes_rows=CP if prow(f"l{l}.fc2.w") else 0)
            bgemm(f"l{l}.fc2", hid, f"l{l}.fc2.w", x, MT, Hd, c.intermediate, bias=w[f"l{l}.fc2.b"], scale=w[f"l{l}.lam2"], res=x, ldr=Hd)
            P.mark(f"layer{l + 1}", x, self.TOK)
            if (l + 1) in c.taps:
                if acc:
                    P.add(f"tap{ti}", "bs_cast_split", x, taps16[ti], MT, Hd, L.dt(xn) | (32 if eng.neck_f8 else 0))
                else:
                    P.add(f"tap{ti}", "bs_cast", x, taps16[ti], x.numel(), L.dt(xn))
                ti += 1
        return taps16

    def _reassemble(self, taps16):
        c, w, P, eng, NB, T0, S, CP, hp, wp = self.c, self.w, self.plan, self.eng, self.NB, self.T0, self.S, self.CP, self.hp, self.wp
        acc, grouped, m2, np3, nf8, Hd = self.acc, self.grouped, self.m2, self.np3, self.nf8, c.hidden
        e16, free, nplain, nconv = self.e16, self.pool.free, self.nplain, self.nconv
        feats, fshape = [], []
        cb = self.e32(NB, Hd)
        r16 = e16(NB * T0, Hd * m2)
        for i, ch in enumerate(c.neck_hidden):
            t16 = taps16[i]
            nplain(f"ro{i}.cls", t16, f"ro{i}.w_cls", cb, NB, Hd, Hd, out_pairs=False, lda=(1 if grouped else S) * Hd * m2,
                   bias=eng.site_bias(f"ro{i}.w_tok", w[f"ro{i}.b"]))
            if grouped:
                nplain(f"ro{i}.tok", t16, f"ro{i}.w_tok", r16, NB * T0, Hd, Hd, a_offset=CP * Hd * m2, bias=cb, bias_group_rows=T0,
                       act=L.ACT_GELU)
            elif acc and f"ro{i}.w_tok" in eng.f8s:
                P.gemm(f"ro{i}.tok", t16, w[f"ro{i}.w_tok"], r16, M=NB * T0, N=Hd, K=Hd, lda=2 * Hd, conv=(1, S, Hd, 1, T0, 1, 1, 1, 0, -1),
                       f8_seg=2 * Hd, bias=cb, bias_group_rows=T0, act=L.ACT_GELU, ldo=2 * Hd, out_split_off=Hd, out_f8=self.F8O if nf8 else None,
                       precision_passes=1, **self.f8kw(f"ro{i}.w_tok"))
            else:
                P.gemm(f"ro{i}.tok", t16, w[f"ro{i}.w_tok"], r16, M=NB * T0, N=Hd, K=Hd * np3, lda=Hd * m2, conv=(1, S, Hd * m2, 1, T0, 1, 1, 1, 0, -1),
                       seg1=Hd if acc else 0, bias=cb, bias_group_rows=T0, act=L.ACT_GELU, ldo=Hd * m2, out_split_off=Hd if acc else 0,
                       precision_passes=np3)
            pr = e16(NB * T0, ch * m2)
            nplain(f"ra{i}.proj", r16, f"ra{i}.proj.w", pr, NB * T0, ch, Hd, bias=w[f"ra{i}.proj.b"])
            if i == 0 or i == 1:
                s_ = 4 if i == 0 else 2
                up = e16(NB, hp * s_, wp * s_, ch * m2)
                nplain(f"ra{i}.up", pr, f"ra{i}.up.w", up, NB * T0, s_ * s_ * ch, ch, shuffle=(s_, ch, hp, wp), bias=w[f"ra{i}.up.b"])
                free(pr)
                fh, fw, src = hp * s_, wp * s_, up
            elif i == 2:
                fh, fw, src = hp, wp, pr
            else:
                fh, fw = (hp + 2 - 3) // 2 + 1, (wp + 2 - 3) // 2 + 1
                src = e16(NB, fh, fw, ch * m2)
                nconv(f"ra{i}.down", pr, f"ra{i}.down.w", src, hp, wp, ch, ch, stride=2, bias=w[f"ra{i}.down.b"])
                free(pr)
            P.mark(f"reassemble{i}", src, ("nhwc", NB, fh, fw, ch, self.mfmt()))
            f16_ = e16(NB, fh, fw, c.fusion * m2)
            nconv(f"nc{i}", src, f"nc{i}.w", f16_, fh, fw, ch, c.fusion)
            free(src)
            P.mark(f"neckconv{i}", f16_, ("nhwc", NB, fh, fw, c.fusion, self.mfmt()))
            feats.append(f16_)
            fshape.append((fh, fw))
        free(r16, cb)
        return feats, fshape

    def _bins_seed(self, bott, bh_, bw_):
        c, w, P, NB, acc, m2, np3, dev = self.c, self.w, self.plan, self.NB, self.acc, self.m2, self.np3, self.eng.dev
        e16, e32 = self.e16, self.e32
        Mb = NB * bh_ * bw_
        xb = e16(Mb, c.bottleneck * m2)
        self.nplain("mh.conv2", bott, "mh.conv2.w", xb, Mb, c.bottleneck, c.bottleneck, bias=w["mh.conv2.b"], out8=False)
        self.logits = torch.empty(NB, 4, device=dev, dtype=torch.float32)
        self.route = torch.zeros(NB, dtype=torch.int32, device=dev)
        if not c.single_head:
            self._router(xb, bh_, bw_)
        E, nb, SM, PM, KB = c.bin_dim, c.n_bins, c.seed_mlp, c.proj_mlp, c.bottleneck
        sh = e16(Mb, 2 * SM * m2)
        P.gemm("seed.c1", xb, w["seed.c1.w"], sh, M=Mb, N=2 * SM, K=KB * np3, lda=KB * m2, seg1=KB if acc else 0, bias=w["seed.c1.b"], act=L.ACT_RELU,
               ldo=2 * SM * m2, out_split_off=2 * SM if acc else 0, precision_passes=np3)
        bins = e32(NB, bh_, bw_, 2 * nb)
# ... 237 lines not shown
```

include/bodyslam_hip.h:

```cpp
#ifndef BODYSLAM_HIP_H
#define BODYSLAM_HIP_H

#include <stdint.h>

#ifdef __cplusplus
extern "C" {
#endif

typedef enum {
    BS_OK = 0,
    BS_ERR_INVALID = -1,
    BS_ERR_HIP = -2,
    BS_ERR_NOT_INIT = -3
} bs_status;

enum { BS_F32 = 0, BS_F16 = 1, BS_BF16 = 2, BS_F64 = 3  };
enum { BS_ACT_NONE = 0, BS_ACT_RELU = 1, BS_ACT_GELU = 2, BS_ACT_SOFTPLUS = 3, BS_ACT_SOFTPLUS_FAST = 4 };
enum { BS_OUT_PLAIN = 0, BS_OUT_SHUFFLE = 1, BS_OUT_QKV = 2 };

int bs_init(int device);
const char* bs_last_error(void);
int bs_version(void);

#define BS_F8_ACT_HI_EXP 0
#define BS_F8_ACT_LO_EXP 11
typedef struct bs_gemm_desc {
    const void* A;
    const void* W;
    int32_t dtype;
    int32_t M, N, K;
    int32_t lda;
    int32_t conv;
    int32_t Hin, Win, Cin, Hout, Wout, KH, KW, stride, pad_h, pad_w;
    int32_t relu_a;
    const float* bias;
    int32_t bias_group_rows;
    int32_t act;
    const float* scale;
    const void* res;
    int32_t res_dtype;
    int32_t ldr;
    const void* res2;
    void* out;
    void* out2;
    void* out3;
    int32_t out_dtype;
    int32_t ldo;
    int32_t out_mode;
    int32_t out_group_rows, out_group_stride, out_row_offset;
    int32_t shuffle_s, shuffle_cout;
    int32_t qkv_hidden, qkv_tokens, qkv_sp;
    float q_scale;
    int32_t tile;
    int32_t seg1;
    int32_t out_split_off;
    int32_t res_split_off;
    int32_t f8_seg;
    uint32_t f8_scales;
    int32_t out_f8;
    int32_t res_f8;
    int32_t qkv_cls_last;
    int32_t qkv_cls_rows;
    int32_t qkv_patch_row0;
    int32_t f8_wonly_from;
    int32_t out_lo8_rows;
    int32_t f8_skip_from;
    int32_t bias2_row0;
    int32_t bias2_group_rows;
    int32_t out_planes_rows;
    const float* bias2;
    int32_t qkv_lo_off;
    int32_t out2_relu;
} bs_gemm_desc;
int bs_gemm(const bs_gemm_desc* d, void* stream);
int bs_gemm_tile(const bs_gemm_desc* d);

int bs_col_mean(const void* A, int64_t lda, int32_t row0, int32_t rows_per_group, int32_t groups, int32_t row_step, int32_t K,
                void* out_bf16, float* zero_out, int64_t zero_n, int32_t dtype, void* stream);
int bs_rank1_bias(const void* abar_bf16, const void* dw_bf16, float* out, int32_t G, int32_t N, int32_t K, void* stream);

int bs_attention(const void* q, const void* k, const void* vt, const float* bias, void* out,
                 int32_t B, int32_t nh, int32_t S, int32_t Sp, int32_t dtype, void* stream);
int bs_attention_table(const void* q, const void* k, const void* vt, const float* table, void* out,
                       int32_t B, int32_t nh, int32_t hp, int32_t wp, int32_t Sp, int32_t grouped, int32_t dtype, void* stream);
int bs_attention_table_corr(const void* q, const void* k, const void* vt, const void* q_lo, const void* k_lo, const void* vt_lo,
                            const float* table, void* out, int32_t B, int32_t nh, int32_t hp, int32_t wp, int32_t Sp, int32_t grouped,
                            int32_t dtype, void* stream);

int bs_layernorm(const float* x, const float* gamma, const float* beta, void* out16, float* out32, int32_t rows,
                 int32_t cols, float eps, int32_t dtype, void* stream);

int bs_copy_f32(const float* src, float* dst, int64_t n, void* stream);

int bs_cast_split(const float* x, void* out, int64_t rows, int32_t cols, int32_t out_dtype, void* stream);
int bs_relu_split(const void* x, void* out, int64_t rows, int32_t cols, int32_t dtype, void* stream);

int bs_cast(const float* x, void* out, int64_t n, int32_t out_dtype, void* stream);

int bs_preprocess_patches(const uint8_t* frames, void* out, int32_t B, int32_t H, int32_t W, int32_t nh,
                          int32_t nw, int32_t flip, int32_t out_dtype, void* stream);
int bs_preprocess_image(const uint8_t* frames, float* out, int32_t B, int32_t H, int32_t W, int32_t nh,
                        int32_t nw, int32_t flip, void* stream);

int bs_fill_rows(float* x, const float* v, int32_t B, int32_t rows_per_image, int32_t cols, void* stream);

int bs_resize_bilinear_nhwc(const void* x, void* out, int32_t B, int32_t Hin, int32_t Win, int32_t C,
                            int32_t Hout, int32_t Wout, int32_t align_corners, int32_t dtype, void* stream);

int bs_resize_bias_relu_nhwc(const void* x, const float* bias, void* out, int32_t B, int32_t Hin, int32_t Win, int32_t C, int32_t Hout,
                             int32_t Wout, int32_t flags, int32_t dtype, void* stream);

int bs_upconv_tapsum(const float* y, const float* bias, void* out, int32_t B, int32_t Hin, int32_t Win, int32_t Cout,
                     int32_t Hout, int32_t Wout, int32_t align_corners, int32_t relu, int32_t dtype, void* stream);

int bs_upconv_fused(const void* x, const void* w, const float* bias, void* out, int32_t B, int32_t Hin, int32_t Win, int32_t Cin,
                    int32_t Cout, int32_t Hout, int32_t Wout, int32_t flags, int32_t relu, int32_t mode, int32_t sa0, int32_t sb0,
                    int32_t sa1, int32_t sb1, int32_t dtype, void* stream);

int bs_attractor_step(const float* A, const float* bins_prev, float* bins_out, const int32_t* route, int32_t B,
                      int32_t Hp, int32_t Wp, int32_t H, int32_t W, int32_t groups, int32_t n_bins, int32_t n_attr,
                      void* stream);
int bs_mlp2(const void* x, int32_t ldx, const void* W1, const float* b1, const void* W2, const float* b2, float* out, int32_t M,
            int32_t K1, int32_t N1, int32_t N2, int32_t act2, int32_t dtype, void* stream);
int bs_mlp2_add(const void* emb, const void* prev, const void* W1, const float* b1, const void* W2, const float* b2, float* out,
                int32_t B, int32_t Hp, int32_t Wp, int32_t H, int32_t W, int32_t K1, int32_t N1, int32_t N2, int32_t act2, int32_t dtype,
                void* stream);
int bs_projector_level(const void* z, const float* b_c1, const void* emb_prev, const void* Wc2, const float* b_c2, const void* We,
                       const float* b_e, void* x_out, void* emb_out, float* eh_out, int32_t B, int32_t Hl, int32_t Wl, int32_t H, int32_t W,
                       int32_t PM, int32_t E, int32_t NE, int32_t dtype, void* stream);
int bs_add_resized(const void* x, const void* prev, void* out, int32_t B, int32_t Hp, int32_t Wp, int32_t H,
                   int32_t W, int32_t C, int32_t dtype, void* stream);
int bs_logbinom_depth(const void* last, const float* Eh, const float* bins, const float* w0_last, const float* w2,
                      const float* b2, const int32_t* route, float* depth, int32_t B, int32_t H, int32_t W,
                      int32_t He, int32_t We, float min_temp, float max_temp, int32_t dtype, void* stream);
int bs_logbinom_depth_ex(const void* last, const float* Eh, const float* bins, const float* w0_last, const float* w2,
                         const float* b2, const float* rel_w, int32_t hid, const int32_t* route, float* depth, int32_t B,
                         int32_t H, int32_t W, int32_t He, int32_t We, float min_temp, float max_temp, int32_t dtype,
                         void* stream);
int bs_small_attention(const float* qkv, void* out, int32_t B, int32_t S, int32_t nheads, int32_t dtype, void* stream);
int bs_route_argmax(const float* logits, int32_t ld, int32_t* route, int32_t B, void* stream);

int bs_postprocess_depth(const float* depth_net, float* depth_m, uint16_t* depth_u16, int32_t B, int32_t H,
                         int32_t W, int32_t nh, int32_t nw, int32_t flip, void* stream);

int bs_cyclepose_im2col(const uint8_t* frames, const int32_t* pairs, void* out, int32_t P, int32_t H, int32_t W,
                        int32_t dtype, void* stream);
int bs_cyclepose_im2col_window(const uint8_t* frames, const int32_t* pairs, void* out, int32_t P, int32_t H, int32_t W,
                               int32_t top, int32_t left, int32_t CH, int32_t CW, int32_t dtype, void* stream);
int bs_instnorm_relu_nhwc(const float* x, void* out, float* out_f32, float* scratch, int32_t P, int32_t HW, int32_t C,
                          float eps, int32_t dtype, void* stream);
int bs_avgpool_nhwc(const float* x, float* out, int32_t P, int32_t HW, int32_t C, void* stream);
int bs_cyclepose_head(const float* pooled, const float* x2, const float* w_skip_pool, const float* w_skip_x2,
                      const float* b_skip, const float* w1, const float* b1, const float* w2, const float* b2,
                      float* pose7, float* T, float* scratch , int32_t P,
                      int32_t HW, int32_t C, void* stream);
// ... 243 lines not shown
```

Before: 495.7.

## Store V in row-major token layout and read transposed fragments via ds_read_tr16

The QKV GEMM epilogue now writes V in the same token-major row layout as Q and K, with no transposed scatter, when the new v_rows flag is set. The table attention kernels then stage V rows through LDS with a swizzle and use ds_read_tr16_b64 transposed LDS reads to build the MFMA fragments. The CLS query pass also stages V through LDS instead of doing strided global loads. This removes the transposed-store cost in the GEMM epilogue and makes V loads contiguous, at the price of extra LDS traffic, waitcnt barriers and a bumped engine format version.

```diff
diff --git a/bodyslam_amd/_lib.py b/bodyslam_amd/_lib.py
--- a/bodyslam_amd/_lib.py
+++ b/bodyslam_amd/_lib.py
@@ -41,7 +41,7 @@
         ("qkv_cls_last", C.c_int32), ("qkv_cls_rows", C.c_int32), ("qkv_patch_row0", C.c_int32), ("f8_wonly_from", C.c_int32), ("out_lo8_rows", C.c_int32),
         ("f8_skip_from", C.c_int32), ("bias2_row0", C.c_int32), ("bias2_group_rows", C.c_int32), ("out_planes_rows", C.c_int32),
         ("bias2", C.c_void_p),
-        ("qkv_lo_off", C.c_int32), ("out2_relu", C.c_int32),
+        ("qkv_lo_off", C.c_int32), ("out2_relu", C.c_int32), ("qkv_v_rows", C.c_int32),
     ]
 
 
@@ -296,6 +296,7 @@
         d.qkv_cls_rows = int(qkv[7]) if len(qkv) > 7 else 0
         d.qkv_patch_row0 = int(qkv[8]) if len(qkv) > 8 else d.qkv_cls_rows
         d.qkv_lo_off = int(qkv[9]) if len(qkv) > 9 else 0
+        d.qkv_v_rows = int(bool(qkv[10])) if len(qkv) > 10 else 0
         d.qkv_hidden, d.qkv_tokens, d.qkv_sp, d.q_scale = hidden, tokens, sp, q_scale
         d.out2 = out_k.data_ptr()
         d.out3 = out_vt.data_ptr()
@@ -535,14 +536,14 @@
     check(load_library().bs_attention(p(q), p(k), p(vt), p(bias), p(out), B, nh, S, Sp, dt(q) | split, stream_ptr()), "bs_attention")
 
 
-def attention_table(q, k, vt, table, out, B, nh, hp, wp, Sp, split=0, grouped=0):
-    check(load_library().bs_attention_table(p(q), p(k), p(vt), p(table), p(out), B, nh, hp, wp, Sp, int(grouped), dt(q) | split, stream_ptr()),
-          "bs_attention_table")
-
-
-def attention_table_corr(q, k, vt, q_lo, k_lo, vt_lo, table, out, B, nh, hp, wp, Sp, split=0, grouped=0):
+def attention_table(q, k, vt, table, out, B, nh, hp, wp, Sp, split=0, grouped=0, v_rows=False):
+    check(load_library().bs_attention_table(p(q), p(k), p(vt), p(table), p(out), B, nh, hp, wp, Sp, int(grouped),
+                                            dt(q) | split | (128 if v_rows else 0), stream_ptr()), "bs_attention_table")
+
+
+def attention_table_corr(q, k, vt, q_lo, k_lo, vt_lo, table, out, B, nh, hp, wp, Sp, split=0, grouped=0, v_rows=False):
     check(load_library().bs_attention_table_corr(p(q), p(k), p(vt), p(q_lo), p(k_lo), p(vt_lo), p(table), p(out), B, nh, hp, wp, Sp, int(grouped),
-                                                 dt(q) | split, stream_ptr()), "bs_attention_table_corr")
+                                                 dt(q) | split | (128 if v_rows else 0), stream_ptr()), "bs_attention_table_corr")
 
 
 def layernorm(x, gamma, beta, out16, out32, rows, cols, eps, dtype=F16):
diff --git a/bodyslam_amd/csrc/attention.hip b/bodyslam_amd/csrc/attention.hip
--- a/bodyslam_amd/csrc/attention.hip
+++ b/bodyslam_amd/csrc/attention.hip
@@ -465,15 +465,32 @@
                       grouped ? (int64_t)b : (int64_t)b * S, S, q0, active, lane, cls_planes);
 }
 
-template <typename T, int QW, bool CORR>
+__device__ __forceinline__ int vr_swz(int key) { return (key & 2) << 1; }
+__device__ __forceinline__ int vr_lane_base(int lane) {
+    const int i = lane & 15, q = i >> 2, p = i & 3, g1 = (lane >> 4) & 1, h2 = lane >> 5;
+    return (h2 * 8 + q) * 128 + (((2 * g1 + (p >> 1)) ^ vr_swz(q)) << 4) + 8 * (p & 1);
+}
+template <typename T>
+__device__ __forceinline__ typename T16<T>::v8 vr_frag(const char* p) {
+    typedef short s16x4_ __attribute__((ext_vector_type(4)));
+    typedef short s16x8_ __attribute__((ext_vector_type(8)));
+    typedef __attribute__((address_space(3))) s16x4_ lds_s16x4_;
+    const s16x4_ a = __builtin_amdgcn_ds_read_tr16_b64_v4i16((lds_s16x4_*)p);
+    const s16x4_ b = __builtin_amdgcn_ds_read_tr16_b64_v4i16((lds_s16x4_*)(p + 512));
+    const s16x8_ ab = __builtin_shufflevector(a, b, 0, 1, 2, 3, 4, 5, 6, 7);
+    return __builtin_bit_cast(typename T16<T>::v8, ab);
+}
+
+template <typename T, int QW, bool CORR, bool VR>
 __device__ __forceinline__ void cls_query_pass(const T* __restrict__ Qg, const T* __restrict__ Kg, const T* __restrict__ Vg, const T* __restrict__ Qlg,
                                                const T* __restrict__ Klg, const T* __restrict__ Vlg, int Sp, int hp, const float* __restrict__ tail3,
                                                char* area, int wave, int lane, T* __restrict__ out, int split, int nh, int head, int64_t row0,
-                                               int64_t row_cls, int S, bool cls_planes) {
+                                               int64_t row_cls, int S, bool cls_planes, char* vstage) {
     typedef typename T16<T>::v8 v8;
     const int r = lane & 31, h2 = lane >> 5;
     const int kap = (r & ~12) | ((r & 4) << 1) | ((r & 8) >> 1);
     const int q0 = hp * 32;
+    const int vb0 = vr_lane_base(lane);
     constexpr float THR = 6.0f;
     const float b_cp = tail3[0], b_cc = tail3[2];
     v8 qf[4], qlf[CORR ? 4 : 1];
@@ -503,14 +520,24 @@
 #pragma unroll 1
     for (int ky = wave; ky <= hp; ky += QW) {
         v8 vf[4], vfl[CORR ? 4 : 1];
-#pragma unroll
-        for (int dh = 0; dh < 2; ++dh)
-#pragma unroll
-            for (int s2 = 0; s2 < 2; ++s2) {
-                const int64_t voff = (int64_t)(dh * 32 + r) * Sp + ky * 32 + (2 * s2 + h2) * 8;
-                vf[dh * 2 + s2] = *reinterpret_cast<const v8*>(Vg + voff);
-                if constexpr (CORR) vfl[dh * 2 + s2] = *reinterpret_cast<const v8*>(Vlg + voff);
-            }
+        if constexpr (VR) {
+            asm volatile("s_waitcnt lgkmcnt(0)" ::: "memory");
+#pragma unroll
+            for (int i = 0; i < (CORR ? 8 : 4); ++i) {
+                const int row = (i & 3) * 8 + (lane >> 3);
+                const int cs8 = ((lane & 7) ^ vr_swz(row)) * 8;
+                glds16((CORR && i >= 4 ? Vlg : Vg) + (int64_t)(ky * 32 + row) * 64 + cs8, vstage + i * 1024);
+            }
+        } else {
+#pragma unroll
+            for (int dh = 0; dh < 2; ++dh)
+#pragma unroll
+                for (int s2 = 0; s2 < 2; ++s2) {
+                    const int64_t voff = (int64_t)(dh * 32 + r) * Sp + ky * 32 + (2 * s2 + h2) * 8;
+                    vf[dh * 2 + s2] = *reinterpret_cast<const v8*>(Vg + voff);
+                    if constexpr (CORR) vfl[dh * 2 + s2] = *reinterpret_cast<const v8*>(Vlg + voff);
+                }
+        }
         v8 kn[4], knl[CORR ? 4 : 1];
         const int kyn = ky + QW <= hp ? ky + QW : ky;
         load_k(kyn, kn, knl);
@@ -555,6 +582,17 @@
                 if constexpr (CORR) pfl[s2][e] = T16<T>::from_f32(pv - T16<T>::to_f32(pf[s2][e]));
             }
         l_run += psum;
+        if constexpr (VR) {
+            asm volatile("s_waitcnt vmcnt(0)" ::: "memory");
+#pragma unroll
+            for (int dh = 0; dh < 2; ++dh)
+#pragma unroll
+                for (int s2 = 0; s2 < 2; ++s2) {
+                    const char* fp = vstage + s2 * 2048 + (vb0 ^ (dh << 6));
+                    vf[dh * 2 + s2] = vr_frag<T>(fp);
+                    if constexpr (CORR) vfl[dh * 2 + s2] = vr_frag<T>(fp + 4096);
+                }
+        }
 #pragma unroll
         for (int dh = 0; dh < 2; ++dh)
 #pragma unroll
@@ -610,7 +648,7 @@
     store_out_tile<T>(area, oacc, 1.0f / L, out, split, nh, head, row0, row_cls, S, q0, true, lane, cls_planes);
 }
 
-template <typename T, int QW, int WPE, bool CORR, bool PK = false, bool CLS2 = false>
+template <typename T, int QW, int WPE, bool CORR, bool PK = false, bool CLS2 = false, bool VR = false>
 __global__ __launch_bounds__(QW * 64, WPE) void attention_tab2_kernel(const T* __restrict__ Q, const T* __restrict__ K, const T* __restrict__ Vt,
                                                                   const T* __restrict__ Ql, const T* __restrict__ Kl, const T* __restrict__ Vtl,
                                                                   const float* __restrict__ table, T* __restrict__ out, int split, int B, int nh,
@@ -620,6 +658,7 @@
     const int abl = split >> 3;
     split &= 3;
     typedef typename T16<T>::v8 v8;
+    static_assert(!(CLS2 && VR) || QW <= 8, "cls_query_pass stages V rows through a quarter stage per wave: at most 8 waves");
     constexpr int HALF = 16 * 1024;
     constexpr int STAGE = CORR ? 2 * HALF : HALF;
     constexpr int WP = 32, RW = 2 * WP - 1;
@@ -672,7 +711,9 @@
             const int cs8 = ((lane & 7) ^ ((row >> 1) & 7)) * 8;
             const T* kb = (CORR && i >= 16) ? Klg : Kg;
             const T* vb = (CORR && i >= 16) ? Vlg : Vg;
-            const T* src = j < 8 ? kb + (int64_t)(kt * 64 + row) * 64 + cs8 : vb + (int64_t)row * Sp + kt * 64 + cs8;
+            const T* src;
+            if constexpr (VR) src = j < 8 ? kb + (int64_t)(kt * 64 + row) * 64 + cs8 : vb + (int64_t)(kt * 64 + row) * 64 + ((lane & 7) ^ vr_swz(row)) * 8;
+            else src = j < 8 ? kb + (int64_t)(kt * 64 + row) * 64 + cs8 : vb + (int64_t)row * Sp + kt * 64 + cs8;
             glds16(src, sb + i * 1024);
         }
     };
@@ -687,6 +728,7 @@
     bool first = true;
     const int kap = (r & ~12) | ((r & 4) << 1) | ((r & 8) >> 1);
     constexpr float THR = 6.0f;
+    const int vb0 = vr_lane_base(lane);
 
     const int nbody = ntab - 3;
     const float* lt = cls_tile ? creg : tab + (nbody - RW - (qt + hp - 1) * RW) + (31 - r + 8 * h2);
@@ -766,12 +808,16 @@
 #pragma unroll
             for (int s2 = 0; s2 < 2; ++s2) {
                 const int chunk = sub * 4 + 2 * s2 + h2;
-                const int off = drow * 128 + ((chunk ^ ((drow >> 1) & 7)) << 4);
-                const v8 vf = *reinterpret_cast<const v8*>(sv + off);
+                const int off = VR ? sub * 4096 + s2 * 2048 + (vb0 ^ (dh << 6)) : drow * 128 + ((chunk ^ ((drow >> 1) & 7)) << 4);
+                v8 vf;
+                if constexpr (VR) vf = vr_frag<T>(sv + off);
+                else vf = *reinterpret_cast<const v8*>(sv + off);
                 oacc[dh] = T16<T>::mfma32(vf, pf[s2], oacc[dh]);
                 if constexpr (CORR) {
                     oacc[dh] = T16<T>::mfma32(vf, pfl[s2], oacc[dh]);
-                    const v8 vfl = *reinterpret_cast<const v8*>(sv + HALF + off);
+                    v8 vfl;
+                    if constexpr (VR) vfl = vr_frag<T>(sv + HALF + off);
+                    else vfl = *reinterpret_cast<const v8*>(sv + HALF + off);
                     oacc[dh] = T16<T>::mfma32(vfl, pf[s2], oacc[dh]);
                 }
             }
@@ -825,15 +871,15 @@
     if constexpr (CLS2) {
         if (qblk == 0) {
             __syncthreads();
-            cls_query_pass<T, QW, CORR>(Qg, Kg, Vg, CORR ? Ql + bh * Sp * 64 : nullptr, Klg, Vlg, Sp, hp, table + (int64_t)head * ntab + ntab - 3,
-                                        smem + 2 * STAGE + (ntab_pad + 64) * 4, wave, lane, out, split, nh, head,
-                                        grouped ? (int64_t)grouped + (int64_t)b * (S - 1) : (int64_t)b * S + 1, grouped ? (int64_t)b : (int64_t)b * S, S,
-                                        cls_planes);
-        }
-    }
-}
-
-template <typename T>
+            cls_query_pass<T, QW, CORR, VR>(Qg, Kg, Vg, CORR ? Ql + bh * Sp * 64 : nullptr, Klg, Vlg, Sp, hp, table + (int64_t)head * ntab + ntab - 3,
+                                            smem + 2 * STAGE + (ntab_pad + 64) * 4, wave, lane, out, split, nh, head,
+                                            grouped ? (int64_t)grouped + (int64_t)b * (S - 1) : (int64_t)b * S + 1, grouped ? (int64_t)b : (int64_t)b * S, S,
+                                            cls_planes, smem + wave * (STAGE / 4));
+        }
+    }
+}
+
+template <typename T, bool VR>
 static int launch_attn_tab(const void* q, const void* k, const void* vt, const void* ql, const void* kl, const void* vtl, const float* table, void* out,
                            int split, int B, int nh, int hp, int Sp, int grouped, hipStream_t st) {
     constexpr int QW = 5;
@@ -842,7 +888,7 @@
     if (ql) {
         static const bool cls2_ok = diag_env("BS_ATTN_NO_CLS2") == nullptr;
         if (cls2_ok && hp % 8 == 0) {
-            auto kb = attention_tab2_kernel<T, 8, 2, true, false, true>;
+            auto kb = attention_tab2_kernel<T, 8, 2, true, false, true, VR>;
             BS_MAX_DYNAMIC_LDS(reinterpret_cast<const void*>(kb), 96 * 1024);
             hipLaunchKernelGGL(kb, dim3(B * nh * (hp / 8)), dim3(8 * 64), 64 * 1024 + tab_bytes + 8192, st, (const T*)q, (const T*)k, (const T*)vt,
                                (const T*)ql, (const T*)kl, (const T*)vtl, table, (T*)out, split, B, nh, hp, Sp, hp / 8, ntab, grouped);
@@ -853,7 +899,7 @@
             const int nb8 = cdiv(nqt, 8), qw8 = cdiv(nqt, nb8);
 #define BS_ATTN_CORR_BIG(QWB)                                                                                                                \
     do {                                                                                                                                     \
-        auto kb = attention_tab2_kernel<T, QWB, 2, true>;                                                                                    \
+        auto kb = attention_tab2_kernel<T, QWB, 2, true, false, false, VR>;                                                                  \
         BS_MAX_DYNAMIC_LDS(reinterpret_cast<const void*>(kb), 96 * 1024); \
         hipLaunchKernelGGL(kb, dim3(B * nh * nb8), dim3(QWB * 64), 64 * 1024 + tab_bytes, st, (const T*)q, (const T*)k, (const T*)vt,        \
                            (const T*)ql, (const T*)kl, (const T*)vtl, table, (T*)out, split, B, nh, hp, Sp, nb8, ntab, grouped);             \
@@ -864,7 +910,7 @@
             if (qw8 == 8) BS_ATTN_CORR_BIG(8);
 #undef BS_ATTN_CORR_BIG
         }
-        auto kc = attention_tab2_kernel<T, QW, 2, true>;
+        auto kc = attention_tab2_kernel<T, QW, 2, true, false, false, VR>;
         BS_MAX_DYNAMIC_LDS(reinterpret_cast<const void*>(kc), 88 * 1024);
         hipLaunchKernelGGL(kc, dim3(B * nh * nqb), dim3(QW * 64), 64 * 1024 + tab_bytes, st, (const T*)q, (const T*)k, (const T*)vt, (const T*)ql,
                            (const T*)kl, (const T*)vtl, table, (T*)out, split, B, nh, hp, Sp, nqb, ntab, grouped);
@@ -878,13 +924,18 @@
     static const bool pipelined_ok = diag_env("BS_ATTN_NO_PIPE") == nullptr;
     if (hp % 2 == 0 && pipelined_ok) {
         static const bool wpe3 = diag_env("BS_ATTN_WPE3") != nullptr, pk = diag_env("BS_ATTN_NO_PK") == nullptr;
-        auto kern2 = wpe3 ? (pk ? attention_tab2_kernel<T, QW, 3, false, true> : attention_tab2_kernel<T, QW, 3, false>)
-                          : (pk ? attention_tab2_kernel<T, QW, 4, false, true> : attention_tab2_kernel<T, QW, 4, false>);
+        auto kern2 = attention_tab2_kernel<T, QW, 4, false, true, false, VR>;
+        if constexpr (VR) {
+            if (wpe3 || !pk) { set_error("bs_attention_table: the V-rows mode is not built for the BS_ATTN_WPE3 / BS_ATTN_NO_PK variants"); return BS_ERR_INVALID; }
+        } else {
+            kern2 = wpe3 ? (pk ? attention_tab2_kernel<T, QW, 3, false, true> : attention_tab2_kernel<T, QW, 3, false>)
+                         : (pk ? attention_tab2_kernel<T, QW, 4, false, true> : attention_tab2_kernel<T, QW, 4, false>);
+        }
         BS_MAX_DYNAMIC_LDS(reinterpret_cast<const void*>(kern2), 64 * 1024);
         static const int abl = diag_env("BS_ATTN_ABL") ? atoi(diag_env("BS_ATTN_ABL")) : 0;
         static const bool cls2_ok = diag_env("BS_ATTN_NO_CLS2") == nullptr;
         if (!wpe3 && pk && abl == 0 && cls2_ok && hp % 8 == 0) {
-            auto kb = attention_tab2_kernel<T, 8, 4, false, true, true>;
+            auto kb = attention_tab2_kernel<T, 8, 4, false, true, true, VR>;
             BS_MAX_DYNAMIC_LDS(reinterpret_cast<const void*>(kb), 128 * 1024);
             const int ldsb = 8 * 8192 > 32 * 1024 + tab_bytes + 8192 ? 8 * 8192 : 32 * 1024 + tab_bytes + 8192;
             hipLaunchKernelGGL(kb, dim3(B * nh * (hp / 8)), dim3(8 * 64), ldsb, st, (const T*)q, (const T*)k, (const T*)vt, (const T*)nullptr,
@@ -896,7 +947,7 @@
             const int nb_big = cdiv(nqt, 14), qw_big = cdiv(nqt, nb_big);
 #define BS_ATTN_BIG(QWB)                                                                                                                     \
     do {                                                                                                                                     \
-        auto kb = attention_tab2_kernel<T, QWB, 4, false, true>;                                                                             \
+        auto kb = attention_tab2_kernel<T, QWB, 4, false, true, false, VR>;                                                                  \
         BS_MAX_DYNAMIC_LDS(reinterpret_cast<const void*>(kb), 128 * 1024); \
         const int ldsb = QWB * 8192 > 32 * 1024 + tab_bytes ? QWB * 8192 : 32 * 1024 + tab_bytes;                                            \
         hipLaunchKernelGGL(kb, dim3(B * nh * nb_big), dim3(QWB * 64), ldsb, st, (const T*)q, (const T*)k, (const T*)vt, (const T*)nullptr,   \
@@ -915,6 +966,7 @@
         BS_CHECK_LAUNCH();
         return BS_OK;
     }
+    if constexpr (VR) { set_error("bs_attention_table: the V-rows mode is built for the pipelined kernel (hp even; hp=%d)", hp); return BS_ERR_INVALID; }
     hipLaunchKernelGGL(kern, dim3(B * nh * nqb), dim3(QW * 64), smem, st, (const T*)q, (const T*)k, (const T*)vt, table, (T*)out, split, B,
                        nh, hp, Sp, nqb, ntab, grouped, diag_env("BS_ATTN_ABLATE") ? atoi(diag_env("BS_ATTN_ABLATE")) : 0);
     BS_CHECK_LAUNCH();
@@ -971,12 +1023,17 @@
     BS_REQUIRE(Sp % 64 == 0 && Sp >= S, "%s: Sp=%d must be a multiple of 64 and >= S=%d", who, Sp, S);
     int split = (dtype & 32) ? 2 : ((dtype & 16) ? 1 : 0);
     if ((dtype & 64) && split == 2) split |= 4;
+    const bool vrows = (dtype & 128) != 0;
     dtype &= 15;
     BS_REQUIRE(dtype == BS_F16 || dtype == BS_BF16, "%s: dtype", who);
+    BS_REQUIRE(!vrows || hp % 2 == 0, "%s: the V-rows mode is built for an even number of patch rows (hp=%d)", who, hp);
     if (B == 0) return BS_OK;
     hipStream_t st = reinterpret_cast<hipStream_t>(stream);
-    return dtype == BS_F16 ? launch_attn_tab<f16>(q, k, vt, ql, kl, vtl, table, out, split, B, nh, hp, Sp, grouped, st)
-                           : launch_attn_tab<bf16>(q, k, vt, ql, kl, vtl, table, out, split, B, nh, hp, Sp, grouped, st);
+    if (vrows)
+        return dtype == BS_F16 ? launch_attn_tab<f16, true>(q, k, vt, ql, kl, vtl, table, out, split, B, nh, hp, Sp, grouped, st)
+                               : launch_attn_tab<bf16, true>(q, k, vt, ql, kl, vtl, table, out, split, B, nh, hp, Sp, grouped, st);
+    return dtype == BS_F16 ? launch_attn_tab<f16, false>(q, k, vt, ql, kl, vtl, table, out, split, B, nh, hp, Sp, grouped, st)
+                           : launch_attn_tab<bf16, false>(q, k, vt, ql, kl, vtl, table, out, split, B, nh, hp, Sp, grouped, st);
 }
 
 extern "C" int bs_attention_table(const void* q, const void* k, const void* vt, const float* table, void* out, int32_t B, int32_t nh,
diff --git a/bodyslam_amd/csrc/engine.hip b/bodyslam_amd/csrc/engine.hip
--- a/bodyslam_amd/csrc/engine.hip
+++ b/bodyslam_amd/csrc/engine.hip
@@ -14,7 +14,7 @@
 
 namespace {
 
-constexpr char kMagic[8] = {'B', 'S', 'E', 'N', 'G', '0', '2', '\0'};
+constexpr char kMagic[8] = {'B', 'S', 'E', 'N', 'G', '0', '3', '\0'};
 enum { KIND_WORKSPACE = 0, KIND_ZERO = 1, KIND_DATA = 2 };
 enum { ARG_I64 = 0, ARG_F64 = 1, ARG_PTR = 2, ARG_NULL = 3, ARG_DESC = 4 };
 enum { OP_CALL = 0, OP_SIGNAL = 1, OP_WAIT = 2 };
diff --git a/bodyslam_amd/csrc/igemm.hip b/bodyslam_amd/csrc/igemm.hip
--- a/bodyslam_amd/csrc/igemm.hip
+++ b/bodyslam_amd/csrc/igemm.hip
@@ -205,6 +205,8 @@
     p.qkv_cls_rows = d->qkv_cls_rows;
     p.qkv_patch_row0 = d->qkv_patch_row0;
     p.qkv_lo_off = d->qkv_lo_off;
+    p.qkv_v_rows = d->qkv_v_rows != 0;
+    BS_REQUIRE(!d->qkv_v_rows || d->out_mode == BS_OUT_QKV, "bs_gemm: qkv_v_rows needs BS_OUT_QKV");
     p.out2_relu = d->out2_relu;
     BS_REQUIRE(!d->out2_relu || (d->out2 && d->out_mode == BS_OUT_PLAIN && d->out_f8 && !d->scale && !d->out_group_rows && !d->bias_group_rows &&
                                  !d->bias2 && (d->act == BS_ACT_NONE || d->act == BS_ACT_RELU) && d->out_split_off == d->N && d->N % 256 == 0 &&
diff --git a/bodyslam_amd/csrc/igemm_kernel.h b/bodyslam_amd/csrc/igemm_kernel.h
--- a/bodyslam_amd/csrc/igemm_kernel.h
+++ b/bodyslam_amd/csrc/igemm_kernel.h
@@ -35,6 +35,7 @@
     int qkv_cls_rows;
     int qkv_patch_row0;
     int qkv_lo_off;
+    int qkv_v_rows;
     int f8_wonly_from;
     float q_scale;
     int ntm, ntn;
@@ -649,7 +650,7 @@
     (void)frow; (void)fq;
     {
     const int n_wave = tn * BN + wn * TN;
-    const bool v_tile = (p.out_mode == BS_OUT_QKV) && (tn * BN >= 2 * p.qkv_hidden);
+    const bool v_tile = (p.out_mode == BS_OUT_QKV) && !p.qkv_v_rows && (tn * BN >= 2 * p.qkv_hidden);
     if (p.ablate & 4) {
         if (acc[0][0][0] == 12345.678f) reinterpret_cast<float*>(p.out)[0] = 1.f;
         return;
@@ -667,6 +668,7 @@
         auto epi = [&](auto act_tag) {
             constexpr int ACT = decltype(act_tag)::value;
             BS_FRESH_LANE
+            void* const out_v = p.out3;
             f32x4 bj[FN], sj[FN];
             int n0j[FN];
             int64_t coff[FN];
@@ -695,6 +697,7 @@
 #pragma unroll
                         for (int e = 0; e < 4; ++e) { sj[j][e] *= p.q_scale; bj[j][e] *= 1.0f; }
                     }
+                    if (w_ == 2) sj[j] = f32x4{1.f, 1.f, 1.f, 1.f};
                 }
             }
             const bool wide_ok = (p.out_mode == BS_OUT_QKV) || (p.ldo % 8 == 0 && p.split_off % 8 == 0);
@@ -797,6 +800,7 @@
                     const int j0 = jp * 2, j1 = j0 + 1;
                     if (n0j[j0] >= p.N) continue;
                     void* dst = (p.out_mode == BS_OUT_QKV && which[j0] == 1) ? p.out2 : p.out;
+                    if (p.out_mode == BS_OUT_QKV && which[j0] == 2) dst = out_v;
                     const int so = p.out_mode != BS_OUT_QKV ? p.split_off : p.qkv_lo_off;
                     if (F8 && p.out_f8) {
                         const int nloc = p.out_mode == BS_OUT_SHUFFLE ? n0j[j0] % p.shuffle_cout : n0j[j0];
@@ -809,6 +813,7 @@
                         if (n0j[j1] < p.N) {
                             const float(&yb)[4] = *reinterpret_cast<const float(*)[4]>(y8 + 4);
                             void* dst1 = (p.out_mode == BS_OUT_QKV && which[j1] == 1) ? p.out2 : p.out;
+                            if (p.out_mode == BS_OUT_QKV && which[j1] == 2) dst1 = out_v;
                             store4<T>(dst1, roff + coff[j1], p.out_dtype, yb, so);
                         }
                     }
@@ -1028,8 +1033,13 @@
             p.out_dtype != BS_F32 && !(p.ablate & 16)) {
             BS_FRESH_LANE
             const int part = (tn * BN) / p.qkv_hidden;
-            T* dst = reinterpret_cast<T*>(part == 1 ? p.out2 : p.out);
+            T* const dst_q = reinterpret_cast<T*>(p.out);
+            T* const dst_k = reinterpret_cast<T*>(p.out2);
+            T* const dst_v = reinterpret_cast<T*>(p.out3);
+            T* dst = part == 1 ? dst_k : dst_q;
+            if (part == 2) dst = dst_v;
             const float qs = part == 0 ? p.q_scale : 1.0f;
+            const bool use_scale = p.scale && part != 2;
             f32x4 bj[FN], sj[FN];
             int64_t coff[FN / 2];
 #pragma unroll
@@ -1037,7 +1047,7 @@
                 const int n0 = n_wave + (j >> 1) * 32 + fq * 8 + (j & 1) * 4;
                 bj[j] = *reinterpret_cast<const f32x4*>(p.bias + n0);
                 if (g2 >= 0) bj[j] += *reinterpret_cast<const f32x4*>(p.bias2 + (int64_t)g2 * p.N + n0);
-                sj[j] = p.scale ? *reinterpret_cast<const f32x4*>(p.scale + n0) : f32x4{1.f, 1.f, 1.f, 1.f};
+                sj[j] = use_scale ? *reinterpret_cast<const f32x4*>(p.scale + n0) : f32x4{1.f, 1.f, 1.f, 1.f};
 #pragma unroll
                 for (int e = 0; e < 4; ++e) sj[j][e] *= qs;
                 if (!(j & 1)) {
diff --git a/bodyslam_amd/engine_export.py b/bodyslam_amd/engine_export.py
--- a/bodyslam_amd/engine_export.py
+++ b/bodyslam_amd/engine_export.py
@@ -9,7 +9,7 @@
 
 from . import _lib as L
 
-MAGIC = b"BSENG02\0"
+MAGIC = b"BSENG03\0"
 KIND_WORKSPACE, KIND_ZERO, KIND_DATA = 0, 1, 2
 ARG_I64, ARG_F64, ARG_PTR, ARG_NULL, ARG_DESC = 0, 1, 2, 3, 4
 OP_CALL = 0
diff --git a/bodyslam_amd/zoedepth.py b/bodyslam_amd/zoedepth.py
--- a/bodyslam_amd/zoedepth.py
+++ b/bodyslam_amd/zoedepth.py
@@ -88,6 +88,7 @@
 AUTO_CAL_SEEDS = DEFAULT_POLICY.cal_seeds
 AUTO_HOLDOUT_SEEDS = DEFAULT_POLICY.holdout_seeds
 ACCURATE_NECK_MODE = "full"
+QKV_V_ROWS = True
 
 _CALIBRATION_CACHE: Dict[Tuple, dict] = {}
 _ARITHMETIC_SWITCHES = ("BS_UPCONV_FUSED", "BS_NECK_PLAIN", "BS_MLP2", "BS_NECK_BIAS_CORR", "BS_PROJECTOR_LEVEL", "BS_AUTO_WSTAT")
@@ -199,6 +200,7 @@
         self._bias_corr_cache: Dict[str, torch.Tensor] = {}
         self.neck_mode = neck_mode or os.environ.get("BS_NECK_MODE") or ACCURATE_NECK_MODE
         self.fuse_mlp = int(os.environ.get("BS_MLP2", "2"))
+        self.qkv_v_rows = {"1": False, "0": True}.get(os.environ.get("BS_QKV_VT", ""), QKV_V_ROWS)
         c_ = self.cfg
         self.neck_f8 = self.acc and self.neck_mode != "pairs" and all(v % 128 == 0 for v in (c_.hidden, c_.fusion, c_.fusion // 2, *c_.neck_hidden))
         with torch.no_grad():
@@ -694,6 +696,7 @@
         self.NSP = (32 if nf8 else 16) if acc else 0
         self.RZ = 1 | ((4 if nf8 else 2) if acc else 0)
         self.attn_corr = bool(acc and eng.attn_mode == "corr" and self.use_tab and hp % 2 == 0)
+        self.v_rows = bool(eng.qkv_v_rows and self.use_tab and hp % 2 == 0)
 
         x = self._embed()
         taps16 = self._backbone(x)
@@ -842,6 +845,8 @@
         bias = eng._rel_table(hp, wp) if use_tab else eng._rel_bias(hp, wp, Sp)
         xn = z16(MT, Hd * m2)
         QN = NB * c.heads * Sp * 64
+        v_rows = self.v_rows
+        vr = 128 if v_rows else 0
         q, k, vt = z16((2 if corr else 1) * NB, c.heads, Sp, 64), z16((2 if corr else 1) * NB, c.heads, Sp, 64), z16((2 if corr else 1) * NB, c.heads, 64, Sp)
         ao = z16(MT, Hd * m2)
         hid = z16(MT, c.intermediate * m2)
@@ -851,13 +856,13 @@
             P.add(f"l{l}.ln1", "bs_layernorm", x, w[f"l{l}.ln1.g"], w[f"l{l}.ln1.b"], xn, None, MT, Hd, c.ln_eps,
                   L.dt(xn) | fmt(f"l{l}.qkv.w") | prow(f"l{l}.qkv.w"))
             bgemm(f"l{l}.qkv", xn, f"l{l}.qkv.w", q, MT, 3 * Hd, Hd, bias=w[f"l{l}.qkv.b"],
-                  qkv=(Hd, S, Sp, LOG2E / math.sqrt(64.0), k, vt, use_tab, NB if grouped else 0, CP, QN if corr else 0))
+                  qkv=(Hd, S, Sp, LOG2E / math.sqrt(64.0), k, vt, use_tab, NB if grouped else 0, CP, QN if corr else 0, v_rows))
             if corr:
                 P.add(f"l{l}.attn", "bs_attention_table_corr", q, k, vt, q.view(-1)[QN:], k.view(-1)[QN:], vt.view(-1)[QN:], bias[l], ao, NB,
-                      c.heads, hp, wp, Sp, CP, L.dt(q) | fmt(f"l{l}.o.w") | (64 if prow(f"l{l}.o.w") else 0))
+                      c.heads, hp, wp, Sp, CP, L.dt(q) | fmt(f"l{l}.o.w") | (64 if prow(f"l{l}.o.w") else 0) | vr)
             elif use_tab:
                 P.add(f"l{l}.attn", "bs_attention_table", q, k, vt, bias[l], ao, NB, c.heads, hp, wp, Sp, CP,
-                      L.dt(q) | fmt(f"l{l}.o.w") | (64 if prow(f"l{l}.o.w") else 0))
+                      L.dt(q) | fmt(f"l{l}.o.w") | (64 if prow(f"l{l}.o.w") else 0) | vr)
             else:
                 P.add(f"l{l}.attn", "bs_attention", q, k, vt, bias[l], ao, NB, c.heads, S, Sp, L.dt(q) | fmt(f"l{l}.o.w"))
             bgemm(f"l{l}.o", ao, f"l{l}.o.w", x, MT, Hd, Hd, bias=w[f"l{l}.o.b"], scale=w[f"l{l}.lam1"], res=x, ldr=Hd)
diff --git a/include/bodyslam_hip.h b/include/bodyslam_hip.h
--- a/include/bodyslam_hip.h
+++ b/include/bodyslam_hip.h
@@ -71,6 +71,7 @@
     const float* bias2;
     int32_t qkv_lo_off;
     int32_t out2_relu;
+    int32_t qkv_v_rows;
 } bs_gemm_desc;
 int bs_gemm(const bs_gemm_desc* d, void* stream);
 int bs_gemm_tile(const bs_gemm_desc* d);
```

After: 497.6, median of 6. No clear change (+0.4%).
